# theo2021/OnDA

Hardware: AMD Instinct MI355X
Metric: adaptation-step images/sec (fwd+bwd+proto) 512x1024 bs=4 (higher is better)
Workload: dtype f32 (f16x2 split emulation); 1 GPU; hybrid_switch adaptation step (step + update_ema), 1024x512, bs=4 per micro-batch, 1 micro-batch(es) per GPU and optimizer step, dynamic branch, DeepLabV2-ResNet50 ProDA head, random-init weights; global_batch=4, parallelism=dp1, branch=dynamic, micro_batches_per_gpu=1, inputs=resident in HBM

## Files before the change

include/onda_hip.h:

```cpp
#ifndef ONDA_HIP_H
#define ONDA_HIP_H

#include <stdint.h>

#ifdef __cplusplus
extern "C" {
#endif

typedef void* onda_stream_t;

#define ONDA_OK 0
#define ONDA_EINVAL (-1)
#define ONDA_EALIGN (-2)

typedef struct OndaConv {
  int B, Hi, Wi, Cin;
  int Ho, Wo, Cout;
  int kh, kw, stride, dil, pad;
  int ldx;
  int ldy;
  int ldr;
  int out_os;
  int Hf, Wf;
  int relu;
  const int32_t* run_if;
  int64_t stat_split;
  int32_t plain_schedule;
  const int32_t* pix_table;
  int64_t pix_stride;
} OndaConv;

int onda_conv_tiles_m(int M);
int onda_conv_tiles_mc(int M, int Cout);

int64_t onda_conv_ws_floats(void);
int onda_conv2d_fwd(const float* x, const float* w, float* y, const float* scale, const float* shift,
                    const float* residual, float* stats, float* ws, const OndaConv* c, onda_stream_t s);

#define ONDA_AMAX_SLOTS 64
#define ONDA_AMAX_FLOATS 2048
int onda_absmax(const float* x, int64_t rows, int C, int ld, float* amax, onda_stream_t s);
int onda_pack_weight_h2(const float* w_oihw, void* dst, int Cout, int Cin, int taps, int rows_pad, int Kp, int dgrad,
                        int Cout_pad, const float* amax, onda_stream_t s);
typedef struct {
  const float* w;
  void* fwd;
  void* dgrad;
  float* amax;
  int Cout, Cin, taps;
  int first_block;
} OndaPackEntry;
int onda_pack_blocks(int Cout, int Cin, int taps);
int onda_pack_weights_h2_multi(const OndaPackEntry* table, int n, int64_t total_blocks, onda_stream_t s);
int onda_split_h2(const float* x, int64_t rows, int C, int ldx, void* dst, int ldo, int64_t plane, const float* amax,
                  onda_stream_t s);
typedef struct OndaLimbOut {
  void* out;
  int64_t out_plane;
  float* out_bound;
  float* out_amax;
  const float* kb;
  const float* xtrue;
  const void* res;
  int64_t res_plane;
  const float* res_amax;
  const float* res_true;
} OndaLimbOut;
int onda_conv2d_fwd_l2_limbs(const void* xl, int64_t xplane, const float* xamax, const void* w2, const float* wamax,
                             const float* scale, const float* shift, const OndaLimbOut* lo, float* ws, const OndaConv* c,
                             onda_stream_t s);

void onda_debug_stamps(void* buffer);

int onda_stem_im2col_l2(const float* x_nchw, const float* xamax, void* dst, int64_t plane, int B, int H, int W, int Ho, int Wo,
                        int Kp, onda_stream_t s);
int onda_s2d_split_h2(const float* x, int nchw, int B, int C, int H, int W, int ldx, float slope, const float* amax, void* dst,
                      onda_stream_t s);
int onda_d2s_bwd(const float* gs, const float* gamax, const float* x, int nchw, int B, int C, int H, int W, int ldx, float slope,
                 void* dst_limbs, float* dst_f32, onda_stream_t s);
int onda_conv_l2_variant(int64_t M, int Cout);
int onda_conv_l2_kernel_id(int64_t M, int Cout, int taps, int Cin);
int onda_conv_l2_tiles_m(int64_t M, int Cout, int taps, int Cin);
int onda_conv_l2_tiles_m_split(int64_t M, int Cout, int taps, int Cin, int64_t stat_split, int plain_schedule, int* tile_rows);
double onda_conv_l2_live_fraction(const OndaConv* c, int with_stats);
double onda_conv_wgrad_l2_live_fraction(const OndaConv* c, int splitk);
int onda_conv2d_fwd_l2(const void* xl, int64_t xplane, const float* xamax, const void* w2, const float* wamax, float* y,
                       const float* scale, const float* shift, const float* residual, float* stats, int stats_rows, float* ws,
                       float* yamax, const OndaConv* c, onda_stream_t s);

int onda_bn_finalize_l2(const float* partials, int tiles, int C, int64_t count, float eps, float* mean, float* invstd,
                        float* running_mean, float* running_var, int64_t* nbt, float momentum, const float* gamma,
                        const float* beta, const float* res_amax, int relu, float* xhat_amax, float* out_amax, int64_t split,
                        int tile_rows, int run_group, const float* y, int ldy, onda_stream_t s);
int onda_bn_apply_l2(const float* x, const float* mean, const float* invstd, const float* gamma, const float* beta,
                     const void* res, int64_t res_plane, const float* res_amax, void* out, int64_t out_plane,
                     const float* out_amax, int64_t M, int C, int relu, uint8_t* relu_mask, int64_t split, onda_stream_t s);
int onda_bn_train_l2(const float* x, const float* partials, int tiles, float eps, float* mean, float* invstd, float* running_mean,
                     float* running_var, int64_t* nbt, float momentum, const float* gamma, const float* beta, const void* res,
                     const float* res_amax, int relu, float* xhat_amax, void* out, float* out_amax, int64_t M, int C,
                     uint8_t* relu_mask, int64_t split, int tile_rows, int run_group, onda_stream_t s);
int64_t onda_bn_bwd_l2_ws(int64_t M, int C);
int onda_bn_bwd_l2(const float* dout, const void* out, int64_t out_plane, const float* x, const float* mean, const float* invstd,
                   const float* gamma, const float* xhat_amax, void* dx, int64_t dx_plane, float* dx_amax, float* dres, float* ws,
                   int64_t M, int C, int relu, const uint8_t* relu_mask, int64_t split, int fuse_sums, onda_stream_t s);

int onda_conv_wgrad_l2_variant(int Cout, int Cin);
int64_t onda_conv2d_wgrad_l2_table_stride(const OndaConv* c);
int onda_conv2d_wgrad_l2_table(const OndaConv* c, int32_t* table, onda_stream_t s);
int onda_conv2d_wgrad_l2(const void* xl, int64_t xplane, const float* xamax, const void* dyl, int64_t dyplane, const float* dyamax,
                         float* slabs, int lddy, int splitk, const OndaConv* c, onda_stream_t s);

int onda_conv2d_wgrad(const float* x, const float* dy, float* slabs, int lddy, int splitk,
                      const OndaConv* c, onda_stream_t s);
int onda_wgrad_reduce(const float* slabs, float* dw, int splitk, int Cout, int taps, int Cin,
                      int Cout_real, int Cin_real, int flat_k, int accumulate, onda_stream_t s);

int onda_pack_weight_fwd(const float* w_oihw, float* dst, int Cout, int Cin, int taps, int Cout_pad, int Kp,
                         onda_stream_t s);
int onda_pack_weight_dgrad(const float* w_oihw, float* dst, int Cout, int Cin, int taps, int Cout_pad,
                           onda_stream_t s);

int onda_stem_im2col(const float* x_nchw, float* col, int B, int H, int W, int Ho, int Wo, int Kp, onda_stream_t s);

int onda_bn_finalize(const float* partials, int tiles, int C, int64_t count, float eps, float* mean, float* invstd,
                     float* running_mean, float* running_var, int64_t* num_batches_tracked, float momentum,
                     onda_stream_t s);
int onda_bn_stats(const float* x, int64_t M, int C, int ldx, float* partials, int* tiles_out, onda_stream_t s);
int onda_bn_apply(const float* x, const float* mean, const float* invstd, const float* gamma, const float* beta,
                  const float* residual, float* out, int64_t M, int C, int relu, float* amax, onda_stream_t s);
int onda_bn_fold(const float* gamma, const float* beta, const float* running_mean, const float* running_var,
                 float eps, float* scale, float* shift, int C, onda_stream_t s);
int64_t onda_bn_bwd_ws(int64_t M, int C);
int onda_bn_bwd(const float* dout, const float* out, const float* x, const float* mean, const float* invstd,
                const float* gamma, float* dx, float* dres, float* ws, int64_t M, int C, int relu, float* amax, onda_stream_t s);

int64_t onda_gn_ws(int B, int64_t HW, int C);
int onda_gn_fwd(const float* x, int ldx, const float* gamma, const float* beta, const float* chmul, float* out, int ldo,
                float* mean, float* rstd, float* ws, int B, int64_t HW, int C, int groups, float eps, int relu,
                float* amax ,
                onda_stream_t s);
int onda_gn_bwd(const float* dout, int lddo, const float* out, int ldo, const float* x, int ldx, const float* gamma,
                const float* chmul, const float* mean, const float* rstd, float* dx, float* dgamma, float* dbeta,
                float* ws, int B, int64_t HW, int C, int groups, int relu, onda_stream_t s);

int onda_maxpool_fwd(const float* x, float* y, uint8_t* idx, int B, int Hi, int Wi, int C, int Ho, int Wo,
                     onda_stream_t s);
int onda_maxpool_fwd_limbs(const float* x, const float* xamax, void* yl, uint8_t* idx, int B, int Hi, int Wi, int C, int Ho, int Wo,
                           onda_stream_t s);
int onda_maxpool_bwd(const float* dy, const uint8_t* idx, float* dx, int B, int Hi, int Wi, int C, int Ho, int Wo,
                     onda_stream_t s);

int64_t onda_colsum_ws(int B, int64_t HW, int C);
int onda_colsum(const float* x, int ldx, const float* y, int ldy, float* out, float alpha, float* ws, int B,
                int64_t HW, int C, onda_stream_t s);
int onda_se_fc_fwd(const float* pooled, const float* w1, const float* b1, const float* w2, const float* b2,
                   float* hidden, float* gate, int B, int C, int R, onda_stream_t s);
int onda_se_fc_bwd(const float* dgate, const float* pooled, const float* hidden, const float* gate, const float* w1,
                   const float* w2, float* dw1, float* db1, float* dw2, float* db2, float* dpooled, float* ws,
                   float dpooled_scale, int B, int C, int R, onda_stream_t s);
int onda_chan_scale(const float* x, const float* gate, const float* add, float* out, int B, int64_t HW, int C,
                    onda_stream_t s);
int onda_chan_scale_limbs(const float* x, const float* gate, void* out, int64_t out_plane, const float* x_amax, int B, int64_t HW,
                          int C, onda_stream_t s);

int onda_upsample_fwd(const float* logits, int ldl, float* out_nchw, int B, int h, int w, int K, int H, int W,
                      onda_stream_t s);
int onda_upsample_bwd(const float* dout_nchw, float* dlogits, int ldl, int B, int h, int w, int K, int H, int W,
                      onda_stream_t s);
int onda_upsample_ce_fused(int w, int W);
int64_t onda_upsample_ce_ws(int B, int H, int W);
int onda_upsample_ce_fwd(const float* logits, int ldl, const uint8_t* labels, float* result, float* ws, int B, int h, int w, int K,
                         int H, int W, onda_stream_t s);
int64_t onda_upsample_ce_bwd_ws(int B, int w, int K, int H);
int onda_upsample_ce_bwd(const float* logits, int ldl, const uint8_t* labels, const float* result, const float* gscale, float w_ce,
                         float* dlogits, float* ws, int B, int h, int w, int K, int H, int W, onda_stream_t s);
int onda_upsample_entropy_fwd(const float* logits, int ldl, float* out, int B, int h, int w, int K, int H, int W, onda_stream_t s);
int64_t onda_upsample_entropy_bwd_ws(int B, int w, int K, int H, int W);
int onda_upsample_entropy_bwd(const float* logits, int ldl, const float* dout, float* dlogits, float* ws, int B, int h, int w, int K,
                              int H, int W, onda_stream_t s);
int onda_upsample_argmax(const float* logits, int ldl, uint8_t* cls, int B, int h, int w, int K, int H, int W,
                         onda_stream_t s);

int onda_upsample_argmax_hist(const float* logits, int ldl, const uint8_t* labels, int64_t* hist, uint8_t* cls, int B,
                              int h, int w, int K, int H, int W, onda_stream_t s);

int onda_ece_bins_local(void);
int onda_upsample_ece(const float* rows, int ld, const uint8_t* labels, int64_t* table, int bins, int probs, int64_t* hist, int B,
                      int h, int w, int K, int H, int W, onda_stream_t s);

int onda_softmax_stats(const float* logits, int ldl, float* probs, int ldp, int32_t* argmax, float* result,
                       float* ws, int64_t N, int K, onda_stream_t s);

int onda_seg_loss_fwd(const float* logits, int ldl, const int64_t* labels, float* result, float* ws, int64_t N, int K,
                      onda_stream_t s);
int onda_seg_loss_bwd(const float* logits, int ldl, const int64_t* labels, const float* result, const float* gscale,
                      float w_ce, float w_rce, float w_reg, float* dlogits, int64_t N, int K, onda_stream_t s);

int onda_target_loss_fwd(const float* logits, int ldl, const int64_t* labels, int regularizer, float w_ce, float w_rce,
                         float w_reg, float w_js, float* result, float* ws, int64_t N, int K, onda_stream_t s);
int onda_target_loss_bwd(const float* logits, int ldl, const int64_t* labels, int regularizer, float w_ce, float w_rce,
                         float w_reg, float w_js, const float* result, const float* gscale, float* dlogits, int64_t N,
                         int K, onda_stream_t s);

int onda_proto_assign_blocks(int64_t N);
int onda_proto_sigma(const float* proto, const float* sqmean, const float* counter, float* sigma, int K, int C,
                     onda_stream_t s);
int onda_proto_assign(const float* feat, int ldf, const float* prior, int ldp, const float* proto, const float* sigma,
                      int mahalanobis, float tau, float thresh, int64_t* labels, float* soft, float* result,
                      float* ws, int64_t N, int C, int K, onda_stream_t s);
int onda_proto_distances(const float* feat, int ldf, const float* proto, const float* sigma, int mahalanobis, float* dist,
                         int64_t N, int C, int K, onda_stream_t s);
int64_t onda_proto_sums_ws(int64_t N, int C, int K);
int onda_proto_class_sums(const float* feat, int ldf, const int32_t* cls, float* sums, float* counts, float* ws,
                          int64_t N, int C, int K, onda_stream_t s);
int onda_proto_ema(float* proto, float* sqmean, const float* sums, const float* counts, float lam, int K, int C,
                   onda_stream_t s);
int onda_proto_append(float* proto, float* sqmean, float* counter, const float* sums, const float* counts, int K,
                      int C, onda_stream_t s);

typedef struct OndaSgdEntry {
  float* p; const float* g; float* buf; int64_t n; float lr; int times; int fresh;
  int first_block;
} OndaSgdEntry;
int onda_multi_tensor_block(void);
int onda_sgd_multi(const OndaSgdEntry* table, int n, float momentum, float weight_decay, float grad_scale,
                   int64_t total_blocks, onda_stream_t s);
typedef struct OndaEmaEntry { float* k; const float* q; int64_t n; float keep; float blend; int first_block; } OndaEmaEntry;
int onda_ema_multi(const OndaEmaEntry* table, int n, int64_t total_blocks, onda_stream_t s);

int onda_resample_h_u8(const unsigned char* in, unsigned char* out, int H, int Win, int Wout, const int* bounds,
                       const int* kk, int ksize, onda_stream_t s);
int onda_resample_v_norm(const unsigned char* tmp, float* out, int Hin, int W, int Hout, const int* bounds, const int* kk,
                         int ksize, const float* mean3, const float* std3, int flip, onda_stream_t s);
int onda_resize_nearest_lut(const unsigned char* in, unsigned char* out, int Win, int Hout, int Wout, const int* xtab,
                            const int* ytab, const unsigned char* lut256, onda_stream_t s);

const char* onda_version(void);
float onda_limb2_scale(void);

typedef struct OndaSwitchCfg {
  int limit;
  int level_kind;
  int use_exp;
  int pad_;
  double exp_const, one_minus_exp_const, taps_total;
  double gray_lo, gray_hi, dev_threshold;
} OndaSwitchCfg;
int onda_switch_state_doubles(int limit);
int onda_switch_max_window(void);
int onda_switch_step(double* state, int32_t* istate, const void* sample, int sample_f64, const double* taps,
                     const OndaSwitchCfg* cfg, int32_t* flag, onda_stream_t s);
int onda_select_prior(const int32_t* flag, const float* a, float wa, const float* b, float wb, float* out, int64_t n,
                      onda_stream_t s);
int onda_gate_scalar(const int32_t* flag, const float* v, float* out, onda_stream_t s);

#ifdef __cplusplus
}
#endif
#endif
```

onda_amd/_lib.py:

```python
import ctypes
import os
from ctypes import POINTER, Structure, c_char_p, c_float, c_int, c_int64, c_void_p

HERE = os.path.dirname(os.path.abspath(__file__))
LIB_PATH = os.environ.get("ONDA_LIB_PATH") or os.path.join(HERE, "libonda_hip.so")

P = c_void_p
I, L, F = c_int, c_int64, c_float


class OndaConv(Structure):
    _fields_ = [(n, c_int) for n in ("B Hi Wi Cin Ho Wo Cout kh kw stride dil pad ldx ldy ldr out_os Hf Wf relu").split()] + \
               [("run_if", c_void_p), ("stat_split", c_int64), ("plain_schedule", c_int), ("pix_table", c_void_p),
                ("pix_stride", c_int64)]


class OndaSwitchCfg(Structure):
    _fields_ = [("limit", c_int), ("level_kind", c_int), ("use_exp", c_int), ("pad_", c_int), ("exp_const", ctypes.c_double),
                ("one_minus_exp_const", ctypes.c_double), ("taps_total", ctypes.c_double), ("gray_lo", ctypes.c_double),
                ("gray_hi", ctypes.c_double), ("dev_threshold", ctypes.c_double)]


class OndaLimbOut(Structure):
    _fields_ = [("out", c_void_p), ("out_plane", c_int64), ("out_bound", c_void_p), ("out_amax", c_void_p), ("kb", c_void_p),
                ("xtrue", c_void_p), ("res", c_void_p), ("res_plane", c_int64), ("res_amax", c_void_p), ("res_true", c_void_p)]


class OndaSgdEntry(Structure):
    _fields_ = [("p", c_void_p), ("g", c_void_p), ("buf", c_void_p), ("n", c_int64), ("lr", c_float),
                ("times", c_int), ("fresh", c_int), ("first_block", c_int)]


class OndaPackEntry(Structure):
    _fields_ = [("w", c_void_p), ("fwd", c_void_p), ("dgrad", c_void_p), ("amax", c_void_p), ("Cout", c_int), ("Cin", c_int),
                ("taps", c_int), ("first_block", c_int)]


class OndaEmaEntry(Structure):
    _fields_ = [("k", c_void_p), ("q", c_void_p), ("n", c_int64), ("keep", c_float), ("blend", c_float), ("first_block", c_int)]


SIGNATURES = {
    "onda_conv_tiles_m": (I, [I]),
    "onda_conv_tiles_mc": (I, [I, I]),
    "onda_conv_ws_floats": (L, []),
    "onda_conv2d_fwd": (I, [P, P, P, P, P, P, P, P, POINTER(OndaConv), P]),
    "onda_absmax": (I, [P, L, I, I, P, P]),
    "onda_pack_weight_h2": (I, [P, P, I, I, I, I, I, I, I, P, P]),
    "onda_pack_weights_h2_multi": (I, [P, I, L, P]),
    "onda_pack_blocks": (I, [I, I, I]),
    "onda_split_h2": (I, [P, L, I, I, P, I, L, P, P]),
    "onda_stem_im2col_l2": (I, [P, P, P, L, I, I, I, I, I, I, P]),
    "onda_s2d_split_h2": (I, [P, I, I, I, I, I, I, F, P, P, P]),
    "onda_d2s_bwd": (I, [P, P, P, I, I, I, I, I, I, F, P, P, P]),
    "onda_debug_stamps": (None, [P]),
    "onda_conv2d_fwd_l2_limbs": (I, [P, L, P, P, P, P, P, P, P, P, P]),
    "onda_switch_state_doubles": (I, [I]),
    "onda_switch_max_window": (I, []),
    "onda_switch_step": (I, [P, P, P, I, P, POINTER(OndaSwitchCfg), P, P]),
    "onda_select_prior": (I, [P, P, F, P, F, P, L, P]),
    "onda_gate_scalar": (I, [P, P, P, P]),
    "onda_conv_l2_variant": (I, [L, I]),
    "onda_conv_l2_kernel_id": (I, [L, I, I, I]),
    "onda_conv_l2_tiles_m": (I, [L, I, I, I]),
    "onda_conv_l2_tiles_m_split": (I, [L, I, I, I, L, I, POINTER(c_int)]),
    "onda_conv_l2_live_fraction": (ctypes.c_double, [POINTER(OndaConv), I]),
    "onda_conv_wgrad_l2_live_fraction": (ctypes.c_double, [POINTER(OndaConv), I]),
    "onda_conv_wgrad_l2_variant": (I, [I, I]),
    "onda_conv2d_wgrad_l2_table_stride": (L, [POINTER(OndaConv)]),
    "onda_conv2d_wgrad_l2_table": (I, [POINTER(OndaConv), P, P]),
    "onda_conv2d_wgrad_l2": (I, [P, L, P, P, L, P, P, I, I, POINTER(OndaConv), P]),
    "onda_conv2d_fwd_l2": (I, [P, L, P, P, P, P, P, P, P, P, I, P, P, POINTER(OndaConv), P]),
    "onda_bn_finalize_l2": (I, [P, I, I, L, F, P, P, P, P, P, F, P, P, P, I, P, P, L, I, I, P, I, P]),
    "onda_bn_apply_l2": (I, [P, P, P, P, P, P, L, P, P, L, P, L, I, I, P, L, P]),
    "onda_bn_bwd_l2_ws": (L, [L, I]),
    "onda_bn_train_l2": (I, [P, P, I, F, P, P, P, P, P, F, P, P, P, P, I, P, P, P, L, I, P, L, I, I, P]),
    "onda_bn_bwd_l2": (I, [P, P, L, P, P, P, P, P, P, L, P, P, P, L, I, I, P, L, I, P]),
    "onda_conv2d_wgrad": (I, [P, P, P, I, I, POINTER(OndaConv), P]),
    "onda_wgrad_reduce": (I, [P, P, I, I, I, I, I, I, I, I, P]),
    "onda_pack_weight_fwd": (I, [P, P, I, I, I, I, I, P]),
    "onda_pack_weight_dgrad": (I, [P, P, I, I, I, I, P]),
    "onda_stem_im2col": (I, [P, P, I, I, I, I, I, I, P]),
    "onda_bn_finalize": (I, [P, I, I, L, F, P, P, P, P, P, F, P]),
    "onda_bn_stats": (I, [P, L, I, I, P, POINTER(c_int), P]),
    "onda_bn_apply": (I, [P, P, P, P, P, P, P, L, I, I, P, P]),
    "onda_bn_fold": (I, [P, P, P, P, F, P, P, I, P]),
    "onda_bn_bwd_ws": (L, [L, I]),
    "onda_bn_bwd": (I, [P, P, P, P, P, P, P, P, P, L, I, I, P, P]),
    "onda_gn_ws": (L, [I, L, I]),
    "onda_gn_fwd": (I, [P, I, P, P, P, P, I, P, P, P, I, L, I, I, F, I, P, P]),
    "onda_gn_bwd": (I, [P, I, P, I, P, I, P, P, P, P, P, P, P, P, I, L, I, I, I, P]),
    "onda_maxpool_fwd": (I, [P, P, P, I, I, I, I, I, I, P]),
    "onda_maxpool_fwd_limbs": (I, [P, P, P, P, I, I, I, I, I, I, P]),
    "onda_maxpool_bwd": (I, [P, P, P, I, I, I, I, I, I, P]),
    "onda_colsum_ws": (L, [I, L, I]),
    "onda_colsum": (I, [P, I, P, I, P, F, P, I, L, I, P]),
    "onda_se_fc_fwd": (I, [P, P, P, P, P, P, P, I, I, I, P]),
    "onda_se_fc_bwd": (I, [P, P, P, P, P, P, P, P, P, P, P, P, F, I, I, I, P]),
    "onda_chan_scale": (I, [P, P, P, P, I, L, I, P]),
    "onda_chan_scale_limbs": (I, [P, P, P, L, P, I, L, I, P]),
    "onda_upsample_fwd": (I, [P, I, P, I, I, I, I, I, I, P]),
    "onda_upsample_bwd": (I, [P, P, I, I, I, I, I, I, I, P]),
    "onda_upsample_argmax": (I, [P, I, P, I, I, I, I, I, I, P]),
    "onda_upsample_ce_fused": (I, [I, I]),
    "onda_upsample_ce_ws": (L, [I, I, I]),
    "onda_upsample_ce_fwd": (I, [P, I, P, P, P, I, I, I, I, I, I, P]),
    "onda_upsample_ce_bwd_ws": (L, [I, I, I, I]),
    "onda_upsample_ce_bwd": (I, [P, I, P, P, P, F, P, P, I, I, I, I, I, I, P]),
    "onda_upsample_entropy_fwd": (I, [P, I, P, I, I, I, I, I, I, P]),
    "onda_upsample_entropy_bwd_ws": (L, [I, I, I, I, I]),
    "onda_upsample_entropy_bwd": (I, [P, I, P, P, P, I, I, I, I, I, I, P]),
    "onda_upsample_argmax_hist": (I, [P, I, P, P, P, I, I, I, I, I, I, P]),
    "onda_ece_bins_local": (I, []),
    "onda_upsample_ece": (I, [P, I, P, P, I, I, P, I, I, I, I, I, I, P]),
    "onda_softmax_stats": (I, [P, I, P, I, P, P, P, L, I, P]),
    "onda_seg_loss_fwd": (I, [P, I, P, P, P, L, I, P]),
    "onda_seg_loss_bwd": (I, [P, I, P, P, P, F, F, F, P, L, I, P]),
    "onda_target_loss_fwd": (I, [P, I, P, I, F, F, F, F, P, P, L, I, P]),
    "onda_target_loss_bwd": (I, [P, I, P, I, F, F, F, F, P, P, P, L, I, P]),
    "onda_proto_sigma": (I, [P, P, P, P, I, I, P]),
    "onda_proto_assign_blocks": (I, [L]),
    "onda_proto_assign": (I, [P, I, P, I, P, P, I, F, F, P, P, P, P, L, I, I, P]),
    "onda_proto_distances": (I, [P, I, P, P, I, P, L, I, I, P]),
    "onda_proto_sums_ws": (L, [L, I, I]),
    "onda_proto_class_sums": (I, [P, I, P, P, P, P, L, I, I, P]),
    "onda_proto_ema": (I, [P, P, P, P, F, I, I, P]),
    "onda_proto_append": (I, [P, P, P, P, P, I, I, P]),
    "onda_sgd_multi": (I, [P, I, F, F, F, L, P]),
    "onda_ema_multi": (I, [P, I, L, P]),
    "onda_multi_tensor_block": (I, []),
    "onda_resample_h_u8": (I, [P, P, I, I, I, P, P, I, P]),
    "onda_resample_v_norm": (I, [P, P, I, I, I, P, P, I, POINTER(c_float), POINTER(c_float), I, P]),
    "onda_resize_nearest_lut": (I, [P, P, I, I, I, P, P, P, P]),
    "onda_version": (c_char_p, []),
    "onda_limb2_scale": (F, []),
}

_lib = None


class OndaLibraryError(RuntimeError):
    pass


def load():
    global _lib
    if _lib is not None:
        return _lib
    if not os.path.exists(LIB_PATH):
        raise OndaLibraryError(
            f"{LIB_PATH} is missing: build it with `python -m onda_amd.build` (hipcc --offload-arch=gfx950). "
            "onda_amd has no fallback path.")
    import torch
    lib = ctypes.CDLL(LIB_PATH)
    for name, (res, args) in SIGNATURES.items():
        try:
            fn = getattr(lib, name)
        except AttributeError as e:
            raise OndaLibraryError(f"{LIB_PATH} does not export {name}") from e
        fn.restype, fn.argtypes = res, args
    _lib = lib
    return lib


def call(name, *args):
    rc = getattr(load(), name)(*args)
    if rc != 0:
        kind = {-1: "ONDA_EINVAL (unsupported shape / null pointer)", -2: "ONDA_EALIGN (16-byte alignment)"}.get(
            rc, f"hipError_t {rc}")
        raise RuntimeError(f"{name} failed: {kind}")


def query(name, *args):
    return getattr(load(), name)(*args)
```

onda_amd/csrc/common.h:

```cpp
#pragma once
#include <hip/hip_runtime.h>
#include <stdint.h>
#include <stdio.h>
#include <stdlib.h>

#include "onda_hip.h"

#ifndef ONDA_LIMB2_SCALE
#define ONDA_LIMB2_SCALE 2048.f
#endif
typedef float f32x4 __attribute__((ext_vector_type(4)));
typedef float f32x16 __attribute__((ext_vector_type(16)));

constexpr int LIMB2_OFS = 32;
__host__ __device__ __forceinline__ size_t limb_at(size_t row, int c, int ld) {
  return row * 2 * (size_t)ld + (size_t)((c >> 5) << 6) + (size_t)(c & 31);
}

#define ONDA_STREAM(s) (reinterpret_cast<hipStream_t>(s))
#define ONDA_REQUIRE(cond)                                                                              \
  do {                                                                                                  \
    (void)hipGetLastError();                                                                            \
    if (!(cond)) {                                                                                      \
      if (getenv("ONDA_DEBUG_REQUIRE")) fprintf(stderr, "onda_hip: %s:%d: requirement failed: %s\n", __FILE__, __LINE__, #cond); \
      return ONDA_EINVAL;                                                                               \
    }                                                                                                   \
  } while (0)
#define ONDA_ALIGNED16(p) ((reinterpret_cast<uintptr_t>(p) & 15u) == 0)
#define ONDA_LAUNCH_RESULT() static_cast<int>(hipGetLastError())

static inline int64_t ceil_div64(int64_t a, int64_t b) { return (a + b - 1) / b; }

__device__ __forceinline__ float wave_sum(float v) {
#pragma unroll
  for (int o = 32; o > 0; o >>= 1) v += __shfl_xor(v, o, 64);
  return v;
}
__device__ __forceinline__ float wave_max(float v) {
#pragma unroll
  for (int o = 32; o > 0; o >>= 1) v = fmaxf(v, __shfl_xor(v, o, 64));
  return v;
}

constexpr int AMAX_STRIDE = ONDA_AMAX_FLOATS / ONDA_AMAX_SLOTS;
__device__ __forceinline__ void amax_update(float* amax, float m) {
  m = wave_max(m);
  if ((threadIdx.x & 63) == 0 && m > 0.f)
    atomicMax(reinterpret_cast<unsigned*>(amax) + ((blockIdx.x * 4 + (threadIdx.x >> 6)) & (ONDA_AMAX_SLOTS - 1)) * AMAX_STRIDE,
              __float_as_uint(m));
}
__device__ __forceinline__ void amax_update_block(float* amax, float m, float* red) {
  m = wave_max(m);
  if ((threadIdx.x & 63) == 0) red[threadIdx.x >> 6] = m;
  __syncthreads();
  if (threadIdx.x == 0) {
    m = fmaxf(fmaxf(red[0], red[1]), fmaxf(red[2], red[3]));
    if (m > 0.f)
      atomicMax(reinterpret_cast<unsigned*>(amax) + (blockIdx.x & (ONDA_AMAX_SLOTS - 1)) * AMAX_STRIDE, __float_as_uint(m));
  }
}
__device__ __forceinline__ float amax_read(const float* __restrict__ amax) {
  static_assert(ONDA_AMAX_SLOTS == 64, "one slot per lane");
  return wave_max(amax[(threadIdx.x & 63) * AMAX_STRIDE]);
}

__device__ __forceinline__ double wave_sum_d(double v) {
#pragma unroll
  for (int o = 32; o > 0; o >>= 1) v += __shfl_xor(v, o, 64);
  return v;
}

__device__ __forceinline__ float block_sum_256(float v, float* red) {
  v = wave_sum(v);
  __syncthreads();
  if ((threadIdx.x & 63) == 0) red[threadIdx.x >> 6] = v;
  __syncthreads();
  return red[0] + red[1] + red[2] + red[3];
}
```

onda_amd/csrc/conv_l2.hip:

```cpp
#include "conv_common.h"

namespace {

typedef _Float16 f16x8 __attribute__((ext_vector_type(8)));
typedef _Float16 f16x2 __attribute__((ext_vector_type(2)));
typedef _Float16 f16x4 __attribute__((ext_vector_type(4)));
typedef float f32x2 __attribute__((ext_vector_type(2)));
typedef unsigned int u32x2 __attribute__((ext_vector_type(2)));
typedef unsigned int u32x4 __attribute__((ext_vector_type(4)));
typedef int i32x4 __attribute__((ext_vector_type(4)));

#define ZZ(i, jj) (((i) & 1) ? 3 - (jj) : (jj))

constexpr float LIMB2_SCALE = ONDA_LIMB2_SCALE, LIMB2_UNSCALE = 1.f / ONDA_LIMB2_SCALE;

#ifndef ONDA_NT_OUT
#define ONDA_NT_OUT 1
#endif
constexpr int NT_AUX = ONDA_NT_OUT ? 2 : 0;
template <class T>
__device__ __forceinline__ void store_out(T* p, T v) {
  if constexpr (ONDA_NT_OUT) __builtin_nontemporal_store(v, p); else *p = v;
}
constexpr unsigned OOB = 0x80000000u;

__device__ __forceinline__ __amdgpu_buffer_rsrc_t make_rsrc(const void* base, unsigned bytes) {
  return __builtin_amdgcn_make_buffer_rsrc(const_cast<void*>(base), 0, (int)bytes, 0x00020000);
}
__device__ __forceinline__ int swz8(int row) { return (row & 15) >> 1; }
__device__ __forceinline__ unsigned dma_chunk16(int lane, int odd) { return (unsigned)(((lane & 7) ^ (4 * odd + (lane >> 4))) << 4); }
__device__ __forceinline__ int frag_ofs(int lane, int limb) {
  return (lane & 15) * 128 + ((((limb << 2) | (lane >> 4)) ^ swz8(lane & 15)) << 4);
}
struct RowPos {
  int hw;
  int bH;
};
__device__ __forceinline__ RowPos row_pos(int m, int M, const OndaConv& c, int b0) {
  const bool vm = m < M;
  const int mm = vm ? m : 0;
  const int wo = mm % c.Wo, tq = mm / c.Wo;
  const int ho = tq % c.Ho, b = tq / c.Ho;
  const int hi0 = vm ? ho * c.stride - c.pad : -32768, wi0 = wo * c.stride - c.pad;
  return RowPos{(int)((unsigned)(hi0 & 0xFFFF) | ((unsigned)wi0 << 16)), (vm ? b - b0 : 0) * c.Hi};
}
__device__ __forceinline__ __amdgpu_buffer_rsrc_t x_window(const ConvK& a, int m0, int& b0) {
  const OndaConv& c = a.c;
  b0 = m0 / (c.Ho * c.Wo);
  const long long at = (long long)b0 * c.Hi * c.Wi * c.ldx * 4, left = a.x_total - at;
  return make_rsrc(reinterpret_cast<const char*>(a.x) + at, (unsigned)(left < 0x7FFFF000ll ? left : 0x7FFFF000ll));
}
__device__ __forceinline__ unsigned row_tap_ofs(const RowPos& p, int rr, int ss, const OndaConv& c, unsigned chunk16) {
  const int hi = (int)(short)(p.hw & 0xFFFF) + rr * c.dil, wi = (p.hw >> 16) + ss * c.dil;
  const bool ok = (unsigned)hi < (unsigned)c.Hi && (unsigned)wi < (unsigned)c.Wi;
  return ok ? (unsigned)(((p.bH + hi) * c.Wi + wi) * c.ldx) * 4u + chunk16 : 0x80000000u;
}

struct Scale2 {
  float s, inv;
};
__device__ __forceinline__ Scale2 scale_from(float m);
__device__ __forceinline__ Scale2 scale_of(const float* __restrict__ amax) { return scale_from(amax_read(amax)); }
__device__ __forceinline__ Scale2 scale_from(const float m) {
  int e = 0;
  if (m > 0.f && m < 3.0e38f) {
    int ex;
    frexpf(m, &ex);
    e = 15 - ex;
    e = e > 100 ? 100 : (e < -100 ? -100 : e);
  }
  return Scale2{ldexpf(1.f, e), ldexpf(1.f, -e)};
}

__device__ __forceinline__ unsigned cvt2h(float lo, float hi) {
  return __builtin_bit_cast(unsigned, __builtin_convertvector(f32x2{lo, hi}, f16x2));
}
__device__ __forceinline__ f32x2 unpack2h(unsigned p) {
  return __builtin_convertvector(__builtin_bit_cast(f16x2, p), f32x2);
}

__global__ __launch_bounds__(256) void split_h2_kernel(const float* __restrict__ x, long long rows, int C, int ldx,
                                                       _Float16* __restrict__ dst, int ldo, long long plane,
                                                       const float* __restrict__ amax) {
  const float s = scale_of(amax).s;
  const int c8 = C >> 3;
  const long long n = rows * c8;
  for (long long e = (long long)blockIdx.x * 256 + threadIdx.x; e < n; e += (long long)gridDim.x * 256) {
    const long long row = e / c8;
    const int ch = (int)(e - row * c8) * 8;
    const f32x4 v0 = *reinterpret_cast<const f32x4*>(x + row * ldx + ch) * s;
    const f32x4 v1 = *reinterpret_cast<const f32x4*>(x + row * ldx + ch + 4) * s;
    u32x4 l1, l2;
#pragma unroll
    for (int h = 0; h < 4; ++h) {
      const float a = h < 2 ? v0[2 * h] : v1[2 * h - 4], b = h < 2 ? v0[2 * h + 1] : v1[2 * h - 3];
      const unsigned p = cvt2h(a, b);
      const f32x2 f = unpack2h(p);
      l1[h] = p;
      l2[h] = cvt2h((a - f[0]) * LIMB2_SCALE, (b - f[1]) * LIMB2_SCALE);
    }
    _Float16* o = dst + limb_at((size_t)row, ch, ldo);
    *reinterpret_cast<u32x4*>(o) = l1;
    *reinterpret_cast<u32x4*>(o + LIMB2_OFS) = l2;
  }
}

__global__ __launch_bounds__(256) void stem_im2col_l2_kernel(const float* __restrict__ x, _Float16* __restrict__ dst,
                                                             long long plane, int B, int H, int W, int Ho, int Wo, int Kp,
                                                             const float* __restrict__ amax) {
  const float sc = scale_of(amax).s;
  const int k8 = Kp >> 3;
  const long long n = (long long)B * Ho * Wo * k8;
  for (long long e = (long long)blockIdx.x * 256 + threadIdx.x; e < n; e += (long long)gridDim.x * 256) {
    const long long m = e / k8;
    const int k0 = (int)(e - m * k8) * 8;
    const int wo = (int)(m % Wo);
    const long long tq = m / Wo;
    const int ho = (int)(tq % Ho), b = (int)(tq / Ho);
    float v[8];
#pragma unroll
    for (int j = 0; j < 8; ++j) {
      const int k = k0 + j;
      float val = 0.f;
      if (k < 147) {
        const int tap = k / 3, cc = k - tap * 3;
        const int r = tap / 7, t7 = tap - r * 7;
        const int hi = ho * 2 - 3 + r, wi = wo * 2 - 3 + t7;
        if ((unsigned)hi < (unsigned)H && (unsigned)wi < (unsigned)W) val = x[(((size_t)b * 3 + cc) * H + hi) * W + wi];
      }
      v[j] = val * sc;
    }
    u32x4 l1, l2;
#pragma unroll
    for (int h = 0; h < 4; ++h) {
      const unsigned pk = cvt2h(v[2 * h], v[2 * h + 1]);
      const f32x2 f = unpack2h(pk);
      l1[h] = pk;
      l2[h] = cvt2h((v[2 * h] - f[0]) * LIMB2_SCALE, (v[2 * h + 1] - f[1]) * LIMB2_SCALE);
    }
    _Float16* o = dst + limb_at((size_t)m, k0, Kp);
    *reinterpret_cast<u32x4*>(o) = l1;
    *reinterpret_cast<u32x4*>(o + LIMB2_OFS) = l2;
  }
}

#define ONDA_SWAP4(INSN, A, B)                                                                                          \
  asm volatile("s_nop 1\n\t" INSN " %0, %4\n\t" INSN " %1, %5\n\t" INSN " %2, %6\n\t" INSN " %3, %7\n\ts_nop 0"         \
               : "+v"(A[0]), "+v"(A[1]), "+v"(A[2]), "+v"(A[3]), "+v"(B[0]), "+v"(B[1]), "+v"(B[2]), "+v"(B[3]))
__device__ __forceinline__ void rows_reduce4(float& s1, float& s2, float& mn, float& mx) {
#if defined(__HIP_DEVICE_COMPILE__)
  float A[4] = {s1, s2, mn, mx}, B[4] = {s1, s2, mn, mx};
  ONDA_SWAP4("v_permlane16_swap_b32", A, B);
  float C[4] = {A[0] + B[0], A[1] + B[1], fminf(A[2], B[2]), fmaxf(A[3], B[3])};
  float D[4] = {C[0], C[1], C[2], C[3]};
  ONDA_SWAP4("v_permlane32_swap_b32", C, D);
  s1 = C[0] + D[0];
  s2 = C[1] + D[1];
  mn = fminf(C[2], D[2]);
  mx = fmaxf(C[3], D[3]);
#endif
}

template <int WM, int WN, bool COUNTED = false, bool AFFINE = true>
__device__ __forceinline__ void l2_epilogue(const ConvK& a, const f32x4 (&acc)[4][4], unsigned char* scratch, int tile_m, int m0,
                                            int n0, int wm, int wn, int lane, float ua, float ub, unsigned y_bytes = 0) {
  constexpr int BN = 64 * WN, NW = WM * WN, NT = NW * 64;
  constexpr int TRS = 68;
  const OndaConv& c = a.c;
  const int t = threadIdx.x, wave = t >> 6;
  unsigned long long* est = a.stamps != nullptr && t == 0 ? a.stamps + (size_t)blockIdx.x * 32 + 24 : nullptr;
  if (est) est[0] = __builtin_amdgcn_s_memtime();
  float* red = reinterpret_cast<float*>(scratch + NW * (16 * TRS * 4));
  const int SR = a.stats_rows;
  if (a.stats != nullptr) {
#pragma unroll
    for (int jn = 0; jn < 4; ++jn) {
      float s1 = 0.f, s2 = 0.f, mn = 3.0e38f, mxv = -3.0e38f;
#pragma unroll
      for (int i = 0; i < 4; ++i)
#pragma unroll
        for (int e = 0; e < 4; ++e) {
          const float v = acc[i][jn][e];
          s1 += v;
          s2 += v * v;
          mn = fminf(mn, v);
          mxv = fmaxf(mxv, v);
        }
      rows_reduce4(s1, s2, mn, mxv);
      if (lane < 16) {
        const int col = (wn * 4 + jn) * 16 + lane;
        red[(wm * BN + col) * 4 + 0] = (s1 * ua) * ub;
        red[(wm * BN + col) * 4 + 1] = (((s2 * ua) * ub) * ua) * ub;
        red[(wm * BN + col) * 4 + 2] = (mn * ua) * ub;
        red[(wm * BN + col) * 4 + 3] = (mxv * ua) * ub;
      }
    }
  }

  if (est) est[1] = __builtin_amdgcn_s_memtime();
  const bool plain = (c.out_os == 1 && c.Hf == c.Ho && c.Wf == c.Wo);
  const int cl = (lane & 15) * 4, rl = lane >> 4;
  const int n = n0 + wn * 64 + cl;
  const bool vn = n < c.Cout;
  f32x4 sc = {1.f, 1.f, 1.f, 1.f}, sh = {0.f, 0.f, 0.f, 0.f};
  if constexpr (AFFINE) {
    if (vn && a.scale) sc = *reinterpret_cast<const f32x4*>(a.scale + n);
    if (vn && a.shift) sh = *reinterpret_cast<const f32x4*>(a.shift + n);
  }
  sc = (sc * ua) * ub;
  float* tr = reinterpret_cast<float*>(scratch + wave * (16 * TRS * 4));
  float mx = 0.f;
  f32x4 rv[4][4];
  if (AFFINE && a.res) {
#pragma unroll
    for (int i = 0; i < 4; ++i)
#pragma unroll
      for (int r = 0; r < 4; ++r) {
        const int m = m0 + (wm * 4 + i) * 16 + 4 * r + rl;
        const bool live = m < a.M && vn;
        rv[i][r] = live ? *reinterpret_cast<const f32x4*>(a.res + (size_t)m * c.ldr + n) : f32x4{0.f, 0.f, 0.f, 0.f};
      }
  }
  const bool track = a.amax != nullptr;
  const bool full_rows = m0 + 64 * WM <= a.M;
  const int mw = m0 + wm * 64 + rl;
  const unsigned vbase = vn ? (unsigned)(((size_t)(mw - m0) * c.ldy + n) * 4) : OOB;
  const long long y_left = (long long)(a.M - m0) * c.ldy * 4;
  const unsigned y_win = (unsigned)(y_left < 0x7FFFF000ll ? y_left : 0x7FFFF000ll);
  float* const ytile = a.y + (size_t)m0 * c.ldy;
  float* const ybase = a.y + (size_t)mw * c.ldy + n;
#pragma unroll
  for (int i = 0; i < 4; ++i) {
#pragma unroll
    for (int jn = 0; jn < 4; ++jn)
#pragma unroll
      for (int e = 0; e < 4; ++e) tr[(4 * (lane >> 4) + e) * TRS + jn * 16 + (lane & 15)] = acc[i][jn][e];
    __builtin_amdgcn_wave_barrier();
#pragma unroll
    for (int r = 0; r < 4; ++r) {
      const int row = 4 * r + rl;
      f32x4 v = *reinterpret_cast<const f32x4*>(tr + row * TRS + cl);
      const int m = mw + i * 16 + 4 * r;
      const bool live = (full_rows || m < a.M) && vn;
      if constexpr (AFFINE) {
        v = v * sc + sh;
        if (a.res) v += rv[i][r];
        if (c.relu) {
#pragma unroll
          for (int q = 0; q < 4; ++q) v[q] = fmaxf(v[q], 0.f);
        }
      } else {
        v = v * sc;
      }
      if (plain) {
        if constexpr (COUNTED) {
#if defined(__HIP_DEVICE_COMPILE__)
          __builtin_amdgcn_raw_buffer_store_b128(__builtin_bit_cast(u32x4, v), make_rsrc(ytile, y_win),
                                                 vbase + (unsigned)((i * 16 + 4 * r) * c.ldy * 4), 0, NT_AUX);
#endif
        } else if (live) {
          store_out(reinterpret_cast<f32x4*>(ybase + (size_t)((i * 16 + 4 * r) * c.ldy)), v);
        }
      } else {
        const int mm = live ? m : 0;
        const int wo = mm % c.Wo, tq = mm / c.Wo;
        const int ho = tq % c.Ho, b = tq / c.Ho;
        const size_t orow = ((size_t)b * c.Hf + (size_t)ho * c.out_os) * c.Wf + (size_t)wo * c.out_os;
        if constexpr (COUNTED) {
#if defined(__HIP_DEVICE_COMPILE__)
          const unsigned off = live ? (unsigned)((orow * c.ldy + n) * 4) : OOB;
          __builtin_amdgcn_raw_buffer_store_b128(__builtin_bit_cast(u32x4, v), make_rsrc(a.y, y_bytes), off, 0, NT_AUX);
#endif
        } else if (live) {
          store_out(reinterpret_cast<f32x4*>(a.y + orow * c.ldy + n), v);
        }
      }
      if (track && live) mx = fmaxf(fmaxf(mx, fmaxf(fabsf(v[0]), fabsf(v[1]))), fmaxf(fabsf(v[2]), fabsf(v[3])));
    }
    __builtin_amdgcn_wave_barrier();
  }
  if (est) est[2] = __builtin_amdgcn_s_memtime();
  float* ar = red + WM * BN * 4;
  if (a.amax != nullptr) {
    mx = wave_max(mx);
    if (lane == 0) ar[wave] = mx;
  }
  if (a.stats != nullptr || a.amax != nullptr) {
    if constexpr (COUNTED) {
      asm volatile("s_waitcnt lgkmcnt(0)" ::: "memory");
      __builtin_amdgcn_s_barrier();
    } else {
      __syncthreads();
    }
  }
  if (est) est[3] = __builtin_amdgcn_s_memtime();
  if (a.stats != nullptr) {
    for (int col = t; col < BN; col += NT) {
      if (n0 + col >= c.Cout) continue;
      float s1 = 0.f, s2 = 0.f, mn = 3.0e38f, mxv = -3.0e38f;
#pragma unroll
      for (int w_ = 0; w_ < WM; ++w_) {
        s1 += red[(w_ * BN + col) * 4 + 0];
        s2 += red[(w_ * BN + col) * 4 + 1];
        mn = fminf(mn, red[(w_ * BN + col) * 4 + 2]);
        mxv = fmaxf(mxv, red[(w_ * BN + col) * 4 + 3]);
      }
      float* dst = a.stats + (size_t)tile_m * SR * c.Cout + n0 + col;
      dst[0] = s1;
      dst[c.Cout] = s2;
      if (SR == 4) {
        dst[2 * c.Cout] = mn;
        dst[3 * c.Cout] = mxv;
      }
    }
  }
  if (a.amax != nullptr && t == 0) {
    float m = ar[0];
#pragma unroll
    for (int w_ = 1; w_ < NW; ++w_) m = fmaxf(m, ar[w_]);
    if (m > 0.f)
      atomicMax(reinterpret_cast<unsigned*>(a.amax) + (blockIdx.x & (ONDA_AMAX_SLOTS - 1)) * AMAX_STRIDE, __float_as_uint(m));
  }
  if (est) est[4] = __builtin_amdgcn_s_memtime();
}

__device__ __forceinline__ float limb_out_bound(const ConvK& a) {
  float b = amax_read(a.xtrue) * a.kb[0] + a.kb[1];
  if (a.resl != nullptr) b += amax_read(a.res_true);
  return b * 1.0001f;
}

template <int WM, int WN, bool COUNTED>
__device__ __forceinline__ void l2_epilogue_limbs(const ConvK& a, const f32x4 (&acc)[4][4], unsigned char* scratch, int m0, int n0,
                                                  int wm, int wn, int lane, float ua, float ub) {
  constexpr int BN = 64 * WN, NW = WM * WN;
  constexpr int TRS = 68;
  const OndaConv& c = a.c;
  if constexpr (COUNTED) asm volatile("" : "+v"(lane));
  int t = threadIdx.x;
  if constexpr (COUNTED) asm volatile("" : "+v"(t));
  const int wave = t >> 6;
  const float bound = limb_out_bound(a);
  const float so = scale_from(bound).s;
  if (t == 0) a.ybound[(blockIdx.x & (ONDA_AMAX_SLOTS - 1)) * AMAX_STRIDE] = bound;
  const float ri = a.resl != nullptr ? scale_of(a.res_amax).inv : 0.f;
  const int cl = (lane & 15) * 4, rl = lane >> 4;
  const int n = n0 + wn * 64 + cl;
  const bool vn = n < c.Cout;
  f32x4 sc = {1.f, 1.f, 1.f, 1.f}, sh = {0.f, 0.f, 0.f, 0.f};
  if (vn && a.scale) sc = *reinterpret_cast<const f32x4*>(a.scale + n);
  if (vn && a.shift) sh = *reinterpret_cast<const f32x4*>(a.shift + n);
  sc = (sc * ua) * ub;
  float* tr = reinterpret_cast<float*>(scratch + wave * (16 * TRS * 4));
  float* ar = reinterpret_cast<float*>(scratch + NW * (16 * TRS * 4));
  const int mw = m0 + wm * 64 + rl;
  u32x2 r1[4][4], r2[4][4];
  if (a.resl != nullptr) {
#pragma unroll
    for (int i = 0; i < 4; ++i)
#pragma unroll
      for (int r = 0; r < 4; ++r) {
        const int m = mw + i * 16 + 4 * r;
        const bool live = m < a.M && vn;
        const _Float16* p = a.resl + limb_at((size_t)(live ? m : 0), live ? n : 0, c.ldr);
        r1[i][r] = live ? *reinterpret_cast<const u32x2*>(p) : u32x2{0u, 0u};
        r2[i][r] = live ? *reinterpret_cast<const u32x2*>(p + LIMB2_OFS) : u32x2{0u, 0u};
      }
  }
  float mx = 0.f;
  const long long out_left = (long long)(a.M - m0) * c.ldy * 4;
  const unsigned out_bytes = (unsigned)(out_left < 0x7FFFF000ll ? out_left : 0x7FFFF000ll);
  _Float16* const ytile = a.yl + (size_t)m0 * 2 * c.ldy;
#pragma unroll
  for (int i = 0; i < 4; ++i) {
#pragma unroll
    for (int jn = 0; jn < 4; ++jn)
#pragma unroll
      for (int e = 0; e < 4; ++e) tr[(4 * (lane >> 4) + e) * TRS + jn * 16 + (lane & 15)] = acc[i][jn][e];
    __builtin_amdgcn_wave_barrier();
#pragma unroll
    for (int r = 0; r < 4; ++r) {
      const int row = 4 * r + rl;
      f32x4 v = *reinterpret_cast<const f32x4*>(tr + row * TRS + cl);
      const int m = mw + i * 16 + 4 * r;
      const bool live = m < a.M && vn;
      v = v * sc + sh;
      if (a.resl != nullptr) {
#pragma unroll
        for (int h = 0; h < 2; ++h) {
          const f32x2 p1 = unpack2h(r1[i][r][h]), p2 = unpack2h(r2[i][r][h]);
          v[2 * h] += (p1[0] + p2[0] * LIMB2_UNSCALE) * ri;
          v[2 * h + 1] += (p1[1] + p2[1] * LIMB2_UNSCALE) * ri;
        }
      }
      if (c.relu) {
#pragma unroll
        for (int q = 0; q < 4; ++q) v[q] = fmaxf(v[q], 0.f);
      }
      if (live) mx = fmaxf(fmaxf(mx, fmaxf(fabsf(v[0]), fabsf(v[1]))), fmaxf(fabsf(v[2]), fabsf(v[3])));
      const f32x4 w = v * so;
      u32x2 l1, l2;
#pragma unroll
      for (int h = 0; h < 2; ++h) {
        const unsigned pk = cvt2h(w[2 * h], w[2 * h + 1]);
        const f32x2 f = unpack2h(pk);
        l1[h] = pk;
        l2[h] = cvt2h((w[2 * h] - f[0]) * LIMB2_SCALE, (w[2 * h + 1] - f[1]) * LIMB2_SCALE);
      }
      if constexpr (COUNTED) {
#if defined(__HIP_DEVICE_COMPILE__)
        const unsigned off = vn ? (unsigned)(limb_at((size_t)(m - m0), n, c.ldy) * 2) : OOB;
        __builtin_amdgcn_raw_buffer_store_b64(l1, make_rsrc(ytile, out_bytes), off, 0, NT_AUX);
        __builtin_amdgcn_raw_buffer_store_b64(l2, make_rsrc(ytile, out_bytes), off, 2 * LIMB2_OFS, NT_AUX);
#endif
      } else if (live) {
        _Float16* dst = a.yl + limb_at((size_t)m, n, c.ldy);
        store_out(reinterpret_cast<u32x2*>(dst), l1);
        store_out(reinterpret_cast<u32x2*>(dst + LIMB2_OFS), l2);
      }
    }
    __builtin_amdgcn_wave_barrier();
  }
  if (a.amax != nullptr) {
    mx = wave_max(mx);
    if (lane == 0) ar[wave] = mx;
    if constexpr (COUNTED) {
      asm volatile("s_waitcnt lgkmcnt(0)" ::: "memory");
      __builtin_amdgcn_s_barrier();
    } else {
      __syncthreads();
    }
    if (t == 0) {
      float mm = ar[0];
#pragma unroll
      for (int w_ = 1; w_ < NW; ++w_) mm = fmaxf(mm, ar[w_]);
      if (mm > 0.f)
        atomicMax(reinterpret_cast<unsigned*>(a.amax) + (blockIdx.x & (ONDA_AMAX_SLOTS - 1)) * AMAX_STRIDE, __float_as_uint(mm));
    }
  }
}

template <int WM, int WN, int STAGES, int OCC, bool SK, int DBG = 0>
__global__ __launch_bounds__(WM * WN * 64, OCC) void conv_l2_kernel(const ConvK a, unsigned xplane, unsigned wplane, unsigned x_bytes,
                                                                   unsigned w_bytes, const float* __restrict__ xamax,
                                                                   const float* __restrict__ wamax) {
// ... 1188 lines not shown
      }
    }
  }

  f32x4 acc[4][4], accx[4][4];
#pragma unroll
  for (int i = 0; i < 4; ++i)
#pragma unroll
    for (int j = 0; j < 4; ++j)
#pragma unroll
      for (int e = 0; e < 4; ++e) acc[i][j][e] = accx[i][j][e] = 0.f;

  if (stp) {
    stp[1] = __builtin_amdgcn_s_memtime();
    stp[5] = (unsigned long long)nlive;
  }
  int i_cur = 0, i_iss = 0;
  int st_issue = 0, st_read = 0;
  auto issue_next = [&]() {
    issue(live_at(i_iss), st_issue);
    st_issue = st_issue + STAGE == STAGES * STAGE ? 0 : st_issue + STAGE;
    ++i_iss;
  };
  bool second_part_due = false;
  auto issue_first_part = [&]() {
    second_part_due = i_iss < nlive;
    if (second_part_due) {
      issue_addr(live_at(i_iss), st_issue);
      issue_part(0);
      st_issue = st_issue + STAGE == STAGES * STAGE ? 0 : st_issue + STAGE;
      ++i_iss;
    }
  };
  auto issue_second_part = [&]() {
    if (second_part_due) issue_part(1);
    second_part_due = false;
  };
  auto wait_landed_half = [&](bool first_part_in_flight) {
    if (first_part_in_flight)
      asm volatile("s_waitcnt vmcnt(%0)" ::"n"(DPW / 2) : "memory");
    else
      asm volatile("s_waitcnt vmcnt(0)" ::: "memory");
  };
  auto wait_landed = [&](bool more_in_flight) {
    if (more_in_flight)
      asm volatile("s_waitcnt vmcnt(%0)" ::"n"(DPW) : "memory");
    else
      asm volatile("s_waitcnt vmcnt(0)" ::: "memory");
  };
  constexpr int AHEAD = STAGES >= 3 ? 2 : 1;
  static_assert(!STAGGER || STAGES >= 3, "the staggered halves need two steps in flight");
  if constexpr (MODE == 0) {
    if (i_iss < nlive) issue_next();
    if (AHEAD == 2 && i_iss < nlive) issue_next();
  }
  f16x8 af[4][2], bf[4], b1[4];
  const unsigned lds0 = (unsigned)(size_t)(__attribute__((address_space(3))) unsigned char*)lds;
  unsigned base;
  auto prepare = [&]() {
    base = lds0 + st_read;
    st_read = st_read + STAGE == STAGES * STAGE ? 0 : st_read + STAGE;
#pragma unroll
    for (int i = 0; i < 4; ++i) {
      const unsigned a0 = base + fa[i][0], a1 = base + fa[i][1];
      af[i][0] = tr_read8<0>(a0, a1);
      af[i][1] = tr_read8<256>(a0, a1);
    }
#pragma unroll
    for (int j = 0; j < 4; ++j) {
      const unsigned a0 = base + fb[j][0], a1 = base + fb[j][1];
      bf[j] = tr_read8<256>(a0, a1);
      if constexpr (STAGGER) b1[j] = tr_read8<0>(a0, a1);
    }
  };
  auto prepared = [&]() {
    lds_wait(af[0][0], af[1][0], af[2][0], af[3][0]);
    lds_wait(af[0][1], af[1][1], af[2][1], af[3][1]);
    lds_wait(bf[0], bf[1], bf[2], bf[3]);
    if constexpr (STAGGER) lds_wait(b1[0], b1[1], b1[2], b1[3]);
    __builtin_amdgcn_sched_barrier(0);
  };
  auto compute = [&]() {
    if constexpr (!STAGGER) {
#pragma unroll
      for (int j = 0; j < 4; ++j) b1[j] = tr_read8(base + fb[j][0], base + fb[j][1]);
    }
#pragma unroll
    for (int i = 0; i < 4; ++i)
#pragma unroll
      for (int jj = 0; jj < 4; ++jj) accx[i][ZZ(i, jj)] = __builtin_amdgcn_mfma_f32_16x16x32_f16(af[i][0], bf[ZZ(i, jj)], accx[i][ZZ(i, jj)], 0, 0, 0);
    if constexpr (!STAGGER) lds_wait(b1[0], b1[1], b1[2], b1[3]);
    if constexpr (STAGGER) issue_second_part();
    __builtin_amdgcn_sched_barrier(0);
#pragma unroll
    for (int i = 0; i < 4; ++i)
#pragma unroll
      for (int jj = 0; jj < 4; ++jj) accx[i][ZZ(i, jj)] = __builtin_amdgcn_mfma_f32_16x16x32_f16(af[i][1], b1[ZZ(i, jj)], accx[i][ZZ(i, jj)], 0, 0, 0);
#pragma unroll
    for (int i = 0; i < 4; ++i)
#pragma unroll
      for (int jj = 0; jj < 4; ++jj) acc[i][ZZ(i, jj)] = __builtin_amdgcn_mfma_f32_16x16x32_f16(af[i][0], b1[ZZ(i, jj)], acc[i][ZZ(i, jj)], 0, 0, 0);
  };
  if constexpr (MODE >= 1) {
    static_assert(STAGGER && GPW == 1 && STAGES == 3, "the eight-wave tile");
    const unsigned lddy4 = (unsigned)a.lddy * 4u, ldx4 = (unsigned)c.ldx * 4u;
    unsigned dy_lane[2], x_lane[2];
#pragma unroll
    for (int h = 0; h < 2; ++h) {
      const unsigned pix = (unsigned)(wave * 4 + 2 * lam + h);
      dy_lane[h] = pix * lddy4;
      x_lane[h] = (pix + (unsigned)(mbeg - b_first * c.Ho * c.Wo)) * ldx4;
    }
    const int base_px = b_first * c.Hi * c.Wi;
    const i32x4* tab = MODE == 2 ? reinterpret_cast<const i32x4*>(a.pix + (size_t)tap * a.pix_stride + mbeg + wave * 4) : nullptr;
    i32x4 t_next = {-1, -1, -1, -1};
    auto offsets = [&](int kt, const i32x4& te, unsigned kill) {
#pragma unroll
      for (int h = 0; h < 2; ++h) {
        pdy_s[0][h] = (unsigned)kt * 32u * lddy4 + dy_lane[h] + kill;
        if constexpr (MODE == 1) {
          px_s[0][h] = (unsigned)kt * 32u * ldx4 + x_lane[h] + kill;
        } else {
          const int lo = te[h], hi = te[2 + h];
          const int e = lam ? hi : lo;
          px_s[0][h] = (e >= 0 ? __umul24((unsigned)(e - base_px), ldx4) : PAST) + kill;
        }
      }
    };
    auto issue_first = [&]() {
      stage_s = st_issue;
      issue_part(0);
    };
    auto issue_second = [&]() {
      issue_part(1);
      st_issue = st_issue + STAGE == STAGES * STAGE ? 0 : st_issue + STAGE;
      ++i_iss;
    };
    auto issue_dmas = [&]() {
      issue_first();
      issue_second();
    };
    const unsigned long long tab_u = reinterpret_cast<unsigned long long>(tab);
    const unsigned tab_lo = __builtin_amdgcn_readfirstlane((unsigned)tab_u), tab_hi = __builtin_amdgcn_readfirstlane((unsigned)(tab_u >> 32));
    auto entry = [&](int kt) -> i32x4 {
      i32x4 r = {0, 0, 0, 0};
      if constexpr (MODE == 2) {
        const unsigned long long p = (((unsigned long long)tab_hi << 32) | tab_lo) + (unsigned long long)(unsigned)kt * 128ull;
        asm volatile("s_load_dwordx4 %0, %1, 0x0" : "=s"(r) : "s"(p));
      }
      return r;
    };
    auto entry_wait = [&](i32x4& r) {
      if constexpr (MODE == 2) asm volatile("s_waitcnt lgkmcnt(0)" : "+s"(r));
    };
    const int n_pre = late ? 3 : 2;
    if (nlive > 0) {
      for (int j = 0; j < n_pre; ++j) {
        const int kt = live_at(j < nlive ? j : 0);
        i32x4 te = entry(kt);
        entry_wait(te);
        offsets(kt, te, j < nlive ? 0u : PAST);
        issue_dmas();
      }
      int kt_next = live_at(i_iss < nlive ? i_iss : 0);
      t_next = entry(kt_next);
      entry_wait(t_next);
      if (late) {
        asm volatile("s_waitcnt vmcnt(%0)" ::"n"(2 * DPW) : "memory");
        __builtin_amdgcn_s_barrier();
      }
      for (; i_cur < nlive; ++i_cur) {
        if (!late) asm volatile("s_waitcnt vmcnt(%0)" ::"n"(DPW / 2) : "memory");
        __builtin_amdgcn_s_barrier();
        if (i_cur > 0) issue_second();
        const unsigned short ktv = live_list[i_iss + 1 < nlive ? i_iss + 1 : 0];
        prepare();
        prepared();
        const int kt_after = __builtin_amdgcn_readfirstlane((int)ktv);
        i32x4 t_after = entry(kt_after);
        if (late) asm volatile("s_waitcnt vmcnt(%0)" ::"n"(DPW) : "memory");
        __builtin_amdgcn_s_barrier();
        offsets(kt_next, t_next, i_iss < nlive ? 0u : PAST);
#pragma unroll
        for (int i = 0; i < 4; ++i)
#pragma unroll
          for (int jj = 0; jj < 4; ++jj) accx[i][ZZ(i, jj)] = __builtin_amdgcn_mfma_f32_16x16x32_f16(af[i][0], bf[ZZ(i, jj)], accx[i][ZZ(i, jj)], 0, 0, 0);
        issue_first();
#pragma unroll
        for (int i = 0; i < 4; ++i)
#pragma unroll
          for (int jj = 0; jj < 4; ++jj) accx[i][ZZ(i, jj)] = __builtin_amdgcn_mfma_f32_16x16x32_f16(af[i][1], b1[ZZ(i, jj)], accx[i][ZZ(i, jj)], 0, 0, 0);
#pragma unroll
        for (int i = 0; i < 4; ++i)
#pragma unroll
          for (int jj = 0; jj < 4; ++jj) acc[i][ZZ(i, jj)] = __builtin_amdgcn_mfma_f32_16x16x32_f16(af[i][0], b1[ZZ(i, jj)], acc[i][ZZ(i, jj)], 0, 0, 0);
        constexpr int NI = DPW / 2;
        __builtin_amdgcn_sched_group_barrier(0x008, 16, 0);
#pragma unroll
        for (int q = 0; q < 14; ++q) {
          __builtin_amdgcn_sched_group_barrier(0x008, 1, 0);
          __builtin_amdgcn_sched_group_barrier(0x002, 2, 0);
        }
#pragma unroll
        for (int q = 0; q < NI; ++q) {
          __builtin_amdgcn_sched_group_barrier(0x008, 2, 0);
          __builtin_amdgcn_sched_group_barrier(0x006, 2, 0);
          __builtin_amdgcn_sched_group_barrier(0x020, 1, 0);
        }
        __builtin_amdgcn_sched_group_barrier(0x008, 48 - 16 - 14 - 2 * NI, 0);
        __builtin_amdgcn_sched_barrier(0);
        entry_wait(t_after);
        kt_next = kt_after;
        t_next = t_after;
      }
      if (!late) __builtin_amdgcn_s_barrier();
      asm volatile("s_waitcnt vmcnt(0)" ::: "memory");
    }
  } else if constexpr (!STAGGER) {
    for (; i_cur < nlive; ++i_cur) {
      wait_landed(AHEAD == 2 && i_cur + 1 < nlive);
      __builtin_amdgcn_s_barrier();
      if (i_iss < nlive) issue_next();
      prepare();
      prepared();
      compute();
    }
  } else {
    if (late && nlive > 0) {
      wait_landed(nlive > 1);
      __builtin_amdgcn_s_barrier();
    }
    for (; i_cur < nlive; ++i_cur) {
      if (!late) wait_landed(i_cur + 1 < nlive);
      __builtin_amdgcn_s_barrier();
      unsigned long long tk0 = 0, tk1 = 0, tk2 = 0;
      if (stp) tk0 = __builtin_amdgcn_s_memtime();
      issue_first_part();
      if (stp) tk1 = __builtin_amdgcn_s_memtime();
      prepare();
      prepared();
      if (stp) tk2 = __builtin_amdgcn_s_memtime();
      if (late && i_cur + 1 < nlive) wait_landed_half(i_cur + 2 < nlive);
      __builtin_amdgcn_s_barrier();
      if (stp && i_cur == nlive / 2) {
        const unsigned long long tk3 = __builtin_amdgcn_s_memtime();
        stp[4] = ((tk1 - tk0) << 40) | ((tk2 - tk1) << 20) | (tk3 - tk2);
        stp[6] = tk3;
      }
      compute();
      if (stp && i_cur == nlive / 2) stp[7] = __builtin_amdgcn_s_memtime() - stp[6];
    }
    if (!late && nlive > 0) __builtin_amdgcn_s_barrier();
  }

#pragma unroll
  for (int i = 0; i < 4; ++i)
#pragma unroll
    for (int j = 0; j < 4; ++j) acc[i][j] = ((acc[i][j] + accx[i][j] * LIMB2_UNSCALE) * unscale_a) * unscale_b;
  if (stp) stp[2] = __builtin_amdgcn_s_memtime();
  __syncthreads();
  float* tr = reinterpret_cast<float*>(lds + (t >> 6) * 4096);
  const int cl = (lane & 15) * 4, rl = lane >> 4;
  const int cc = c0 + wn * 64 + cl;
#pragma unroll
  for (int i = 0; i < 4; ++i) {
#pragma unroll
    for (int jn = 0; jn < 4; ++jn)
#pragma unroll
      for (int e = 0; e < 4; ++e) tr[(4 * (lane >> 4) + e) * 64 + jn * 16 + (lane & 15)] = acc[i][jn][e];
    __builtin_amdgcn_wave_barrier();
#pragma unroll
    for (int r = 0; r < 4; ++r) {
      const int row = 4 * r + rl;
      const f32x4 v = *reinterpret_cast<const f32x4*>(tr + row * 64 + cl);
      const int n = n0 + (wm * 4 + i) * 16 + row;
      if (n < c.Cout && cc < c.Cin) *reinterpret_cast<f32x4*>(a.slabs + (((size_t)ks * c.Cout + n) * a.taps + tap) * c.Cin + cc) = v;
    }
    __builtin_amdgcn_wave_barrier();
  }
  if (stp) stp[3] = __builtin_amdgcn_s_memtime();
}

}

extern "C" {

int onda_split_h2(const float* x, int64_t rows, int C, int ldx, void* dst, int ldo, int64_t plane, const float* amax,
                  onda_stream_t s) {
  (void)plane;
  ONDA_REQUIRE(x && dst && amax && rows > 0 && C > 0 && C % 8 == 0 && ldx >= C && ldx % 4 == 0 && ldo >= C && ldo % 32 == 0);
  if (!ONDA_ALIGNED16(x) || !ONDA_ALIGNED16(dst)) return ONDA_EALIGN;
  const long long n = rows * (C / 8);
  const int blocks = (int)(n / 256 / 4 + 1 > 2048 ? 2048 : n / 256 / 4 + 1);
  hipLaunchKernelGGL(split_h2_kernel, dim3(blocks), dim3(256), 0, ONDA_STREAM(s), x, (long long)rows, C, ldx,
                     static_cast<_Float16*>(dst), ldo, (long long)plane, amax);
  return ONDA_LAUNCH_RESULT();
}

int onda_stem_im2col_l2(const float* x_nchw, const float* xamax, void* dst, int64_t plane, int B, int H, int W, int Ho, int Wo,
                        int Kp, onda_stream_t s) {
  (void)plane;
  ONDA_REQUIRE(x_nchw && xamax && dst && Kp % 32 == 0 && Kp >= 147 && B > 0 && Ho > 0 && Wo > 0);
  if (!ONDA_ALIGNED16(dst)) return ONDA_EALIGN;
  const long long n = (long long)B * Ho * Wo * (Kp / 8);
  const int blocks = (int)(n / 256 / 2 + 1 > 4096 ? 4096 : n / 256 / 2 + 1);
  hipLaunchKernelGGL(stem_im2col_l2_kernel, dim3(blocks), dim3(256), 0, ONDA_STREAM(s), x_nchw, static_cast<_Float16*>(dst),
                     (long long)plane, B, H, W, Ho, Wo, Kp, xamax);
  return ONDA_LAUNCH_RESULT();
}

}

namespace {
struct L2Overrides { bool has_variant; int variant; bool short_k128, stationary; int sched; };
L2Overrides l2_overrides() {
  static const int short_k128 = getenv("ONDA_L2_SHORTK128") ? atoi(getenv("ONDA_L2_SHORTK128")) : 1;
  const char* v = getenv("ONDA_L2_VARIANT");
  const char* a = getenv("ONDA_L2_STATIONARY");
  return {v != nullptr, v ? atoi(v) : 0, short_k128 != 0, a != nullptr && atoi(a) != 0, conv_sched_override()};
}

int l2_variant_mc(long long M, int Cout, const L2Overrides& o) {
  if (o.has_variant) return o.variant;
  if (Cout <= 64) return 2;
  const long long t256 = ((M + 255) / 256) * ((Cout + 127) / 128);
  return t256 >= 200 ? 0 : 1;
}

constexpr int L2X_MAX_KSTEPS = 32;

struct L2Epilogue { bool plain; bool dense_out; long long y_total; };

struct L2Plan {
  int kernel, variant, BM, BN, tilesM, tilesN, grid, G, rem, sub, tiles_dp;
  bool balanced;
  int rem_rows() const { return tilesM - (tilesM * tilesN - rem) / tilesN; }
  int stats_rows_total() const { return tilesM + (balanced ? rem_rows() * (sub - 1) : 0); }
};

L2Plan l2_plan(long long M, int Cout, int taps, int Cin, bool have_ws, long long stat_split, bool plain_schedule, const L2Epilogue* epi) {
  const L2Overrides o = l2_overrides();
  const int KT = taps * (Cin / 32);
  L2Plan q;
  q.variant = l2_variant_mc(M, Cout, o);
  if (q.variant == 0 && o.short_k128 && !o.has_variant && (KT <= 8 || (KT <= 16 && Cout >= 512) || (KT <= 32 && Cout >= 2048)))
    q.variant = 1;
  q.BM = q.variant == 1 ? 128 : 256;
  q.BN = q.variant == 2 ? 64 : 128;
  q.tilesM = (int)((M + q.BM - 1) / q.BM);
  q.tilesN = (Cout + q.BN - 1) / q.BN;
  const int cus = conv_resident_workgroups() / 2;
  q.G = q.variant == 0 ? cus : 2 * cus;
  q.sub = q.BM / (256 / (q.BN / 4));
  const int tiles = q.tilesM * q.tilesN;
  q.rem = tiles % q.G;
  const double t_tile_us = 2.0 * q.BM * q.BN * taps * Cin / 1.4e6;
  const double fix_us = 6.0 + (q.G + 2.0 * q.rem) * (q.BM * q.BN / 16384.0) * 0.02;
  q.balanced = have_ws && q.rem != 0 && KT >= 4 && t_tile_us * (1.0 - (double)q.rem / q.G) > fix_us &&
               (size_t)q.G * 2 * q.BM * q.BN <= (size_t)onda_conv_ws_floats() && q.G <= 1024;
  if (plain_schedule) q.balanced = false;
  const bool stationary = o.stationary && !o.has_variant && taps == 1 && (Cin == 64 || Cin == 128 || Cin == 256) && Cout >= 256 &&
                          q.variant == 1;
  if (stationary) q.balanced = false;
  if (o.sched == 1 || (o.sched != 0 && !have_ws)) q.balanced = false;
  else if (o.sched == 2) q.balanced = q.rem != 0;
  if (q.balanced && stat_split > 0 && (stat_split + q.BM - 1) / q.BM > (tiles - q.rem) / q.tilesN) q.balanced = false;
  if (stationary && (!epi || (epi->plain && epi->dense_out))) q.kernel = 4;
  else if (q.variant == 0 && KT <= L2X_MAX_KSTEPS && (!epi || epi->dense_out || epi->y_total < 0x7FFFF000ll)) q.kernel = 3;
  else q.kernel = q.variant;
  q.tiles_dp = q.kernel == 3 && !q.balanced ? tiles : tiles - q.rem;
  if (q.kernel == 4) q.grid = tiles < cus ? tiles : cus;
  else if (q.kernel == 3) q.grid = q.balanced || tiles > q.G ? q.G : tiles;
  else q.grid = q.balanced ? q.G : tiles;
  return q;
}
}

extern "C" {

int onda_conv_l2_variant(int64_t M, int Cout) { return l2_variant_mc(M, Cout, l2_overrides()); }

int onda_conv_l2_kernel_id(int64_t M, int Cout, int taps, int Cin) { return l2_plan(M, Cout, taps, Cin, true, 0, false, nullptr).kernel; }

int onda_conv_l2_tiles_m(int64_t M, int Cout, int taps, int Cin) { return l2_plan(M, Cout, taps, Cin, true, 0, false, nullptr).stats_rows_total(); }
int onda_conv_l2_tiles_m_split(int64_t M, int Cout, int taps, int Cin, int64_t stat_split, int plain_schedule, int* tile_rows) {
  const L2Plan q = l2_plan(M, Cout, taps, Cin, true, stat_split, plain_schedule != 0, nullptr);
  if (tile_rows) *tile_rows = q.BM;
  return q.stats_rows_total();
}

double onda_conv_l2_live_fraction(const OndaConv* c, int with_stats) {
  if (!c) return 1.0;
  const long long M = (long long)c->B * c->Ho * c->Wo;
  const int taps = c->kh * c->kw, kcper = c->Cin / 32;
  if (M <= 0 || taps <= 1 || kcper <= 0) return 1.0;
  const L2Plan q = l2_plan(M, c->Cout, taps, c->Cin, true, with_stats ? (long long)c->stat_split : 0, c->plain_schedule != 0, nullptr);
  if (q.kernel == 3) return 1.0;
  const int tiles = q.tilesM * q.tilesN, tiles_dp = q.balanced ? tiles - q.rem : tiles;
  long long live_steps = (long long)(tiles - tiles_dp) * taps * kcper;
  for (int tile_m = 0; tile_m * q.tilesN < tiles_dp; ++tile_m) {
    const int n_dp = tiles_dp - tile_m * q.tilesN < q.tilesN ? tiles_dp - tile_m * q.tilesN : q.tilesN;
    const long long m0 = (long long)tile_m * q.BM, m_last = (M < m0 + q.BM ? M : m0 + q.BM) - 1;
    const long long r0 = m0 / c->Wo, r1 = m_last / c->Wo;
    int live = 0;
    for (int tp = 0; tp < taps; ++tp) {
      const int dh = (tp / c->kw) * c->dil - c->pad;
      bool alive = false;
      for (long long r = r0; r <= r1 && !alive; ++r) alive = (unsigned)((int)(r % c->Ho) * c->stride + dh) < (unsigned)c->Hi;
      live += alive;
    }
    if (live == 0) live = 1;
    live_steps += (long long)n_dp * live * kcper;
  }
  return (double)live_steps / ((double)tiles * taps * kcper);
}

double onda_conv_wgrad_l2_live_fraction(const OndaConv* c, int splitk) {
  if (!c || splitk < 1) return 1.0;
  const long long M = (long long)c->B * c->Ho * c->Wo;
  const int taps = c->kh * c->kw;
  if (M <= 0 || taps <= 1) return 1.0;
  const long long mchunk = ((M + splitk - 1) / splitk + 31) / 32 * 32;
  long long live = 0, all = 0;
  for (int ks = 0; ks < splitk; ++ks) {
    const long long mbeg = ks * mchunk, mend = M < mbeg + mchunk ? M : mbeg + mchunk;
    const long long KT = mend > mbeg ? (mend - mbeg + 31) / 32 : 0;
    all += KT * taps;
    for (int tp = 0; tp < taps; ++tp) {
      const int dh = (tp / c->kw) * c->dil - c->pad;
      for (long long kt = 0; kt < KT; ++kt) {
        const long long m_first = mbeg + kt * 32, m_last = (mend < m_first + 32 ? mend : m_first + 32) - 1;
        bool alive = false;
        for (long long r = m_first / c->Wo; r <= m_last / c->Wo && !alive; ++r)
          alive = (unsigned)((int)(r % c->Ho) * c->stride + dh) < (unsigned)c->Hi;
        live += alive;
      }
    }
  }
  return all > 0 ? (double)live / (double)all : 1.0;
}

static int l2_fwd_impl(const void* xl, int64_t xplane, const float* xamax, const void* w2, const float* wamax, float* y,
                       const float* scale, const float* shift, const float* residual, float* stats, int stats_rows, float* ws,
                       float* yamax, const OndaConv* c, onda_stream_t s, const OndaLimbOut* lo) {
  ONDA_REQUIRE(xl && xamax && w2 && wamax && (y || lo) && c && ws && (stats_rows == 2 || stats_rows == 4));
  if (lo != nullptr) {
    ONDA_REQUIRE(lo->out && lo->out_bound && lo->kb && lo->xtrue && !stats && !residual);
    ONDA_REQUIRE(c->out_os == 1 && c->Hf == c->Ho && c->Wf == c->Wo && c->ldy % 32 == 0 && c->ldy >= c->Cout);
    ONDA_REQUIRE(!lo->res || (lo->res_amax && c->ldr % 32 == 0 && c->ldr >= c->Cout));
    if (!ONDA_ALIGNED16(lo->out) || (lo->res && !ONDA_ALIGNED16(lo->res))) return ONDA_EALIGN;
  }
  ONDA_REQUIRE(c->Cin > 0 && c->Cin % 32 == 0 && c->Cout > 0 && c->Cout % 4 == 0 && c->ldx % 32 == 0 && c->ldx >= c->Cin);
  ONDA_REQUIRE(c->kh >= 1 && c->kw >= 1 && c->stride >= 1 && c->dil >= 1 && c->out_os >= 1);
  (void)xplane;
  if (!ONDA_ALIGNED16(xl) || !ONDA_ALIGNED16(w2)) return ONDA_EALIGN;
  if (c->ldy % 4 != 0 || (y && !ONDA_ALIGNED16(y)) || (residual && (c->ldr % 4 != 0 || !ONDA_ALIGNED16(residual)))) return ONDA_EALIGN;
  if (scale && !ONDA_ALIGNED16(scale)) return ONDA_EALIGN;
  if (shift && !ONDA_ALIGNED16(shift)) return ONDA_EALIGN;
  const long long M = (long long)c->B * c->Ho * c->Wo;
  ONDA_REQUIRE(M > 0 && M < (1ll << 31));
  ONDA_REQUIRE((long long)c->Ho * c->stride + (long long)c->dil * (c->kh - 1) < 32768 &&
               (long long)c->Wo * c->stride + (long long)c->dil * (c->kw - 1) < 32768 && c->pad < 32768);
  {
    const long long img = (long long)c->Hi * c->Wi * c->ldx * 4, per_tile = 256 / ((long long)c->Ho * c->Wo) + 2;
    ONDA_REQUIRE((per_tile < c->B ? per_tile : c->B) * img < 0x7FFFF000ll);
  }
  ONDA_REQUIRE(c->stat_split >= 0 && c->stat_split < M);
  const size_t limb_elems = (size_t)c->Cout * c->kh * c->kw * c->Cin;
  ONDA_REQUIRE(limb_elems * 4 < (1ull << 31));

  ConvK k;
  k.x = static_cast<const float*>(xl); k.w = w2; k.y = y; k.scale = scale; k.shift = shift; k.res = residual; k.stats = stats; k.ws = ws;
  k.amax = yamax;
  k.stats_rows = stats_rows;
  if (lo != nullptr) {
    k.yl = static_cast<_Float16*>(lo->out);
    k.yplane = lo->out_plane;
    k.ybound = lo->out_bound;
    k.amax = lo->out_amax;
    k.kb = lo->kb;
    k.xtrue = lo->xtrue;
    k.resl = static_cast<const _Float16*>(lo->res);
    k.resplane = lo->res_plane;
    k.res_amax = lo->res_amax;
    k.res_true = lo->res_true ? lo->res_true : lo->res_amax;
  }
  k.skip_dead_taps = 1;
  k.late_issue = 1;
  static const int stamp_on = getenv("ONDA_L2X_STAMP") ? atoi(getenv("ONDA_L2X_STAMP")) : 0;
  if (stamp_on)
    k.stamps = reinterpret_cast<unsigned long long*>(ws + onda_conv_ws_floats()) - 1024 * 32;
  k.c = *c;
  k.x_total = (long long)c->B * c->Hi * c->Wi * c->ldx * 4;
  k.M = (int)M;
  k.taps = c->kh * c->kw;
  k.kcper = c->Cin / 32;

  const bool dense_out = c->out_os == 1 && c->Hf == c->Ho && c->Wf == c->Wo;
  const long long y_rows = (long long)c->B * (dense_out ? (long long)c->Ho * c->Wo : (long long)c->Hf * c->Wf);
  const long long y_total = ((y_rows - 1) * c->ldy + c->Cout) * 4;
  const L2Epilogue epi = {lo == nullptr && !scale && !shift && !residual && !c->relu && !yamax, dense_out, y_total};
  const L2Plan q = l2_plan(M, c->Cout, k.taps, c->Cin, true, stats ? (long long)c->stat_split : 0, c->plain_schedule != 0, &epi);
  ONDA_REQUIRE(q.variant >= 0 && q.variant <= 2);
  k.tilesM = q.tilesM;
  k.tilesN = q.tilesN;
  k.tiles_dp = q.tiles_dp;

  const unsigned x_bytes = 0, w_bytes = (unsigned)(limb_elems * 4);
  const unsigned xpl = 0, wpl = 0;
  hipStream_t st = ONDA_STREAM(s);
#define L2_FIXUP(BM_, BN_) \
  hipLaunchKernelGGL((conv_l2_fixup_kernel<BM_, BN_>), dim3(q.rem_rows() * q.tilesN, q.sub), dim3(256), 0, st, k, q.G, q.tilesM)
#define L2_LAUNCH(WM_, WN_, ST_, OCC_, ...)                                                                                  \
  do {                                                                                                                       \
    if (q.balanced) {                                                                                                        \
      hipLaunchKernelGGL((conv_l2_kernel<WM_, WN_, ST_, OCC_, true, ##__VA_ARGS__>), dim3(q.grid), dim3(WM_ * WN_ * 64), 0, st, k, xpl, \
                         wpl, x_bytes, w_bytes, xamax, wamax);                                                               \
      L2_FIXUP(64 * WM_, 64 * WN_);                                                                                          \
    } else {                                                                                                                 \
      hipLaunchKernelGGL((conv_l2_kernel<WM_, WN_, ST_, OCC_, false, ##__VA_ARGS__>), dim3(q.grid), dim3(WM_ * WN_ * 64), 0, st, k, xpl, \
                         wpl, x_bytes, w_bytes, xamax, wamax);                                                               \
    }                                                                                                                        \
  } while (0)
#define L2A_LAUNCH(KB_, NST_, A2L_) \
  hipLaunchKernelGGL((conv_l2a_kernel<KB_, NST_, A2L_, 0>), dim3(q.grid), dim3(512), 0, st, k, w_bytes, (unsigned)y_total, xamax, wamax)
  switch (q.kernel) {
    case 0:
#ifdef ONDA_L2_ABLATIONS
    {
      static const int dbg = getenv("ONDA_L2_DBG") ? atoi(getenv("ONDA_L2_DBG")) : 0;
#define L2_DBG_CASE(D_) case D_: L2_LAUNCH(4, 2, 3, 2, D_); return ONDA_LAUNCH_RESULT()
      switch (dbg) {
        L2_DBG_CASE(1); L2_DBG_CASE(2); L2_DBG_CASE(5); L2_DBG_CASE(7); L2_DBG_CASE(8); L2_DBG_CASE(9); L2_DBG_CASE(10); L2_DBG_CASE(11);
        L2_DBG_CASE(12);
      }
#undef L2_DBG_CASE
    }
#endif
      L2_LAUNCH(4, 2, 3, 2);
      break;
    case 1: L2_LAUNCH(2, 2, 2, 2); break;
    case 2: L2_LAUNCH(4, 1, 2, 2); break;
    case 3:
      hipLaunchKernelGGL((conv_l2x_kernel<4, 2, 3, 2>), dim3(q.grid), dim3(512), 0, st, k, xpl, wpl, x_bytes, w_bytes, (unsigned)y_total,
                         xamax, wamax);
      if (q.balanced) L2_FIXUP(256, 128);
      break;
    case 4:
      ONDA_REQUIRE(c->pad == 0 && (c->stride == 1 || (c->Hi >= (c->Ho - 1) * c->stride + 1 && c->Wi >= (c->Wo - 1) * c->stride + 1)));
      if (c->Cin == 256) L2A_LAUNCH(8, 3, true);
      else if (c->Cin == 128) L2A_LAUNCH(4, 3, false);
      else L2A_LAUNCH(2, 3, false);
      break;
  }
#undef L2A_LAUNCH
#undef L2_LAUNCH
#undef L2_FIXUP
  return ONDA_LAUNCH_RESULT();
}

int onda_conv2d_fwd_l2(const void* xl, int64_t xplane, const float* xamax, const void* w2, const float* wamax, float* y,
                       const float* scale, const float* shift, const float* residual, float* stats, int stats_rows, float* ws,
                       float* yamax, const OndaConv* c, onda_stream_t s) {
  return l2_fwd_impl(xl, xplane, xamax, w2, wamax, y, scale, shift, residual, stats, stats_rows, ws, yamax, c, s, nullptr);
}

int onda_conv2d_fwd_l2_limbs(const void* xl, int64_t xplane, const float* xamax, const void* w2, const float* wamax,
                             const float* scale, const float* shift, const OndaLimbOut* lo, float* ws, const OndaConv* c,
                             onda_stream_t s) {
  ONDA_REQUIRE(lo != nullptr);
  return l2_fwd_impl(xl, xplane, xamax, w2, wamax, nullptr, scale, shift, nullptr, nullptr, 2, ws, nullptr, c, s, lo);
}

static unsigned long long* g_debug_stamps = nullptr;
void onda_debug_stamps(void* p) { g_debug_stamps = static_cast<unsigned long long*>(p); }

int onda_conv_wgrad_l2_variant(int Cout, int Cin) {
  (void)Cin;
  return Cout >= 256 ? 0 : 1;
}

}

namespace {
__global__ __launch_bounds__(256) void wgrad_pixel_table_kernel(int* __restrict__ t, long long stride, int B, int Hi, int Wi, int Ho,
                                                               int Wo, int kw, int cstride, int dil, int pad) {
  const long long M = (long long)B * Ho * Wo;
  const int tap = blockIdx.y, rr = tap / kw, ss = tap - rr * kw;
  for (long long m = (long long)blockIdx.x * 256 + threadIdx.x; m < stride; m += (long long)gridDim.x * 256) {
    int v = -1;
    if (m < M) {
      const int wo = (int)(m % Wo);
      const long long q = m / Wo;
      const int ho = (int)(q % Ho), b = (int)(q / Ho);
      const int hi = ho * cstride + rr * dil - pad, wi = wo * cstride + ss * dil - pad;
      if ((unsigned)hi < (unsigned)Hi && (unsigned)wi < (unsigned)Wi) v = (b * Hi + hi) * Wi + wi;
    }
    t[(size_t)tap * stride + m] = v;
  }
}
}

extern "C" {

static bool wgrad_l2_linear(const OndaConv* c) {
  return c->kh == 1 && c->kw == 1 && c->stride == 1 && c->pad == 0 && c->Hi == c->Ho && c->Wi == c->Wo;
}

int64_t onda_conv2d_wgrad_l2_table_stride(const OndaConv* c) {
  if (!c || c->B <= 0 || c->Ho <= 0 || c->Wo <= 0) return 0;
// ... 66 lines not shown
```

onda_amd/csrc/norm_l2.hip:

```cpp
#include "common.h"

namespace {

typedef _Float16 f16x2 __attribute__((ext_vector_type(2)));
typedef float f32x2 __attribute__((ext_vector_type(2)));
typedef unsigned int u32x4 __attribute__((ext_vector_type(4)));
typedef unsigned int u32x2 __attribute__((ext_vector_type(2)));

constexpr float LIMB2_SCALE = ONDA_LIMB2_SCALE, LIMB2_UNSCALE = 1.f / ONDA_LIMB2_SCALE;

struct Scale2 {
  float s, inv;
};
__device__ __forceinline__ Scale2 scale_of(const float* __restrict__ amax) {
  const float m = amax_read(amax);
  int e = 0;
  if (m > 0.f && m < 3.0e38f) {
    int ex;
    frexpf(m, &ex);
    e = 15 - ex;
    e = e > 100 ? 100 : (e < -100 ? -100 : e);
  }
  return Scale2{ldexpf(1.f, e), ldexpf(1.f, -e)};
}
__device__ __forceinline__ unsigned cvt2h(float lo, float hi) {
  return __builtin_bit_cast(unsigned, __builtin_convertvector(f32x2{lo, hi}, f16x2));
}
__device__ __forceinline__ f32x2 unpack2h(unsigned p) {
  return __builtin_convertvector(__builtin_bit_cast(f16x2, p), f32x2);
}
__device__ __forceinline__ void split8(const f32x4 v0, const f32x4 v1, u32x4& l1, u32x4& l2) {
#pragma unroll
  for (int h = 0; h < 4; ++h) {
    const float a = h < 2 ? v0[2 * h] : v1[2 * h - 4], b = h < 2 ? v0[2 * h + 1] : v1[2 * h - 3];
    const unsigned p = cvt2h(a, b);
    const f32x2 f = unpack2h(p);
    l1[h] = p;
    l2[h] = cvt2h((a - f[0]) * LIMB2_SCALE, (b - f[1]) * LIMB2_SCALE);
  }
}
__device__ __forceinline__ void join8(const u32x4 l1, const u32x4 l2, f32x4& v0, f32x4& v1) {
#pragma unroll
  for (int h = 0; h < 4; ++h) {
    const f32x2 a = unpack2h(l1[h]), b = unpack2h(l2[h]);
    const float x0 = a[0] + b[0] * LIMB2_UNSCALE, x1 = a[1] + b[1] * LIMB2_UNSCALE;
    if (h < 2) {
      v0[2 * h] = x0;
      v0[2 * h + 1] = x1;
    } else {
      v1[2 * h - 4] = x0;
      v1[2 * h - 3] = x1;
    }
  }
}

#define LD4(p) (*reinterpret_cast<const f32x4*>(p))

__device__ __forceinline__ void store_limb_lines(_Float16* o, u32x4 l1, u32x4 l2, bool whole) {
  if (!whole) {
    *reinterpret_cast<u32x4*>(o) = l1;
    *reinterpret_cast<u32x4*>(o + LIMB2_OFS) = l2;
    return;
  }
  const bool hi = (threadIdx.x & 4) != 0;
  const u32x4 send = hi ? l1 : l2;
  u32x4 recv;
#pragma unroll
  for (int j = 0; j < 4; ++j) recv[j] = (unsigned)__shfl_xor((int)send[j], 4, 64);
  const unsigned long long mine = reinterpret_cast<unsigned long long>(o);
  const unsigned long long partner = ((unsigned long long)(unsigned)__shfl_xor((int)(mine >> 32), 4, 64) << 32) |
                                     (unsigned)__shfl_xor((int)(unsigned)mine, 4, 64);
  _Float16* po = reinterpret_cast<_Float16*>(partner);
  _Float16* a1 = hi ? po + LIMB2_OFS : o;
  _Float16* a2 = hi ? o + LIMB2_OFS : po;
  *reinterpret_cast<u32x4*>(a1) = hi ? recv : l1;
  *reinterpret_cast<u32x4*>(a2) = hi ? l2 : recv;
}

#ifndef ONDA_NT_BN
#define ONDA_NT_BN 0
#endif
template <class T>
__device__ __forceinline__ T ld_stream(const T* p) {
  if constexpr (ONDA_NT_BN & 1) return __builtin_nontemporal_load(p); else return *p;
}
template <class T>
__device__ __forceinline__ void st_stream(T* p, T v) {
  if constexpr (ONDA_NT_BN & 2) __builtin_nontemporal_store(v, p); else *p = v;
}
#define LD4S(p) ld_stream(reinterpret_cast<const f32x4*>(p))

__device__ __forceinline__ void grid_publish(float* amax_buf) {
  __threadfence();
  __syncthreads();
  if (threadIdx.x == 0) __hip_atomic_fetch_add(reinterpret_cast<int*>(amax_buf) + 1, 1, __ATOMIC_RELEASE, __HIP_MEMORY_SCOPE_AGENT);
}
__device__ __forceinline__ void grid_wait(float* amax_buf, int target) {
  if (threadIdx.x == 0) {
    int* flag = reinterpret_cast<int*>(amax_buf) + 1;
    int spins = 0;
    while (__hip_atomic_load(flag, __ATOMIC_ACQUIRE, __HIP_MEMORY_SCOPE_AGENT) < target) {
      if (++spins > (1 << 21)) {
        reinterpret_cast<int*>(amax_buf)[2] = 1;
        break;
      }
      __builtin_amdgcn_s_sleep(8);
    }
  }
  __syncthreads();
  __builtin_amdgcn_fence(__ATOMIC_ACQUIRE, "agent");
  asm volatile("" ::: "memory");
}

template <int NV, int NS, bool MINMAX>
__device__ __forceinline__ void reduce_rows16(const float* __restrict__ partials, int rows, int C, int ch0, double (&sum)[NS > 0 ? NS : 1],
                                              float (&ext)[NV - NS > 0 ? NV - NS : 1]) {
  constexpr int NE = NV - NS;
  __shared__ double lsum[4][NS > 0 ? NS : 1][16];
  __shared__ float lext[4][NE > 0 ? NE : 1][16];
  const int t = threadIdx.x, q = t & 3, rg = t >> 2, wave = t >> 6;
  const int col = ch0 + 4 * q;
  double s[NS > 0 ? NS : 1][4];
  float x[NE > 0 ? NE : 1][4];
#pragma unroll
  for (int v = 0; v < NS; ++v)
#pragma unroll
    for (int j = 0; j < 4; ++j) s[v][j] = 0.0;
#pragma unroll
  for (int v = 0; v < NE; ++v)
#pragma unroll
    for (int j = 0; j < 4; ++j) x[v][j] = MINMAX && v == 0 ? 3.0e38f : -3.0e38f;
  if (col < C) {
#pragma unroll 2
    for (int r = rg; r < rows; r += 64) {
      const float* p = partials + (size_t)r * NV * C + col;
      f32x4 val[NV];
#pragma unroll
      for (int v = 0; v < NV; ++v) val[v] = LD4(p + (size_t)v * C);
#pragma unroll
      for (int v = 0; v < NS; ++v)
#pragma unroll
        for (int j = 0; j < 4; ++j) s[v][j] += (double)val[v][j];
#pragma unroll
      for (int v = 0; v < NE; ++v)
#pragma unroll
        for (int j = 0; j < 4; ++j)
          x[v][j] = MINMAX && v == 0 ? fminf(x[v][j], val[NS + v][j]) : fmaxf(x[v][j], val[NS + v][j]);
    }
  }
#pragma unroll
  for (int o = 4; o < 64; o <<= 1) {
#pragma unroll
    for (int v = 0; v < NS; ++v)
#pragma unroll
      for (int j = 0; j < 4; ++j) s[v][j] += __shfl_xor(s[v][j], o, 64);
#pragma unroll
    for (int v = 0; v < NE; ++v)
#pragma unroll
      for (int j = 0; j < 4; ++j) {
        const float other = __shfl_xor(x[v][j], o, 64);
        x[v][j] = MINMAX && v == 0 ? fminf(x[v][j], other) : fmaxf(x[v][j], other);
      }
  }
  if ((t & 63) < 4) {
#pragma unroll
    for (int v = 0; v < NS; ++v)
#pragma unroll
      for (int j = 0; j < 4; ++j) lsum[wave][v][4 * q + j] = s[v][j];
#pragma unroll
    for (int v = 0; v < NE; ++v)
#pragma unroll
      for (int j = 0; j < 4; ++j) lext[wave][v][4 * q + j] = x[v][j];
  }
  __syncthreads();
  if (t < 16) {
#pragma unroll
    for (int v = 0; v < NS; ++v) sum[v] = ((lsum[0][v][t] + lsum[1][v][t]) + lsum[2][v][t]) + lsum[3][v][t];
#pragma unroll
    for (int v = 0; v < NE; ++v) {
      const float a = lext[0][v][t], b = lext[1][v][t], c = lext[2][v][t], d = lext[3][v][t];
      ext[v] = MINMAX && v == 0 ? fminf(fminf(a, b), fminf(c, d)) : fmaxf(fmaxf(a, b), fmaxf(c, d));
    }
  }
}

struct BnFinalizeArgs {
  const float* partials;
  int tiles, C;
  double count;
  float eps;
  float *mean, *invstd, *rmean, *rvar;
  int64_t* nbt;
  float momentum;
  const float *gamma, *beta, *res_amax;
  int relu;
  float *xhat_amax, *out_amax;
  long long split;
  int bm, run_group;
  const float* y;
  int ldy;
};
__device__ __forceinline__ void bn_finalize_block(const BnFinalizeArgs& a, const int bx, const int g) {
  const float* __restrict__ partials = a.partials;
  const int tiles = a.tiles, C = a.C, relu = a.relu, bm = a.bm, run_group = a.run_group, ldy = a.ldy;
  double count = a.count;
  const float eps = a.eps, momentum = a.momentum;
  float *mean = a.mean, *invstd = a.invstd, *rmean = a.rmean, *rvar = a.rvar, *xhat_amax = a.xhat_amax, *out_amax = a.out_amax;
  int64_t* nbt = a.nbt;
  const float* __restrict__ gamma = a.gamma;
  const float* __restrict__ beta = a.beta;
  const float* __restrict__ res_amax = a.res_amax;
  const float* __restrict__ y = a.y;
  const long long split = a.split;
  if (bx == 0 && g == 0 && threadIdx.x == 0 && nbt) *nbt += 1;
  int row0 = 0, nrows = tiles;
  if (split > 0) {
    const int ts = (int)(split / bm);
    if (g == 0) nrows = ts; else row0 = ts, nrows = tiles - ts;
    count = g == 0 ? (double)split : count - (double)split;
  }
  double sum[2];
  float ext[2];
  reduce_rows16<4, 2, true>(partials + (size_t)row0 * 4 * C, nrows, C, bx * 16, sum, ext);
  const int ch = bx * 16 + threadIdx.x;
  float bound = 0.f;
  if (threadIdx.x < 16 && ch < C) {
    if (split > 0 && split % bm != 0) {
      double c1 = 0.0, c2 = 0.0;
      float mn = 3.0e38f, mx = -3.0e38f;
      for (long long r = split - split % bm; r < split; ++r) {
        const float v = y[(size_t)r * ldy + ch];
        c1 += (double)v;
        c2 += (double)v * (double)v;
        mn = fminf(mn, v);
        mx = fmaxf(mx, v);
      }
      if (g == 0) {
        sum[0] += c1;
        sum[1] += c2;
        ext[0] = fminf(ext[0], mn);
        ext[1] = fmaxf(ext[1], mx);
      } else {
        sum[0] -= c1;
        sum[1] -= c2;
      }
    }
    const double mu = sum[0] / count;
    double var = sum[1] / count - mu * mu;
    if (var < 0.0) var = 0.0;
    const float muf = (float)mu, is = (float)(1.0 / sqrt(var + (double)eps));
    const float lo = (ext[0] - muf) * is, hi = (ext[1] - muf) * is;
    const float gm = gamma[ch], b = beta[ch];
    const float f_lo = lo * gm + b, f_hi = hi * gm + b;
    bound = relu ? fmaxf(0.f, fmaxf(f_lo, f_hi)) : fmaxf(fabsf(f_lo), fabsf(f_hi));
    mean[g * C + ch] = muf;
    invstd[g * C + ch] = is;
    xhat_amax[g * C + ch] = fmaxf(fabsf(lo), fabsf(hi));
    if (rmean && (split <= 0 || g == run_group)) {
      const double unbiased = count > 1.0 ? var * count / (count - 1.0) : var;
      rmean[ch] = (1.f - momentum) * rmean[ch] + momentum * muf;
      rvar[ch] = (1.f - momentum) * rvar[ch] + momentum * (float)unbiased;
    }
  }
  if (res_amax != nullptr) bound += amax_read(res_amax);
  bound *= 1.0000005f;
  __shared__ float red[4];
  float m = wave_max(bound);
  if ((threadIdx.x & 63) == 0) red[threadIdx.x >> 6] = m;
  __syncthreads();
  if (threadIdx.x == 0) {
    m = fmaxf(fmaxf(red[0], red[1]), fmaxf(red[2], red[3]));
    if (m > 0.f)
      atomicMax(reinterpret_cast<unsigned*>(out_amax) + ((bx + 7 * g) & (ONDA_AMAX_SLOTS - 1)) * AMAX_STRIDE, __float_as_uint(m));
  }
}
__global__ __launch_bounds__(256) void bn_finalize_l2_kernel(const BnFinalizeArgs a) { bn_finalize_block(a, blockIdx.x, blockIdx.y); }

template <bool FUSED>
__global__ __launch_bounds__(256) void bn_apply_l2_kernel(const float* __restrict__ x, const float* mean, const float* invstd,
                                                          const float* __restrict__ gamma, const float* __restrict__ beta,
                                                          const _Float16* __restrict__ res, size_t res_plane,
                                                          const float* __restrict__ res_amax, _Float16* __restrict__ out,
                                                          size_t out_plane, const float* out_amax, size_t total8, int C, int relu,
                                                          unsigned char* __restrict__ mask, size_t group1_at, const BnFinalizeArgs fin,
                                                          int nfin) {
  if constexpr (FUSED) {
    const int nb = (C + 15) / 16;
    if ((int)blockIdx.x < nfin) {
      bn_finalize_block(fin, blockIdx.x % nb, blockIdx.x / nb);
      grid_publish(fin.out_amax);
    }
    grid_wait(fin.out_amax, nfin);
  }
  const int c8 = C / 8;
  const float so = scale_of(out_amax).s;
  const float ri = res ? scale_of(res_amax).inv : 0.f;
  const size_t e0 = (size_t)blockIdx.x * blockDim.x + threadIdx.x;
  const int col = (int)(e0 % c8) * 8;
  const f32x4 ga0 = LD4(gamma + col), ga1 = LD4(gamma + col + 4);
  const f32x4 sc0 = LD4(invstd + col) * ga0, sc1 = LD4(invstd + col + 4) * ga1;
  const f32x4 mu0 = LD4(mean + col), mu1 = LD4(mean + col + 4), be0 = LD4(beta + col), be1 = LD4(beta + col + 4);
  const int g1 = group1_at > 0 ? C : 0;
  const f32x4 tc0 = LD4(invstd + g1 + col) * ga0, tc1 = LD4(invstd + g1 + col + 4) * ga1;
  const f32x4 nu0 = LD4(mean + g1 + col), nu1 = LD4(mean + g1 + col + 4);
  const size_t stride = (size_t)gridDim.x * blockDim.x;
  const size_t lcol = limb_at(0, col, C);
  auto lofs = [&](size_t e) { return (size_t)((unsigned)e / (unsigned)c8) * 2 * (size_t)C + lcol; };
  auto one = [&](size_t e, f32x4 x0, f32x4 x1, u32x4 r1, u32x4 r2, bool whole) {
    const bool second = group1_at > 0 && e >= group1_at;
    f32x4 v0 = (x0 - (second ? nu0 : mu0)) * (second ? tc0 : sc0) + be0, v1 = (x1 - (second ? nu1 : mu1)) * (second ? tc1 : sc1) + be1;
    if (res) {
      f32x4 q0, q1;
      join8(r1, r2, q0, q1);
      v0 += q0 * ri;
      v1 += q1 * ri;
    }
    if (mask) {
      unsigned bits = 0;
#pragma unroll
      for (int j = 0; j < 4; ++j) bits |= (v0[j] > 0.f ? 1u << j : 0u) | (v1[j] > 0.f ? 16u << j : 0u);
      mask[e] = (unsigned char)bits;
    }
    if (relu) {
#pragma unroll
      for (int j = 0; j < 4; ++j) {
        v0[j] = fmaxf(v0[j], 0.f);
        v1[j] = fmaxf(v1[j], 0.f);
      }
    }
    u32x4 l1, l2;
    split8(v0 * so, v1 * so, l1, l2);
    store_limb_lines(out + lofs(e), l1, l2, whole);
  };
  size_t e = e0;
  for (; e + stride < total8; e += 2 * stride) {
    const size_t f = e + stride;
    const f32x4 a0 = LD4S(x + e * 8), a1 = LD4S(x + e * 8 + 4), b0 = LD4S(x + f * 8), b1 = LD4S(x + f * 8 + 4);
    u32x4 ra1 = {}, ra2 = {}, rb1 = {}, rb2 = {};
    if (res) {
      ra1 = ld_stream(reinterpret_cast<const u32x4*>(res + lofs(e)));
      ra2 = ld_stream(reinterpret_cast<const u32x4*>(res + lofs(e) + LIMB2_OFS));
      rb1 = ld_stream(reinterpret_cast<const u32x4*>(res + lofs(f)));
      rb2 = ld_stream(reinterpret_cast<const u32x4*>(res + lofs(f) + LIMB2_OFS));
    }
    const bool whole = __ballot(1) == ~0ull;
    one(e, a0, a1, ra1, ra2, whole);
    one(f, b0, b1, rb1, rb2, whole);
  }
  if (e < total8) {
    u32x4 r1 = {}, r2 = {};
    if (res) {
      r1 = *reinterpret_cast<const u32x4*>(res + lofs(e));
      r2 = *reinterpret_cast<const u32x4*>(res + lofs(e) + LIMB2_OFS);
    }
    one(e, LD4(x + e * 8), LD4(x + e * 8 + 4), r1, r2, __ballot(1) == ~0ull);
  }
}

struct ColPlan3 {
  int cx, ry, gridx, chunks;
  int64_t rows_per_chunk;
};
static inline ColPlan3 col_plan3(int64_t M, int C) {
  ColPlan3 p;
  const int c4 = C / 4;
  p.cx = 1;
  while (p.cx < c4 && p.cx < 64) p.cx <<= 1;
  p.ry = 256 / p.cx;
  p.gridx = (c4 + p.cx - 1) / p.cx;
  int64_t target = 2048 / p.gridx;
  if (target < 1) target = 1;
  int64_t rpc = (M + target - 1) / target;
  const int64_t min_rows = (int64_t)p.ry * 8;
  if (rpc < min_rows) rpc = min_rows;
  p.rows_per_chunk = rpc;
  p.chunks = (int)((M + rpc - 1) / rpc);
  return p;
}

__device__ __forceinline__ f32x4 relu_mask4(const _Float16* __restrict__ out, const unsigned char* __restrict__ mask, size_t o, f32x4 g,
                                            int C) {
  if (mask != nullptr) {
    const unsigned bits = (unsigned)mask[o >> 3] >> ((o & 4) ? 4 : 0);
#pragma unroll
    for (int j = 0; j < 4; ++j) g[j] = (bits >> j) & 1u ? g[j] : 0.f;
    return g;
  }
  const unsigned orow = (unsigned)(o / (unsigned)C);
  const u32x2 h1 = *reinterpret_cast<const u32x2*>(out + limb_at(orow, (int)(o - (size_t)orow * C), C));
#pragma unroll
  for (int j = 0; j < 2; ++j) {
    const f32x2 a = unpack2h(h1[j]);
    g[2 * j] = a[0] > 0.f ? g[2 * j] : 0.f;
    g[2 * j + 1] = a[1] > 0.f ? g[2 * j + 1] : 0.f;
  }
  return g;
}

__global__ __launch_bounds__(256) void bn_bwd_reduce_l2_kernel(const float* __restrict__ dout, const _Float16* __restrict__ out,
                                                               size_t out_plane, const float* __restrict__ x,
                                                               const float* __restrict__ mean, const float* __restrict__ invstd,
                                                               float* __restrict__ dres, int64_t M, int C, int relu, int cx,
                                                               int64_t rows_per_chunk, float* __restrict__ partials,
                                                               const unsigned char* __restrict__ mask, int64_t split, int chunks0) {
  __shared__ f32x4 red[3][256];
  const int t = threadIdx.x;
  const int ry_n = 256 / cx;
  const int tx = t % cx, ty = t / cx;
  const int col = (blockIdx.x * cx + tx) * 4;
  const int chunk = blockIdx.y;
  const bool second = split > 0 && chunk >= chunks0;
  const int64_t r0 = second ? split + (int64_t)(chunk - chunks0) * rows_per_chunk : (int64_t)chunk * rows_per_chunk;
  const int64_t r1 = min(split > 0 && !second ? split : M, r0 + rows_per_chunk);
  f32x4 s1 = {0.f, 0.f, 0.f, 0.f}, s2 = {0.f, 0.f, 0.f, 0.f}, s3 = {0.f, 0.f, 0.f, 0.f};
  if (col < C) {
    const int gofs = second ? C : 0;
    const f32x4 mu = LD4(mean + gofs + col), is = LD4(invstd + gofs + col);
    for (int64_t r = r0 + ty; r < r1; r += ry_n) {
      const size_t o = (size_t)r * C + col;
      f32x4 g = LD4(dout + o);
      if (relu) g = relu_mask4(out, mask, o, g, C);
      if (dres) *reinterpret_cast<f32x4*>(dres + o) = g;
      const f32x4 xh = (LD4(x + o) - mu) * is;
      s1 += g;
      s2 += g * xh;
#pragma unroll
      for (int j = 0; j < 4; ++j) s3[j] = fmaxf(s3[j], fabsf(g[j]));
    }
  }
  red[0][t] = s1;
  red[1][t] = s2;
  red[2][t] = s3;
  __syncthreads();
  if (ty == 0 && col < C) {
    for (int y = 1; y < ry_n; ++y) {
      s1 += red[0][y * cx + tx];
      s2 += red[1][y * cx + tx];
      const f32x4 o3 = red[2][y * cx + tx];
#pragma unroll
      for (int j = 0; j < 4; ++j) s3[j] = fmaxf(s3[j], o3[j]);
    }
    float* dst = partials + ((size_t)chunk * 3) * C + col;
    *reinterpret_cast<f32x4*>(dst) = s1;
    *reinterpret_cast<f32x4*>(dst + C) = s2;
    *reinterpret_cast<f32x4*>(dst + 2 * C) = s3;
  }
}

struct BnBwdSumsArgs {
  const float* partials;
  int chunks, C;
  double inv_m0, inv_m1;
  const float *gamma, *invstd, *xhat_amax;
  float *sums, *dx_amax;
  int chunks0, groups;
};
__device__ __forceinline__ void bn_bwd_sums_block(const BnBwdSumsArgs& a, const int bx, const int g) {
  const int C = a.C;
  const int row0 = g == 0 ? 0 : a.chunks0, nrows = a.groups == 1 ? a.chunks : (g == 0 ? a.chunks0 : a.chunks - a.chunks0);
  const double inv_m = g == 0 ? a.inv_m0 : a.inv_m1;
  double sum[2];
  float ext[1];
  reduce_rows16<3, 2, false>(a.partials + (size_t)row0 * 3 * C, nrows, C, bx * 16, sum, ext);
  const int ch = bx * 16 + threadIdx.x;
  float bound = 0.f;
  if (threadIdx.x < 16 && ch < C) {
    a.sums[g * 2 * C + ch] = (float)sum[0];
    a.sums[g * 2 * C + C + ch] = (float)sum[1];
    bound = fabsf(a.gamma[ch] * a.invstd[g * C + ch]) *
            (ext[0] + (float)(fabs(sum[0]) * inv_m) + a.xhat_amax[g * C + ch] * (float)(fabs(sum[1]) * inv_m));
  }
  bound *= 1.000001f;
  __shared__ float red[4];
  float m = wave_max(bound);
  if ((threadIdx.x & 63) == 0) red[threadIdx.x >> 6] = m;
  __syncthreads();
  if (threadIdx.x == 0) {
    m = fmaxf(fmaxf(red[0], red[1]), fmaxf(red[2], red[3]));
    if (m > 0.f)
      atomicMax(reinterpret_cast<unsigned*>(a.dx_amax) + ((bx + 7 * g) & (ONDA_AMAX_SLOTS - 1)) * AMAX_STRIDE, __float_as_uint(m));
  }
}
__global__ __launch_bounds__(256) void bn_bwd_sums_l2_kernel(const BnBwdSumsArgs a) { bn_bwd_sums_block(a, blockIdx.x, blockIdx.y); }

template <bool FUSED>
__global__ __launch_bounds__(256) void bn_bwd_apply_l2_kernel(const float* __restrict__ dout, const _Float16* __restrict__ out,
                                                              size_t out_plane, const float* __restrict__ x,
                                                              const float* __restrict__ mean, const float* __restrict__ invstd,
                                                              const float* __restrict__ gamma, const float* sums,
                                                              _Float16* __restrict__ dx, size_t dx_plane, const float* dx_amax,
                                                              size_t total8, int C, float inv_m, int relu,
                                                              const unsigned char* __restrict__ mask, size_t group1_at, float inv_m1,
                                                              const BnBwdSumsArgs fin, int nfin) {
  if constexpr (FUSED) {
    const int nb = (C + 15) / 16;
    if ((int)blockIdx.x < nfin) {
      bn_bwd_sums_block(fin, blockIdx.x % nb, blockIdx.x / nb);
      grid_publish(fin.dx_amax);
    }
    grid_wait(fin.dx_amax, nfin);
  }
  const int c8 = C / 8;
  const float sd = scale_of(dx_amax).s;
  const size_t e0 = (size_t)blockIdx.x * blockDim.x + threadIdx.x;
  const int col = (int)(e0 % c8) * 8;
  f32x4 is[2][2], mu[2][2], gi[2][2], m1[2][2], m2[2][2];
#pragma unroll
  for (int g = 0; g < 2; ++g) {
    const int go = g && group1_at > 0 ? C : 0;
    const float im = g && group1_at > 0 ? inv_m1 : inv_m;
#pragma unroll
    for (int h = 0; h < 2; ++h) {
      const int cc = col + 4 * h;
      is[g][h] = LD4(invstd + go + cc);
      mu[g][h] = LD4(mean + go + cc);
      gi[g][h] = LD4(gamma + cc) * is[g][h];
      m1[g][h] = LD4(sums + 2 * go + cc) * im;
      m2[g][h] = LD4(sums + 2 * go + C + cc) * im;
    }
  }
  for (size_t e = e0; e < total8; e += (size_t)gridDim.x * blockDim.x) {
    const bool second = group1_at > 0 && e >= group1_at;
    f32x4 v[2];
#pragma unroll
    for (int h = 0; h < 2; ++h) {
      const size_t o = e * 8 + 4 * h;
      f32x4 g = LD4S(dout + o);
      if (relu) g = relu_mask4(out, mask, o, g, C);
      const f32x4 xh = (LD4S(x + o) - (second ? mu[1][h] : mu[0][h])) * (second ? is[1][h] : is[0][h]);
      v[h] = (second ? gi[1][h] : gi[0][h]) * (g - (second ? m1[1][h] : m1[0][h]) - xh * (second ? m2[1][h] : m2[0][h]));
    }
    u32x4 l1, l2;
    split8(v[0] * sd, v[1] * sd, l1, l2);
    store_limb_lines(dx + (size_t)((unsigned)e / (unsigned)c8) * 2 * (size_t)C + limb_at(0, col, C), l1, l2, __ballot(1) == ~0ull);
  }
}

__global__ __launch_bounds__(256) void chan_scale_limbs_kernel(const float* __restrict__ x, const float* __restrict__ gate,
                                                               _Float16* __restrict__ out, size_t plane,
                                                               const float* __restrict__ amax, int64_t HW, int C, size_t total8) {
  const int c8 = C / 8;
  const float so = scale_of(amax).s;
  for (size_t e = (size_t)blockIdx.x * blockDim.x + threadIdx.x; e < total8; e += (size_t)gridDim.x * blockDim.x) {
    const int col = (int)(e % c8) * 8;
    const size_t b = (e / c8) / HW;
    const f32x4 v0 = LD4S(x + e * 8) * LD4(gate + b * C + col), v1 = LD4S(x + e * 8 + 4) * LD4(gate + b * C + col + 4);
    u32x4 l1, l2;
    split8(v0 * so, v1 * so, l1, l2);
    _Float16* o = out + (size_t)((unsigned)e / (unsigned)c8) * 2 * (size_t)C + limb_at(0, col, C);
    st_stream(reinterpret_cast<u32x4*>(o), l1);
    st_stream(reinterpret_cast<u32x4*>(o + LIMB2_OFS), l2);
  }
}

static inline unsigned ew_grid(size_t total) {
  size_t g = (total + 255) / 256;
#ifndef ONDA_EW_GRID_CAP
#define ONDA_EW_GRID_CAP 4096
#endif
  if (g > ONDA_EW_GRID_CAP) g = ONDA_EW_GRID_CAP;
  if (g < 1) g = 1;
  return (unsigned)g;
}

}

extern "C" {

static BnFinalizeArgs finalize_args(const float* partials, int tiles, int C, int64_t count, float eps, float* mean, float* invstd,
                                    float* running_mean, float* running_var, int64_t* nbt, float momentum, const float* gamma,
                                    const float* beta, const float* res_amax, int relu, float* xhat_amax, float* out_amax,
                                    int64_t split, int tile_rows, int run_group, const float* y, int ldy) {
  return BnFinalizeArgs{partials, tiles, C, (double)count, eps, mean, invstd, running_mean, running_var, nbt, momentum, gamma, beta,
                        res_amax, relu, xhat_amax, out_amax, (long long)split, tile_rows > 0 ? tile_rows : 1, run_group, y, ldy};
}

int onda_bn_finalize_l2(const float* partials, int tiles, int C, int64_t count, float eps, float* mean, float* invstd,
                        float* running_mean, float* running_var, int64_t* nbt, float momentum, const float* gamma,
                        const float* beta, const float* res_amax, int relu, float* xhat_amax, float* out_amax, int64_t split,
                        int tile_rows, int run_group, const float* y, int ldy, onda_stream_t s) {
  ONDA_REQUIRE(partials && mean && invstd && gamma && beta && xhat_amax && out_amax && tiles >= 1 && C >= 4 && C % 4 == 0 && count >= 1);
  ONDA_REQUIRE(split >= 0 && split < count && (split == 0 || (tile_rows > 0 && y && ldy >= C && split / tile_rows < tiles)));
  if (!ONDA_ALIGNED16(partials)) return ONDA_EALIGN;
  hipLaunchKernelGGL(bn_finalize_l2_kernel, dim3((C + 15) / 16, split > 0 ? 2 : 1), dim3(256), 0, ONDA_STREAM(s),
                     finalize_args(partials, tiles, C, count, eps, mean, invstd, running_mean, running_var, nbt, momentum, gamma, beta,
                                   res_amax, relu, xhat_amax, out_amax, split, tile_rows, run_group, y, ldy));
  return ONDA_LAUNCH_RESULT();
}

int onda_chan_scale_limbs(const float* x, const float* gate, void* out, int64_t out_plane, const float* x_amax, int B, int64_t HW,
                          int C, onda_stream_t s) {
  ONDA_REQUIRE(x && gate && out && x_amax && C % 32 == 0 && B > 0 && HW > 0);
  (void)out_plane;
  if (!ONDA_ALIGNED16(x) || !ONDA_ALIGNED16(out) || !ONDA_ALIGNED16(gate)) return ONDA_EALIGN;
  const size_t total8 = (size_t)B * HW * C / 8;
  hipLaunchKernelGGL(chan_scale_limbs_kernel, dim3(ew_grid(total8)), dim3(256), 0, ONDA_STREAM(s), x, gate,
                     static_cast<_Float16*>(out), (size_t)out_plane, x_amax, HW, C, total8);
  return ONDA_LAUNCH_RESULT();
}

int onda_bn_apply_l2(const float* x, const float* mean, const float* invstd, const float* gamma, const float* beta,
                     const void* res, int64_t res_plane, const float* res_amax, void* out, int64_t out_plane,
                     const float* out_amax, int64_t M, int C, int relu, uint8_t* relu_mask, int64_t split, onda_stream_t s) {
  ONDA_REQUIRE(x && mean && invstd && gamma && beta && out && out_amax && C % 32 == 0 && (!res || res_amax));
  ONDA_REQUIRE(256 % (C / 8) == 0 || (C / 8) % 256 == 0);
  ONDA_REQUIRE(split >= 0 && split < M);
  if (!ONDA_ALIGNED16(x) || !ONDA_ALIGNED16(out) || (res && !ONDA_ALIGNED16(res))) return ONDA_EALIGN;
  const size_t total8 = (size_t)M * C / 8;
  hipLaunchKernelGGL(bn_apply_l2_kernel<false>, dim3(ew_grid(total8)), dim3(256), 0, ONDA_STREAM(s), x, mean, invstd, gamma, beta,
                     static_cast<const _Float16*>(res), (size_t)res_plane, res_amax, static_cast<_Float16*>(out), (size_t)out_plane,
                     out_amax, total8, C, relu, relu_mask, (size_t)split * C / 8, BnFinalizeArgs{}, 0);
  return ONDA_LAUNCH_RESULT();
}

int onda_bn_train_l2(const float* x, const float* partials, int tiles, float eps, float* mean, float* invstd, float* running_mean,
                     float* running_var, int64_t* nbt, float momentum, const float* gamma, const float* beta, const void* res,
                     const float* res_amax, int relu, float* xhat_amax, void* out, float* out_amax, int64_t M, int C,
                     uint8_t* relu_mask, int64_t split, int tile_rows, int run_group, onda_stream_t s) {
  ONDA_REQUIRE(x && partials && mean && invstd && gamma && beta && xhat_amax && out && out_amax && tiles >= 1 && M >= 1);
  ONDA_REQUIRE(C % 32 == 0 && (!res || res_amax) && (256 % (C / 8) == 0 || (C / 8) % 256 == 0));
  ONDA_REQUIRE(split >= 0 && split < M && (split == 0 || (tile_rows > 0 && split / tile_rows < tiles)));
  if (!ONDA_ALIGNED16(x) || !ONDA_ALIGNED16(out) || (res && !ONDA_ALIGNED16(res)) || !ONDA_ALIGNED16(partials)) return ONDA_EALIGN;
  const size_t total8 = (size_t)M * C / 8;
  const int nfin = (C + 15) / 16 * (split > 0 ? 2 : 1);
  const unsigned grid = ew_grid(total8) > (unsigned)nfin ? ew_grid(total8) : (unsigned)nfin;
  hipLaunchKernelGGL(bn_apply_l2_kernel<true>, dim3(grid), dim3(256), 0, ONDA_STREAM(s), x, mean, invstd, gamma, beta,
                     static_cast<const _Float16*>(res), (size_t)0, res_amax, static_cast<_Float16*>(out), (size_t)0, out_amax, total8, C,
                     relu, relu_mask, (size_t)split * C / 8,
                     finalize_args(partials, tiles, C, M, eps, mean, invstd, running_mean, running_var, nbt, momentum, gamma, beta, res_amax,
                                   relu, xhat_amax, out_amax, split, tile_rows, run_group, x, C),
                     nfin);
  return ONDA_LAUNCH_RESULT();
}

static inline void bwd_chunks(const ColPlan3& p, int64_t M, int64_t split, int& chunks0, int& chunks) {
  if (split <= 0) {
    chunks0 = chunks = p.chunks;
    return;
  }
  chunks0 = (int)((split + p.rows_per_chunk - 1) / p.rows_per_chunk);
  chunks = chunks0 + (int)((M - split + p.rows_per_chunk - 1) / p.rows_per_chunk);
}

int64_t onda_bn_bwd_l2_ws(int64_t M, int C) {
  const ColPlan3 p = col_plan3(M, C);
  return (int64_t)(p.chunks + 1) * 3 * C + 4 * C;
}

int onda_bn_bwd_l2(const float* dout, const void* out, int64_t out_plane, const float* x, const float* mean, const float* invstd,
                   const float* gamma, const float* xhat_amax, void* dx, int64_t dx_plane, float* dx_amax, float* dres, float* ws,
                   int64_t M, int C, int relu, const uint8_t* relu_mask, int64_t split, int fuse_sums, onda_stream_t s) {
  ONDA_REQUIRE(dout && x && mean && invstd && gamma && xhat_amax && dx && dx_amax && ws && C % 32 == 0 && (!relu || out || relu_mask));
  ONDA_REQUIRE(256 % (C / 8) == 0 || (C / 8) % 256 == 0);
  ONDA_REQUIRE(split >= 0 && split < M);
  if (!ONDA_ALIGNED16(dout) || !ONDA_ALIGNED16(x) || !ONDA_ALIGNED16(dx) || (out && !ONDA_ALIGNED16(out))) return ONDA_EALIGN;
  const ColPlan3 p = col_plan3(M, C);
  int chunks0, chunks;
  bwd_chunks(p, M, split, chunks0, chunks);
  float* sums = ws + (size_t)(p.chunks + 1) * 3 * C;
  hipStream_t st = ONDA_STREAM(s);
  hipLaunchKernelGGL(bn_bwd_reduce_l2_kernel, dim3(p.gridx, chunks), dim3(256), 0, st, dout, static_cast<const _Float16*>(out),
                     (size_t)out_plane, x, mean, invstd, dres, M, C, relu, p.cx, p.rows_per_chunk, ws, relu_mask, split, chunks0);
  const double inv_m0 = 1.0 / (double)(split > 0 ? split : M), inv_m1 = 1.0 / (double)(M - split);
  const int groups = split > 0 ? 2 : 1;
  const BnBwdSumsArgs fin{ws, chunks, C, inv_m0, inv_m1, gamma, invstd, xhat_amax, sums, dx_amax, chunks0, groups};
  const size_t total8 = (size_t)M * C / 8;
  if (fuse_sums) {
    const int nfin = (C + 15) / 16 * groups;
    const unsigned grid = ew_grid(total8) > (unsigned)nfin ? ew_grid(total8) : (unsigned)nfin;
    hipLaunchKernelGGL(bn_bwd_apply_l2_kernel<true>, dim3(grid), dim3(256), 0, st, dout, static_cast<const _Float16*>(out),
                       (size_t)out_plane, x, mean, invstd, gamma, sums, static_cast<_Float16*>(dx), (size_t)dx_plane, dx_amax, total8, C,
                       (float)inv_m0, relu, relu_mask, (size_t)split * C / 8, (float)inv_m1, fin, nfin);
    return ONDA_LAUNCH_RESULT();
  }
  hipLaunchKernelGGL(bn_bwd_sums_l2_kernel, dim3((C + 15) / 16, groups), dim3(256), 0, st, fin);
  hipLaunchKernelGGL(bn_bwd_apply_l2_kernel<false>, dim3(ew_grid(total8)), dim3(256), 0, st, dout, static_cast<const _Float16*>(out),
                     (size_t)out_plane, x, mean, invstd, gamma, sums, static_cast<_Float16*>(dx), (size_t)dx_plane, dx_amax, total8,
                     C, (float)inv_m0, relu, relu_mask, (size_t)split * C / 8, (float)inv_m1, BnBwdSumsArgs{}, 0);
  return ONDA_LAUNCH_RESULT();
}

}
```

onda_amd/framework/model/deeplabv2.py:

```python
import os

import torch
import torch.nn as nn

from onda_amd import ops

affine_par = True


class HipConv2d(nn.Conv2d):

    def __init__(self, *args, **kwargs):
        super().__init__(*args, **kwargs)
        self._pack = ops._PackCache()

    def geom(self):
        return self.kernel_size[0], self.stride[0], self.dilation[0], self.padding[0]

    def forward(self, x, want_stats=False, cout_pad=None):
        k, stride, dil, pad = self.geom()
        return ops.Conv2dFn.apply(x, self.weight, self.bias, self._pack, stride, dil, pad, want_stats, cout_pad)


class HipBatchNorm2d(nn.BatchNorm2d):

    def folded(self):
        key = tuple((t.data_ptr(), t._version) for t in (self.weight, self.bias, self.running_mean, self.running_var))
        if getattr(self, "_fold_key", None) != key:
            self._fold = ops.bn_eval_fold(self.weight, self.bias, self.running_mean, self.running_var)
            self._fold_key = key
        return self._fold

    def __deepcopy__(self, memo):
        self.__dict__.pop("_bound_cache", None)
        fold = self.__dict__.pop("_fold", None), self.__dict__.pop("_fold_key", None)
        cls = self.__class__
        new = cls.__new__(cls)
        memo[id(self)] = new
        from copy import deepcopy
        for k, v in self.__dict__.items():
            new.__dict__[k] = deepcopy(v, memo)
        if fold[0] is not None:
            self._fold, self._fold_key = fold
        return new




def conv_bn(conv, bn, x, relu, residual=None):
    k, stride, dil, pad = conv.geom()
    if bn.training:
        limbs = ops.limb_mode(conv.out_channels)
        y, stats = conv(x, want_stats=4 if limbs else True)
        running = (bn.running_mean, bn.running_var, bn.num_batches_tracked) if bn.track_running_stats else None
        if bn.momentum is None:
            raise NotImplementedError("onda_amd: cumulative-average BatchNorm (momentum=None) is not on the hot path")
        fn = ops.BNTrainLimbFn if stats.shape[1] == 4 else ops.BNTrainFn
        return fn.apply(y, stats, bn.weight, bn.bias, residual, relu, running, bn.momentum)
    scale, shift = bn.folded()
    with torch.no_grad():
        wp = conv._pack.get_fwd(conv.weight)
        limb_out = None
        if ops.limb_mode(conv.out_channels) and ops._use_l2(wp, x.shape[3]):
            w = conv.weight
            key = (w.data_ptr(), w._version, id(scale), id(shift))
            hit = getattr(bn, "_bound_cache", None)
            if hit is None or hit[0] != key:
                hit = bn._bound_cache = (key, ops.fold_bounds(w, scale, shift), scale, shift)
            limb_out = hit[1]
        y, _, _ = ops.conv_forward(x, wp, k, stride, dil, pad, conv.out_channels, scale=scale, shift=shift, residual=residual,
                                   relu=relu, limb_out=limb_out)
    return y


class Bottleneck(nn.Module):
    expansion = 4

    def __init__(self, inplanes, planes, stride=1, dilation=1, downsample=None, norm_module=HipBatchNorm2d,
                 norm_grad=False):
        super().__init__()
        self.conv1 = HipConv2d(inplanes, planes, kernel_size=1, stride=stride, bias=False)
        self.bn1 = norm_module(planes, affine=affine_par)
        self.conv2 = HipConv2d(planes, planes, kernel_size=3, stride=1, padding=dilation, bias=False,
                               dilation=dilation)
        self.bn2 = norm_module(planes, affine=affine_par)
        self.conv3 = HipConv2d(planes, planes * 4, kernel_size=1, bias=False)
        self.bn3 = norm_module(planes * 4, affine=affine_par)
        if not norm_grad:
            for bn in (self.bn1, self.bn2, self.bn3):
                for p in bn.parameters():
                    p.requires_grad = False
        self.relu = nn.ReLU(inplace=True)
        self.downsample = downsample
        self.stride = stride

    def forward(self, x):
        ops.share_grad(x)
        y = conv_bn(self.conv1, self.bn1, x, True)
        y = conv_bn(self.conv2, self.bn2, y, True)
        if self.downsample is not None:
            residual = conv_bn(self.downsample[0], self.downsample[1], x, False)
        else:
            residual = x
        return conv_bn(self.conv3, self.bn3, y, True, residual)


class SEBlock(nn.Module):
    def __init__(self, inplanes, r=16):
        super().__init__()
        self.global_pool = nn.AdaptiveAvgPool2d((1, 1))
        self.se = nn.Sequential(nn.Linear(inplanes, inplanes // r), nn.ReLU(inplace=True),
                                nn.Linear(inplanes // r, inplanes), nn.Sigmoid())

    def forward(self, x):
        return ops.SEScaleFn.apply(x, self.se[0].weight, self.se[0].bias, self.se[2].weight, self.se[2].bias)


_rank_generators = {}


def _default_drop_mask(batch, channels, p, device):
    from onda_amd import dist as odist
    gen = None
    if odist.is_on():
        key = str(device)
        gen = _rank_generators.get(key)
        if gen is None:
            gen = _rank_generators[key] = torch.Generator(device=device)
            gen.manual_seed(torch.initial_seed() + odist.seed_offset())
    return torch.empty(batch, channels, 1, 1, device=device).bernoulli_(1 - p, generator=gen).div_(1 - p)


drop_mask_fn = _default_drop_mask

_forced_masks = []


def force_mask(mask):
    _forced_masks.append(mask)


def draw_mask(model, batch, device):
    head = model.layer6.head[0]
    if not (head.training and head.p > 0):
        return None
    return drop_mask_fn(batch, 256, head.p, device).reshape(batch, 256).contiguous()


class Classifier_Module2(nn.Module):

    def __init__(self, inplanes, dilation_series, padding_series, num_classes, droprate=0.1, use_se=True):
        super().__init__()
        self.num_classes = num_classes
        self.conv2d_list = nn.ModuleList()
        self.conv2d_list.append(nn.Sequential(
            HipConv2d(inplanes, 256, kernel_size=1, stride=1, padding=0, dilation=1, bias=True),
            nn.GroupNorm(num_groups=32, num_channels=256, affine=True), nn.ReLU(inplace=True)))
        for dilation, padding in zip(dilation_series, padding_series):
            self.conv2d_list.append(nn.Sequential(
                HipConv2d(inplanes, 256, kernel_size=3, stride=1, padding=padding, dilation=dilation, bias=True),
                nn.GroupNorm(num_groups=32, num_channels=256, affine=True), nn.ReLU(inplace=True)))
        mods = [SEBlock(256 * (len(dilation_series) + 1))] if use_se else []
        mods += [HipConv2d(256 * (len(dilation_series) + 1), 256, kernel_size=3, stride=1, padding=1, dilation=1,
                           bias=True),
                 nn.GroupNorm(num_groups=32, num_channels=256, affine=True)]
        self.bottleneck = nn.Sequential(*mods)
        self.head = nn.Sequential(nn.Dropout2d(droprate),
                                  HipConv2d(256, num_classes, kernel_size=1, padding=0, dilation=1, bias=False))
        for m in self.bottleneck:
            if isinstance(m, nn.Conv2d):
                nn.init.kaiming_normal_(m.weight.data, a=0, mode="fan_in")
                m.bias.data.zero_()
            elif isinstance(m, nn.GroupNorm):
                m.weight.data.fill_(1)
                m.bias.data.zero_()
        for m in self.head:
            if isinstance(m, nn.Conv2d):
                m.weight.data.normal_(0, 0.001)

    def forward(self, x, get_feat=False):
        ys, gammas, betas = [], [], []
        ops.share_grad(x)
        for seq in self.conv2d_list:
            y, _ = seq[0](x)
            ys.append(y)
            gammas.append(seq[1].weight)
            betas.append(seq[1].bias)
        y = ops.GNConcatFn.apply(True, None, *ys, *gammas, *betas)
        rest = list(self.bottleneck)
        if isinstance(rest[0], SEBlock):
            y = rest[0](y)
            rest = rest[1:]
        y, _ = rest[0](y)
        drop = self.head[0]
        chmul = None
        if drop.training and drop.p > 0:
            if _forced_masks:
                chmul = _forced_masks.pop(0)
            else:
                chmul = drop_mask_fn(y.shape[0], y.shape[3], drop.p, y.device).reshape(y.shape[0], y.shape[3]).contiguous()
        feat = ops.GNConcatFn.apply(False, chmul, y, rest[1].weight, rest[1].bias)
        out_pad, _ = self.head[1](feat, cout_pad=ops.HEAD_PAD)
        out = ops.ClassSliceFn.apply(out_pad, self.num_classes)
        if get_feat:
            return {"feat": feat.permute(0, 3, 1, 2), "out": out}
        return out


class ResNetMulti(nn.Module):
    def __init__(self, block, layers, num_classes, multi_level, classifier_module="normal",
                 norm_module=HipBatchNorm2d, norm_grad=False):
        if classifier_module != "ProDA":
            raise NotImplementedError("onda_amd implements the ProDA classifier head (MODEL.CLASSIFIER: 'ProDA'), the one "
                                      "the hybrid_switch / static_model configs use")
        self.multi_level = multi_level
        self.feat = True
        self.inplanes = 64
        super().__init__()
        self.conv1 = HipConv2d(3, 64, kernel_size=7, stride=2, padding=3, bias=False)
        self.bn1 = norm_module(64, affine=affine_par)
        if not norm_grad:
            for p in self.bn1.parameters():
                p.requires_grad = False
        self.relu = nn.ReLU(inplace=True)
        self.maxpool = nn.MaxPool2d(kernel_size=3, stride=2, padding=1, ceil_mode=True)
        self.layer1 = self._make_layer(block, 64, layers[0], norm_module=norm_module, norm_grad=norm_grad)
        self.layer2 = self._make_layer(block, 128, layers[1], stride=2, norm_module=norm_module, norm_grad=norm_grad)
        self.layer3 = self._make_layer(block, 256, layers[2], stride=1, dilation=2, norm_module=norm_module,
                                       norm_grad=norm_grad)
        self.layer4 = self._make_layer(block, 512, layers[3], stride=1, dilation=4, norm_module=norm_module,
                                       norm_grad=norm_grad)
        if self.multi_level:
            self.layer5 = Classifier_Module2(1024, [6, 12, 18, 24], [6, 12, 18, 24], num_classes)
        self.layer6 = Classifier_Module2(2048, [6, 12, 18, 24], [6, 12, 18, 24], num_classes)
        for m in self.modules():
            if isinstance(m, nn.Conv2d):
                m.weight.data.normal_(0, 0.01)
            elif isinstance(m, nn.BatchNorm2d):
                m.weight.data.fill_(1)
                m.bias.data.zero_()

    def _make_layer(self, block, planes, blocks, stride=1, dilation=1, norm_module=HipBatchNorm2d, norm_grad=False):
        downsample = None
        if stride != 1 or self.inplanes != planes * block.expansion or dilation in (2, 4):
            downsample = nn.Sequential(
                HipConv2d(self.inplanes, planes * block.expansion, kernel_size=1, stride=stride, bias=False),
                norm_module(planes * block.expansion, affine=affine_par))
            if not norm_grad:
                for p in downsample[1].parameters():
                    p.requires_grad = False
        layers = [block(self.inplanes, planes, stride, dilation=dilation, downsample=downsample)]
        self.inplanes = planes * block.expansion
        for _ in range(1, blocks):
            layers.append(block(self.inplanes, planes, dilation=dilation))
        return nn.Sequential(*layers)

    def __deepcopy__(self, memo):
        packer = self.__dict__.pop("_packer", None)
        sync = self.__dict__.pop("_onda_grad_sync", None)
        try:
            cls = self.__class__
            new = cls.__new__(cls)
            memo[id(self)] = new
            from copy import deepcopy
            for k, v in self.__dict__.items():
                new.__dict__[k] = deepcopy(v, memo)
        finally:
            if packer is not None:
                self.__dict__["_packer"] = packer
            if sync is not None:
                self.__dict__["_onda_grad_sync"] = sync
        return new

    def _stem(self, x):
        bn = self.bn1
        if bn.training:
            return self._stem_train(x, self._running(bn))
        return ops.MaxPoolFn.apply(ops.stem_eval(x, self.conv1.weight, self.conv1._pack, *bn.folded()), True)

    @staticmethod
    def _running(bn):
        return (bn.running_mean, bn.running_var, bn.num_batches_tracked) if bn.track_running_stats else None

    def _stem_train(self, x, running):
        bn = self.bn1
        y, stats = ops.StemConvFn.apply(x, self.conv1.weight, self.conv1._pack, True)
        y = ops.BNTrainFn.apply(y, stats, bn.weight, bn.bias, None, True, running, bn.momentum)
        return ops.MaxPoolFn.apply(y, True)

    def forward(self, x):
        if x.dim() != 4 or x.shape[1] != 3:
            raise ValueError(f"expected an image batch f32[B,3,H,W], got {tuple(x.shape)}")
        ops._require_cuda(x, "image batch")
        x = x.to(torch.float32)
        packer = self.__dict__.get("_packer")
        if packer is None:
            plain = [m for name, m in self.named_modules() if isinstance(m, HipConv2d) and m is not self.conv1
                     and not name.endswith("head.1") and (self.multi_level or not name.startswith("layer5."))]
            packer = self.__dict__["_packer"] = ops.ModelPacker(plain)
        packer.refresh(need_dgrad=torch.is_grad_enabled() and self.training)
        y = self._stem(x)
        y = self.layer1(y)
        y = self.layer2(y)
        y = self.layer3(y)
        x1 = self.layer5(y, True) if self.multi_level else None
        y = self.layer4(y)
        x2 = self.layer6(y, True)
        return x1, x2

    def get_1x_lr_params_no_scale(self):
        for top in (self.conv1, self.bn1, self.layer1, self.layer2, self.layer3, self.layer4):
            for mod in top.modules():
                for p in mod.parameters():
                    if p.requires_grad:
                        yield p

    def get_10x_lr_params(self):
        groups = []
        if self.multi_level:
            groups.append(self.layer5.parameters())
        groups.append(self.layer6.parameters())
        for g in groups:
            for p in g:
                yield p

    def optim_parameters(self, lr):
        return [{"params": self.get_1x_lr_params_no_scale(), "lr": lr},
                {"params": self.get_10x_lr_params(), "lr": 10 * lr}]


def get_deeplab_v2(num_classes=19, multi_level=True, layers=[3, 4, 23, 3], classifier="normal",
                   norm_module=HipBatchNorm2d, norm_grad=False):
    if norm_module is nn.BatchNorm2d:
        norm_module = HipBatchNorm2d
    return ResNetMulti(Bottleneck, layers, num_classes, multi_level, classifier_module=classifier,
                       norm_module=norm_module, norm_grad=norm_grad)
```

onda_amd/ops/conv.py:

```python
import ctypes
from ctypes import byref

import torch

from .. import _lib
from .._lib import OndaLimbOut, call, query
from . import _state
from ._state import STEM_K
from .core import _conv_ws, _desc, _group_split, _l2_name, _launch, _p, _require_cuda, _stream, as_nhwc, conv_out_size, nhwc_ld
from .limbs import H2Weight, Limbs, amax_slot, is_limb_only, known_amax, limb_only, limbs_of, tag_amax
from .tables import _table


def _use_l2(wp, cin):
    return isinstance(wp, H2Weight) and _state.H2_PATH == "dma" and cin % 32 == 0


def _pack_h2(weight, rows_pad, kp, dgrad, cout_pad):
    cout, cin, kh, kw = weight.shape
    w = weight.detach().contiguous()
    slot = known_amax(weight)
    if slot is None:
        slot = amax_slot(weight.device, long_lived=True)
        call("onda_absmax", _p(w), 1, w.numel(), w.numel(), _p(slot), _stream())
# ... 175 lines not shown
        return dx
    if yamax is not None:
        raise RuntimeError("onda_amd: max|dx| from the data gradient's epilogue needs the pre-split path")
    if is_limb_only(dy):
        raise RuntimeError("onda_amd: a limb-only gradient reached a data-gradient kernel that does not take limb planes")
    if isinstance(wpd, H2Weight):
        raise RuntimeError("onda_amd: a pre-split weight reached a data gradient the pre-split kernels do not take (Cout % 32 != 0)")
    _launch("conv_fwd_kernel<128,%d>" % (128 if cin > 64 else 64), 2.0 * B * Ho * Wo * cin * k * k * Co, "onda_conv2d_fwd",
            _p(dy), _p(wpd), _p(dx), None, None, None, None, _p(_conv_ws(dy.device)), byref(d), _stream(),
            tag=("dgrad", B * Ho * Wo if stride != 1 else B * Hi * Wi, cin, Co, k, stride, dil))
    return dx


def _wgrad_splitk(M, cout, cin, taps, l2=False):
    if l2:
        tn = 256 if query("onda_conv_wgrad_l2_variant", cout, cin) == 0 else 128
        tiles = -(-cout // tn) * -(-cin // 128) * taps
        G = query("onda_conv_ws_floats") // (3 * 128 * 128) // (2 if tn == 256 else 1)
        return max(_best_splitk(M, cout, cin, taps, tiles, G, 3.2e14 if tn == 256 else 2.0e14), -(-M // 65536))
    t = 128 if (cout > 64 and cin > 64) else 64
    tiles = -(-cout // t) * -(-cin // t) * taps
    G = query("onda_conv_ws_floats") // (3 * 128 * 128) * (1 if t == 128 else 2)
    return _best_splitk(M, cout, cin, taps, tiles, G, 1.2e14)


def _best_splitk(M, cout, cin, taps, tiles, G, rate):
    t_ideal = 2.0 * M * cout * cin * taps / rate
    wbytes = 4.0 * cout * cin * taps
    best, best_t = 1, None
    for sk in range(1, 257):
        if sk > 1 and (M // sk < 256 or sk * wbytes > (512 << 20)):
            break
        blocks = tiles * sk
        eff = (blocks / G) / -(-blocks // G)
        est = t_ideal / eff + 2.0 * sk * wbytes / 3e12
        if best_t is None or est < best_t * 0.995:
            best, best_t = sk, est
    return best


_PIX_TABLES = {}


def _wgrad_pixel_table(d, device):
    stride = query("onda_conv2d_wgrad_l2_table_stride", byref(d))
    if stride == 0:
        return
    key = (str(device), d.Hi, d.Wi, d.Ho, d.Wo, d.kh, d.kw, d.stride, d.dil, d.pad)
    hit = _PIX_TABLES.get(key)
    cur = torch.cuda.current_stream(device)
    if hit is None or hit[1] < d.B:
        table = torch.empty(d.kh * d.kw * stride, device=device, dtype=torch.int32)
        call("onda_conv2d_wgrad_l2_table", byref(d), _p(table), cur.cuda_stream)
        done = torch.cuda.Event()
        done.record(cur)
        if hit is not None:
            hit[0].record_stream(cur)
        hit = _PIX_TABLES[key] = (table, d.B, stride, done, {cur.cuda_stream})
    elif cur.cuda_stream not in hit[4]:
        cur.wait_event(hit[3])
        hit[4].add(cur.cuda_stream)
    d.pix_table, d.pix_stride = hit[0].data_ptr(), hit[2]


def conv_wgrad(x, dy, k, stride, dil, pad, cout_real, cin_real, flat_k=0, into=None, xlimbs=None):
    B, Hi, Wi, Cin = x.shape
    _, Ho, Wo, Co = dy.shape
    taps = k * k
    M = B * Ho * Wo
    l2 = _state.CONV_MODE == "f16x2" and Cin % 32 == 0 and Co % 32 == 0
    sk = _wgrad_splitk(M, Co, Cin, taps, l2)
    slabs = torch.empty(sk, Co, taps, Cin, device=x.device, dtype=torch.float32)
    d = _desc(B, Hi, Wi, Cin, Ho, Wo, Co, k, stride, dil, pad, 0 if is_limb_only(x) else nhwc_ld(x), Co)
    if not l2 and (is_limb_only(x) or is_limb_only(dy)):
        raise RuntimeError("onda_amd: a limb-only tensor reached a weight-gradient kernel that does not take limb planes")
    if l2:
        xl = xlimbs if xlimbs is not None else limbs_of(x)
        dyl = limbs_of(dy)
        d.ldx = xl.ld
        _wgrad_pixel_table(d, x.device)
        _launch("conv_wgrad_l2_kernel<%d>" % query("onda_conv_wgrad_l2_variant", Co, Cin), 2.0 * M * Co * taps * Cin,
                "onda_conv2d_wgrad_l2", _p(xl.planes), xl.plane, _p(xl.amax), _p(dyl.planes), dyl.plane, _p(dyl.amax), _p(slabs),
                dyl.ld, sk, byref(d), _stream(), tag=("wgrad", M, Co, Cin, k, stride, dil, sk),
                issued=lambda: query("onda_conv_wgrad_l2_live_fraction", byref(d), sk))
    else:
        _launch("conv_wgrad_kernel<%s>" % ("128,128" if (Co > 64 and Cin > 64) else "64,64"), 2.0 * M * Co * taps * Cin,
                "onda_conv2d_wgrad", _p(x), _p(dy), _p(slabs), nhwc_ld(dy), sk, byref(d), _stream(),
                tag=("wgrad", M, Co, Cin, k, stride, dil, sk))
    return _wgrad_finish(slabs, into, sk, Co, taps, Cin, cout_real, cin_real, flat_k, k, x.device)


def _wgrad_finish(slabs, into, sk, Co, taps, Cin, cout_real, cin_real, flat_k, k, device):
    if into is not None:
        call("onda_wgrad_reduce", _p(slabs), _p(into), sk, Co, taps, Cin, cout_real, cin_real, flat_k, 1, _stream())
        return None
    if flat_k:
        dw = torch.empty(cout_real, cin_real, 7, 7, device=device, dtype=torch.float32)
    else:
        dw = torch.empty(cout_real, cin_real, k, k, device=device, dtype=torch.float32)
    call("onda_wgrad_reduce", _p(slabs), _p(dw), sk, Co, taps, Cin, cout_real, cin_real, flat_k, 0, _stream())
    return dw


def _accumulate_target(weight):
    g = weight.grad
    if g is not None and g.is_contiguous() and g.dtype == torch.float32 and g.shape == weight.shape:
        return g
    return None


def colsum(x, y=None, alpha=1.0, per_image=False):
    B, H, W, C = x.shape
    nb, hw = (B, H * W) if per_image else (1, B * H * W)
    ws = torch.empty(query("onda_colsum_ws", nb, hw, C), device=x.device, dtype=torch.float32)
    out = torch.empty(nb, C, device=x.device, dtype=torch.float32)
    call("onda_colsum", _p(x), nhwc_ld(x), _p(y), nhwc_ld(y) if y is not None else 0, _p(out), float(alpha), _p(ws),
         nb, hw, C, _stream())
    return out if per_image else out[0]


class _PackCache:

    def __init__(self):
        self.key_f = self.key_d = None
        self.fwd = self.dgrad = None

    @staticmethod
    def _key(w):
        return (w.data_ptr(), w._version, w.device, _state.CONV_MODE)

    def get_fwd(self, w, cout_pad=None, kp=None):
        k = self._key(w)
        if self.key_f != k:
            self.fwd, self.key_f = pack_weight_fwd(w, cout_pad, kp), k
        return self.fwd

    def get_dgrad(self, w, cout_pad=None):
        k = self._key(w)
        if self.key_d != k:
            self.dgrad, self.key_d = pack_weight_dgrad(w, cout_pad), k
        return self.dgrad

    def __deepcopy__(self, memo):
        return _PackCache()


class ModelPacker:

    def __init__(self, convs):
        self.convs = [c for c in convs if c.weight.shape[0] % 32 == 0 and c.weight.shape[1] % 32 == 0]
        self.bufs = {}

    def refresh(self, need_dgrad):
        if _state.CONV_MODE != "f16x2" or not self.convs:
            return
        stale = []
        for c in self.convs:
            w, cache = c.weight, c._pack
            key = _PackCache._key(w)
            if cache.key_f != key or (need_dgrad and cache.key_d != key):
                stale.append((c, key))
        if not stale:
            return
        dev = stale[0][0].weight.device
        ents, biggest = [], 0
        for c, key in stale:
            w = c.weight.detach()
            if not w.is_contiguous():
                w = w.contiguous()
            cout, cin, kh, kw = w.shape
            buf = self.bufs.get(id(c))
            if buf is None or buf[0].device != w.device:
                buf = self.bufs[id(c)] = (torch.empty(2, cout, kh * kw * cin, device=w.device, dtype=torch.float16),
                                          torch.empty(2, cin, kh * kw * cout, device=w.device, dtype=torch.float16))
            slot = amax_slot(w.device, long_lived=True)
            tag_amax(c.weight, slot)
            cache = c._pack
            cache.fwd, cache.key_f = H2Weight(buf[0], slot), key
            if need_dgrad:
                cache.dgrad, cache.key_d = H2Weight(buf[1], slot), key
            else:
                cache.key_d = None
            ents.append(_lib.OndaPackEntry(w.data_ptr(), buf[0].data_ptr(), buf[1].data_ptr() if need_dgrad else None, slot.data_ptr(),
                                           cout, cin, kh * kw, biggest))
            biggest += query("onda_pack_blocks", cout, cin, kh * kw)
            self._keep = getattr(self, "_keep", [])
            self._keep.append(w)
        table = _table(ents, _lib.OndaPackEntry, dev)
        call("onda_pack_weights_h2_multi", _p(table), len(ents), biggest, _stream())
        self._keep = []


class Conv2dFn(torch.autograd.Function):

    @staticmethod
    def forward(ctx, x, weight, bias, cache, stride, dil, pad, want_stats, cout_pad):
        cout, cin, k, _ = weight.shape
        co = cout_pad or cout
        wp = cache.get_fwd(weight, cout_pad)
        y, stats, _tiles = conv_forward(x, wp, k, stride, dil, pad, co, shift=_pad_vec(bias, co), want_stats=want_stats)
        ctx.save_for_backward(x, weight)
        hit = getattr(x, "_onda_limbs", None)
        ctx.xlimbs = hit[1] if hit is not None and hit[0] == x._version else None
        ctx.weight_param = weight
        ctx.sink = _sink_of(x) if ctx.needs_input_grad[0] else None
        ctx.cache, ctx.geom, ctx.has_bias = cache, (k, stride, dil, pad, cout, cin, cout_pad), bias is not None
        ctx.set_materialize_grads(False)
        if want_stats:
            ctx.mark_non_differentiable(stats)
            return y, stats
        return y, None

    @staticmethod
    def backward(ctx, dy, _dstats):
        if dy is None:
            return (None,) * 9
        x, weight = ctx.saved_tensors
        k, stride, dil, pad, cout, cin, cout_pad = ctx.geom
        if not is_limb_only(dy):
            dy = as_nhwc(dy)
        dx = dw = db = None
        if ctx.needs_input_grad[0]:
            sink = ctx.sink
            wpd = ctx.cache.get_dgrad(weight, cout_pad)
            if sink is not None and sink.buf is not None:
                conv_dgrad(dy, wpd, k, stride, dil, pad, cin, x.shape[1:3], accumulate=sink.buf)
                _sink_done(sink)
            else:
                dx = _sink_give(sink, conv_dgrad(dy, wpd, k, stride, dil, pad, cin, x.shape[1:3]), True)
        if ctx.needs_input_grad[1]:
            into = _accumulate_target(ctx.weight_param)
            dw = conv_wgrad(x, dy, k, stride, dil, pad, cout, cin, into=into, xlimbs=ctx.xlimbs)
            if into is not None and _state.GRAD_READY is not None:
                _state.GRAD_READY(ctx.weight_param)
        if ctx.has_bias and ctx.needs_input_grad[2]:
            db = colsum(dy)[:cout]
        return dx, dw, db, None, None, None, None, None, None


def _pad_vec(v, n):
    if v is None or v.numel() == n:
        return v
    out = torch.zeros(n, device=v.device, dtype=v.dtype)
    out[: v.numel()] = v.detach()
    return out


def stem_patches(x_nchw, Ho, Wo, l2):
    hit = getattr(x_nchw, "_onda_patches", None)
    key = (x_nchw._version, bool(l2), Ho, Wo)
    if hit is not None and hit[0] == key:
        return hit[1]
    B, _, H, W = x_nchw.shape
    dev = x_nchw.device
    if l2:
        amax = amax_slot(dev)
        call("onda_absmax", _p(x_nchw), 1, x_nchw.numel(), x_nchw.numel(), _p(amax), _stream())
        M = B * Ho * Wo
        planes = torch.empty(2, M, STEM_K, device=dev, dtype=torch.float16)
        call("onda_stem_im2col_l2", _p(x_nchw), _p(amax), _p(planes), M * STEM_K, B, H, W, Ho, Wo, STEM_K, _stream())
        col = limb_only((B, Ho, Wo, STEM_K), dev, Limbs(planes, amax, STEM_K, M * STEM_K))
    else:
        col = torch.empty(B, Ho, Wo, STEM_K, device=dev, dtype=torch.float32)
        call("onda_stem_im2col", _p(x_nchw), _p(col), B, H, W, Ho, Wo, STEM_K, _stream())
    try:
        x_nchw._onda_patches = (key, col)
    except AttributeError:
        pass
    return col


def stem_prefetch(x_nchw):
    B, _, H, W = x_nchw.shape
    l2 = _state.CONV_MODE == "f16x2" and _state.H2_PATH == "dma" and STEM_K % 32 == 0
    return stem_patches(x_nchw, conv_out_size(H, 7, 2, 1, 3), conv_out_size(W, 7, 2, 1, 3), l2)


class StemConvFn(torch.autograd.Function):

    @staticmethod
    def forward(ctx, x_nchw, weight, cache, want_stats):
        _require_cuda(x_nchw, "image")
        x_nchw = x_nchw.contiguous()
        B, _, H, W = x_nchw.shape
        Ho, Wo = conv_out_size(H, 7, 2, 1, 3), conv_out_size(W, 7, 2, 1, 3)
        wp = cache.get_fwd(weight, None, STEM_K)
        col = stem_patches(x_nchw, Ho, Wo, _use_l2(wp, STEM_K))
        y, stats, _ = conv_forward(col, wp, 1, 1, 1, 0, weight.shape[0], want_stats=want_stats)
        ctx.save_for_backward(col)
        ctx.col_limbs = limbs_of(col) if is_limb_only(col) else None
        ctx.cout, ctx.weight = weight.shape[0], weight
        ctx.set_materialize_grads(False)
        if want_stats:
            ctx.mark_non_differentiable(stats)
            return y, stats
        return y, None

    @staticmethod
    def backward(ctx, dy, _dstats):
        if dy is None:
            return None, None, None, None
        (col,) = ctx.saved_tensors
        into = _accumulate_target(ctx.weight)
        dw = conv_wgrad(col, as_nhwc(dy), 1, 1, 1, 0, ctx.cout, 3, flat_k=49, into=into, xlimbs=ctx.col_limbs)
        if into is not None and _state.GRAD_READY is not None:
            _state.GRAD_READY(ctx.weight)
        return None, dw, None, None


def stem_eval(x_nchw, weight, cache, scale, shift):
    _require_cuda(x_nchw, "image")
    with torch.no_grad():
        x_nchw = x_nchw.contiguous()
        B, _, H, W = x_nchw.shape
        Ho, Wo = conv_out_size(H, 7, 2, 1, 3), conv_out_size(W, 7, 2, 1, 3)
        wp = cache.get_fwd(weight, None, STEM_K)
        col = stem_patches(x_nchw, Ho, Wo, _use_l2(wp, STEM_K))
        y, _, _ = conv_forward(col, wp, 1, 1, 1, 0, weight.shape[0], scale=scale, shift=shift, relu=True)
    return y
```

onda_amd/ops/norm.py:

```python
import ctypes
import os
from ctypes import byref

import torch

from .. import _lib
from .._lib import OndaConv, OndaLimbOut, call, query
from . import _state
from ._state import BN_EPS, GN_EPS, GN_GROUPS, HEAD_PAD, STEM_K
from .core import _group_split, _p, _stream, as_nhwc, nhwc_ld
from .limbs import Limbs, _stat_tile_rows, amax_slot, is_limb_only, known_amax, limb_mode, limb_only, limbs_of, tag_amax
from .conv import _sink_give, _sink_of, colsum


class BNTrainFn(torch.autograd.Function):

    @staticmethod
    def _groups(B, H, W):
        split, M = _group_split(B, H, W), B * H * W
        return [(0, M)] if not split else [(0, split), (split, M - split)]

    @staticmethod
    def forward(ctx, y, stats, gamma, beta, residual, relu, running, momentum):
        B, H, W, C = y.shape
        groups = BNTrainFn._groups(B, H, W)
        G = len(groups)
        mean = torch.empty(G, C, device=y.device, dtype=torch.float32)
        invstd = torch.empty_like(mean)
        out = torch.empty_like(y)
        res = as_nhwc(residual) if residual is not None else None
        if res is not None and nhwc_ld(res) != C:
            res = res.contiguous()
        if G > 1 and (nhwc_ld(y) != C or not y.is_contiguous()):
            raise RuntimeError("onda_amd: row groups need a dense conv output")
        amax = amax_slot(y.device) if _state.CONV_MODE == "f16x2" else None
        for g, (r0, rows) in enumerate(groups):
            part, nrows = stats, stats.shape[0]
            if G > 1:
                bm = _stat_tile_rows(stats)
                if groups[1][0] % bm == 0 and stats.shape[1] == 2:
                    ts = groups[1][0] // bm
                    part = stats[:ts] if g == 0 else stats[ts:]
                    nrows = part.shape[0]
                else:
                    part = torch.empty(query("onda_bn_bwd_ws", rows, C), device=y.device, dtype=torch.float32)
                    n = ctypes.c_int(0)
                    call("onda_bn_stats", y.data_ptr() + 4 * r0 * C, rows, C, C, _p(part), byref(n), _stream())
                    nrows = n.value
            run = running if (running is not None and g == G - 1) else None
            rm, rv, nbt = run if run is not None else (None, None, None)
            call("onda_bn_finalize", _p(part), nrows, C, rows, BN_EPS, _p(mean[g]), _p(invstd[g]), _p(rm), _p(rv), _p(nbt),
                 float(momentum), _stream())
            off = 4 * r0 * C
            call("onda_bn_apply", y.data_ptr() + off, _p(mean[g]), _p(invstd[g]), _p(gamma), _p(beta),
                 res.data_ptr() + off if res is not None else None, out.data_ptr() + off, rows, C, int(relu), _p(amax), _stream())
        if running is not None:
            for t in running:
                torch.autograd.graph.increment_version(t)
        if amax is not None:
            tag_amax(out, amax)
        ctx.save_for_backward(y, out if relu else None, mean, invstd, gamma)
        ctx.relu, ctx.has_res, ctx.groups = relu, residual is not None, groups
        ctx.res_sink = _sink_of(residual) if (residual is not None and ctx.needs_input_grad[4]) else None
        return out

    @staticmethod
    def backward(ctx, dout):
        y, out, mean, invstd, gamma = ctx.saved_tensors
        B, H, W, C = y.shape
        dout = dout.contiguous()
        dx = torch.empty_like(y)
        amax = amax_slot(y.device) if _state.CONV_MODE == "f16x2" else None
        need_res = ctx.has_res and ctx.needs_input_grad[4]
        dres = None
        if need_res:
            dres = torch.empty_like(y) if ctx.relu else dout
        for g, (r0, rows) in enumerate(ctx.groups):
            ws = torch.empty(query("onda_bn_bwd_ws", rows, C), device=y.device, dtype=torch.float32)
            off = 4 * r0 * C
            call("onda_bn_bwd", dout.data_ptr() + off, out.data_ptr() + off if out is not None else None, y.data_ptr() + off,
                 _p(mean[g]), _p(invstd[g]), _p(gamma), dx.data_ptr() + off,
                 dres.data_ptr() + off if (need_res and ctx.relu) else None, _p(ws), rows, C, int(ctx.relu), _p(amax), _stream())
        if amax is not None:
            tag_amax(dx, amax)
        if need_res:
            dres = _sink_give(ctx.res_sink, dres, ctx.relu)
        return dx, None, None, None, dres, None, None, None






class BNTrainLimbFn(torch.autograd.Function):

    @staticmethod
    def forward(ctx, y, stats, gamma, beta, residual, relu, running, momentum):
        B, H, W, C = y.shape
        M = B * H * W
        dev = y.device
        split = _group_split(B, H, W)
        mean = torch.empty((2 if split else 1) * C, device=dev, dtype=torch.float32)
        invstd = torch.empty_like(mean)
        xhat_amax = torch.empty_like(mean)
        rm, rv, nbt = running if running is not None else (None, None, None)
        res = limbs_of(residual) if residual is not None else None
        if res is not None and (res.ld != C or tuple(residual.shape) != (B, H, W, C)):
            raise RuntimeError("onda_amd: residual of a BatchNorm must be a dense [B,H,W,C] activation")
        out_amax = amax_slot(dev)
        tile_rows = _stat_tile_rows(stats) if split else 0
        planes = torch.empty(2, M, C, device=dev, dtype=torch.float16)
        mask = torch.empty(M * C // 8, device=dev, dtype=torch.uint8) if relu and any(ctx.needs_input_grad) else None
        if _state.FUSE_BN_FINALIZE and nhwc_ld(y) == C:
            call("onda_bn_train_l2", _p(y), _p(stats), stats.shape[0], BN_EPS, _p(mean), _p(invstd), _p(rm), _p(rv), _p(nbt),
                 float(momentum), _p(gamma), _p(beta), _p(res.planes) if res is not None else None,
                 _p(res.amax) if res is not None else None, int(relu), _p(xhat_amax), _p(planes), _p(out_amax), M, C, _p(mask),
                 split, tile_rows, 1, _stream())
        else:
            call("onda_bn_finalize_l2", _p(stats), stats.shape[0], C, M, BN_EPS, _p(mean), _p(invstd), _p(rm), _p(rv), _p(nbt),
                 float(momentum), _p(gamma), _p(beta), _p(res.amax) if res is not None else None, int(relu), _p(xhat_amax),
                 _p(out_amax), split, tile_rows, 1, _p(y) if split else None, nhwc_ld(y) if split else 0, _stream())
            call("onda_bn_apply_l2", _p(y), _p(mean), _p(invstd), _p(gamma), _p(beta), _p(res.planes) if res is not None else None,
                 res.plane if res is not None else 0, _p(res.amax) if res is not None else None, _p(planes), M * C, _p(out_amax),
                 M, C, int(relu), _p(mask), split, _stream())
        if running is not None:
            for t in running:
                torch.autograd.graph.increment_version(t)
        lb = Limbs(planes, out_amax, C, M * C)
        ctx.split = split
        ctx.save_for_backward(y, mean, invstd, gamma, xhat_amax)
        ctx.out_limbs = lb if relu and mask is None else None
        ctx.relu_mask = mask
        ctx.relu, ctx.has_res = relu, residual is not None
        ctx.res_sink = _sink_of(residual) if (residual is not None and ctx.needs_input_grad[4]) else None
        return limb_only((B, H, W, C), dev, lb)

    @staticmethod
    def backward(ctx, dout):
        y, mean, invstd, gamma, xhat_amax = ctx.saved_tensors
        B, H, W, C = y.shape
        M = B * H * W
        dev = y.device
        if is_limb_only(dout):
            raise RuntimeError("onda_amd: the gradient of a BatchNorm output must be an fp32 tensor")
        dout = dout.contiguous()
        ws = torch.empty(query("onda_bn_bwd_l2_ws", M, C), device=dev, dtype=torch.float32)
        planes = torch.empty(2, M, C, device=dev, dtype=torch.float16)
        dx_amax = amax_slot(dev)
        need_res = ctx.has_res and ctx.needs_input_grad[4]
        dres = None
        if need_res:
            dres = torch.empty_like(y) if ctx.relu else dout
        ol = ctx.out_limbs
        call("onda_bn_bwd_l2", _p(dout), _p(ol.planes) if ol is not None else None, ol.plane if ol is not None else 0, _p(y),
             _p(mean), _p(invstd), _p(gamma), _p(xhat_amax), _p(planes), M * C, _p(dx_amax),
             _p(dres) if (need_res and ctx.relu) else None, _p(ws), M, C, int(ctx.relu), _p(ctx.relu_mask), ctx.split,
             int(_state.FUSE_BN_FINALIZE), _stream())
        dx = limb_only((B, H, W, C), dev, Limbs(planes, dx_amax, C, M * C))
        if need_res:
            dres = _sink_give(ctx.res_sink, dres, ctx.relu)
        return dx, None, None, None, dres, None, None, None


def fold_bounds(weight, scale, shift):
    with torch.no_grad():
        l1 = weight.detach().abs().sum(dim=(1, 2, 3))
        return torch.stack([(scale.abs() * l1).max(), shift.abs().max()]).float().contiguous()


def bn_eval_fold(gamma, beta, rm, rv):
    C = gamma.numel()
    scale = torch.empty(C, device=gamma.device, dtype=torch.float32)
    shift = torch.empty_like(scale)
    call("onda_bn_fold", _p(gamma), _p(beta), _p(rm), _p(rv), BN_EPS, _p(scale), _p(shift), C, _stream())
    return scale, shift


class MaxPoolFn(torch.autograd.Function):
    @staticmethod
    def forward(ctx, x, limbs=False):
        B, Hi, Wi, C = x.shape
        Ho, Wo = -(-(Hi - 1) // 2) + 1, -(-(Wi - 1) // 2) + 1
        if (Ho - 1) * 2 - 1 >= Hi:
            Ho -= 1
        if (Wo - 1) * 2 - 1 >= Wi:
            Wo -= 1
        idx = torch.empty(B, Ho, Wo, C, device=x.device, dtype=torch.uint8)
        x = x.contiguous()
        slot = known_amax(x)
        ctx.save_for_backward(idx)
        ctx.in_shape = (B, Hi, Wi, C)
        if limbs and slot is not None and limb_mode(C):
            planes = torch.empty(2, B * Ho * Wo, C, device=x.device, dtype=torch.float16)
            call("onda_maxpool_fwd_limbs", _p(x), _p(slot), _p(planes), _p(idx), B, Hi, Wi, C, Ho, Wo, _stream())
            return limb_only((B, Ho, Wo, C), x.device, Limbs(planes, slot, C, B * Ho * Wo * C))
        y = torch.empty(B, Ho, Wo, C, device=x.device, dtype=torch.float32)
        call("onda_maxpool_fwd", _p(x), _p(y), _p(idx), B, Hi, Wi, C, Ho, Wo, _stream())
        if slot is not None:
            tag_amax(y, slot)
        return y

    @staticmethod
    def backward(ctx, dy):
        (idx,) = ctx.saved_tensors
        B, Hi, Wi, C = ctx.in_shape
        dy = dy.contiguous()
        dx = torch.empty(B, Hi, Wi, C, device=dy.device, dtype=torch.float32)
        call("onda_maxpool_bwd", _p(dy), _p(idx), _p(dx), B, Hi, Wi, C, dy.shape[1], dy.shape[2], _stream())
        return dx, None


class GNConcatFn(torch.autograd.Function):

    @staticmethod
    def forward(ctx, relu, chmul, *args):
        n = len(args) // 3
        ys, gammas, betas = args[:n], args[n:2 * n], args[2 * n:]
        B, H, W, C = ys[0].shape
        HW = H * W
        cat = torch.empty(B, H, W, C * n, device=ys[0].device, dtype=torch.float32)
        ws = torch.empty(query("onda_gn_ws", B, HW, C), device=cat.device, dtype=torch.float32)
        amax = amax_slot(cat.device) if _state.CONV_MODE == "f16x2" else None
        means, rstds = [], []
        for i in range(n):
            mean = torch.empty(B * GN_GROUPS, device=cat.device, dtype=torch.float32)
            rstd = torch.empty_like(mean)
            sl = cat[..., i * C:(i + 1) * C]
            call("onda_gn_fwd", _p(ys[i]), nhwc_ld(ys[i]), _p(gammas[i]), _p(betas[i]), _p(chmul), _p(sl), C * n,
                 _p(mean), _p(rstd), _p(ws), B, HW, C, GN_GROUPS, GN_EPS, int(relu), _p(amax), _stream())
            means.append(mean)
            rstds.append(rstd)
        if amax is not None:
            tag_amax(cat, amax)
        ctx.save_for_backward(cat, chmul, *ys, *gammas, *means, *rstds)
        ctx.n, ctx.relu = n, relu
        return cat

    @staticmethod
    def backward(ctx, dcat):
        n = ctx.n
        saved = ctx.saved_tensors
        cat, chmul = saved[0], saved[1]
        ys, gammas = saved[2:2 + n], saved[2 + n:2 + 2 * n]
        means, rstds = saved[2 + 2 * n:2 + 3 * n], saved[2 + 3 * n:2 + 4 * n]
        B, H, W, C = ys[0].shape
        HW = H * W
        dcat = as_nhwc(dcat)
        ldd = nhwc_ld(dcat)
        ws = torch.empty(query("onda_gn_ws", B, HW, C), device=cat.device, dtype=torch.float32)
        dys, dgs, dbs = [], [], []
        for i in range(n):
            dx = torch.empty(B, H, W, C, device=cat.device, dtype=torch.float32)
            dg = torch.empty(C, device=cat.device, dtype=torch.float32)
            db = torch.empty_like(dg)
            call("onda_gn_bwd", dcat.data_ptr() + 4 * i * C, ldd, cat.data_ptr() + 4 * i * C, C * n, _p(ys[i]),
                 nhwc_ld(ys[i]), _p(gammas[i]), _p(chmul), _p(means[i]), _p(rstds[i]), _p(dx), _p(dg), _p(db), _p(ws),
                 B, HW, C, GN_GROUPS, int(ctx.relu), _stream())
            dys.append(dx)
            dgs.append(dg)
            dbs.append(db)
        return (None, None, *dys, *dgs, *dbs)




class SEScaleFn(torch.autograd.Function):

    @staticmethod
    def forward(ctx, x, w1, b1, w2, b2):
        B, H, W, C = x.shape
        R = w1.shape[0]
        pooled = colsum(x, alpha=1.0 / (H * W), per_image=True)
        hidden = torch.empty(B, R, device=x.device, dtype=torch.float32)
        gate = torch.empty(B, C, device=x.device, dtype=torch.float32)
        call("onda_se_fc_fwd", _p(pooled), _p(w1), _p(b1), _p(w2), _p(b2), _p(hidden), _p(gate), B, C, R, _stream())
        slot = known_amax(x)
        if slot is not None and limb_mode(C) and x.is_contiguous():
            planes = torch.empty(2, B * H * W, C, device=x.device, dtype=torch.float16)
            call("onda_chan_scale_limbs", _p(x), _p(gate), _p(planes), B * H * W * C, _p(slot), B, H * W, C, _stream())
            out = limb_only((B, H, W, C), x.device, Limbs(planes, slot, C, B * H * W * C))
        else:
            out = torch.empty_like(x)
            call("onda_chan_scale", _p(x), _p(gate), None, _p(out), B, H * W, C, _stream())
        ctx.save_for_backward(x, pooled, hidden, gate, w1, w2)
        return out

    @staticmethod
    def backward(ctx, dout):
        x, pooled, hidden, gate, w1, w2 = ctx.saved_tensors
        B, H, W, C = x.shape
        R = w1.shape[0]
        dout = dout.contiguous()
        dgate = colsum(dout, x, per_image=True)
        dw1, db1 = torch.empty_like(w1), torch.empty(R, device=x.device, dtype=torch.float32)
        dw2, db2 = torch.empty_like(w2), torch.empty(C, device=x.device, dtype=torch.float32)
        dpooled = torch.empty(B, C, device=x.device, dtype=torch.float32)
        ws = torch.empty(B * R, device=x.device, dtype=torch.float32)
        call("onda_se_fc_bwd", _p(dgate), _p(pooled), _p(hidden), _p(gate), _p(w1), _p(w2), _p(dw1), _p(db1), _p(dw2),
             _p(db2), _p(dpooled), _p(ws), 1.0 / (H * W), B, C, R, _stream())
        dx = torch.empty_like(x)
        call("onda_chan_scale", _p(dout), _p(gate), _p(dpooled), _p(dx), B, H * W, C, _stream())
        return dx, dw1, db1, dw2, db2
```

Measured before the change: 42.81 images/s.

## Fuse stem BatchNorm, ReLU and maxpool forward/backward; tile stem im2col in shared memory

Adds fused kernels that apply the stem BatchNorm, ReLU and 3x3/2 maxpool in one pass, writing limb planes and argmax indices directly. A matching backward recomputes the pre-pool values from y and folds the maxpool scatter into the BN-backward reduce and apply. This avoids materializing the full-resolution BN output and its gradient. Separately, the stem im2col now stages an input strip in shared memory and uses cooperative limb stores, and the BN finalize straddle-row reduction is parallelized across the block. The cost is more complex index recomputation inside the fused kernels.

```diff
diff --git a/include/onda_hip.h b/include/onda_hip.h
--- a/include/onda_hip.h
+++ b/include/onda_hip.h
@@ -103,6 +103,12 @@
 int onda_bn_bwd_l2(const float* dout, const void* out, int64_t out_plane, const float* x, const float* mean, const float* invstd,
                    const float* gamma, const float* xhat_amax, void* dx, int64_t dx_plane, float* dx_amax, float* dres, float* ws,
                    int64_t M, int C, int relu, const uint8_t* relu_mask, int64_t split, int fuse_sums, onda_stream_t s);
+int onda_bn_relu_maxpool_l2(const float* y, const float* mean, const float* invstd, const float* gamma, const float* beta, void* out,
+                            const float* out_amax, uint8_t* idx, int B, int Hi, int Wi, int C, int Ho, int Wo, int first_images,
+                            onda_stream_t s);
+int onda_bn_relu_maxpool_bwd_l2(const float* dy, const uint8_t* idx, const float* y, const float* mean, const float* invstd,
+                                const float* gamma, const float* beta, const float* xhat_amax, void* dx, float* dx_amax, float* ws,
+                                int B, int Hi, int Wi, int C, int Ho, int Wo, int first_images, onda_stream_t s);
 
 int onda_conv_wgrad_l2_variant(int Cout, int Cin);
 int64_t onda_conv2d_wgrad_l2_table_stride(const OndaConv* c);
diff --git a/onda_amd/_lib.py b/onda_amd/_lib.py
--- a/onda_amd/_lib.py
+++ b/onda_amd/_lib.py
@@ -76,6 +76,8 @@
     "onda_bn_bwd_l2_ws": (L, [L, I]),
     "onda_bn_train_l2": (I, [P, P, I, F, P, P, P, P, P, F, P, P, P, P, I, P, P, P, L, I, P, L, I, I, P]),
     "onda_bn_bwd_l2": (I, [P, P, L, P, P, P, P, P, P, L, P, P, P, L, I, I, P, L, I, P]),
+    "onda_bn_relu_maxpool_l2": (I, [P, P, P, P, P, P, P, P, I, I, I, I, I, I, I, P]),
+    "onda_bn_relu_maxpool_bwd_l2": (I, [P, P, P, P, P, P, P, P, P, P, P, I, I, I, I, I, I, I, P]),
     "onda_conv2d_wgrad": (I, [P, P, P, I, I, POINTER(OndaConv), P]),
     "onda_wgrad_reduce": (I, [P, P, I, I, I, I, I, I, I, I, P]),
     "onda_pack_weight_fwd": (I, [P, P, I, I, I, I, I, P]),
diff --git a/onda_amd/csrc/common.h b/onda_amd/csrc/common.h
--- a/onda_amd/csrc/common.h
+++ b/onda_amd/csrc/common.h
@@ -15,6 +15,28 @@
 constexpr int LIMB2_OFS = 32;
 __host__ __device__ __forceinline__ size_t limb_at(size_t row, int c, int ld) {
   return row * 2 * (size_t)ld + (size_t)((c >> 5) << 6) + (size_t)(c & 31);
+}
+
+typedef unsigned int onda_u32x4 __attribute__((ext_vector_type(4)));
+__device__ __forceinline__ void store_limb_lines(_Float16* o, onda_u32x4 l1, onda_u32x4 l2, bool whole) {
+  if (!whole) {
+    *reinterpret_cast<onda_u32x4*>(o) = l1;
+    *reinterpret_cast<onda_u32x4*>(o + LIMB2_OFS) = l2;
+    return;
+  }
+  const bool hi = (threadIdx.x & 4) != 0;
+  const onda_u32x4 send = hi ? l1 : l2;
+  onda_u32x4 recv;
+#pragma unroll
+  for (int j = 0; j < 4; ++j) recv[j] = (unsigned)__shfl_xor((int)send[j], 4, 64);
+  const unsigned long long mine = reinterpret_cast<unsigned long long>(o);
+  const unsigned long long partner = ((unsigned long long)(unsigned)__shfl_xor((int)(mine >> 32), 4, 64) << 32) |
+                                     (unsigned)__shfl_xor((int)(unsigned)mine, 4, 64);
+  _Float16* po = reinterpret_cast<_Float16*>(partner);
+  _Float16* a1 = hi ? po + LIMB2_OFS : o;
+  _Float16* a2 = hi ? o + LIMB2_OFS : po;
+  *reinterpret_cast<onda_u32x4*>(a1) = hi ? recv : l1;
+  *reinterpret_cast<onda_u32x4*>(a2) = hi ? l2 : recv;
 }
 
 #define ONDA_STREAM(s) (reinterpret_cast<hipStream_t>(s))
diff --git a/onda_amd/csrc/conv_l2.hip b/onda_amd/csrc/conv_l2.hip
--- a/onda_amd/csrc/conv_l2.hip
+++ b/onda_amd/csrc/conv_l2.hip
@@ -105,42 +105,52 @@
   }
 }
 
-__global__ __launch_bounds__(256) void stem_im2col_l2_kernel(const float* __restrict__ x, _Float16* __restrict__ dst,
-                                                             long long plane, int B, int H, int W, int Ho, int Wo, int Kp,
-                                                             const float* __restrict__ amax) {
+constexpr int STEM_WT = 64, STEM_NC = 2 * STEM_WT + 5, STEM_KP_MAX = 256;
+__global__ __launch_bounds__(256) void stem_im2col_l2_kernel(const float* __restrict__ x, _Float16* __restrict__ dst, int H, int W,
+                                                             int Ho, int Wo, int Kp, int strips, const float* __restrict__ amax) {
+  __shared__ unsigned tile[21 * STEM_NC];
+  __shared__ short ofs[STEM_KP_MAX];
   const float sc = scale_of(amax).s;
-  const int k8 = Kp >> 3;
-  const long long n = (long long)B * Ho * Wo * k8;
-  for (long long e = (long long)blockIdx.x * 256 + threadIdx.x; e < n; e += (long long)gridDim.x * 256) {
-    const long long m = e / k8;
-    const int k0 = (int)(e - m * k8) * 8;
-    const int wo = (int)(m % Wo);
-    const long long tq = m / Wo;
-    const int ho = (int)(tq % Ho), b = (int)(tq / Ho);
-    float v[8];
-#pragma unroll
-    for (int j = 0; j < 8; ++j) {
-      const int k = k0 + j;
-      float val = 0.f;
-      if (k < 147) {
-        const int tap = k / 3, cc = k - tap * 3;
-        const int r = tap / 7, t7 = tap - r * 7;
-        const int hi = ho * 2 - 3 + r, wi = wo * 2 - 3 + t7;
-        if ((unsigned)hi < (unsigned)H && (unsigned)wi < (unsigned)W) val = x[(((size_t)b * 3 + cc) * H + hi) * W + wi];
-      }
-      v[j] = val * sc;
+  const int strip = (int)(blockIdx.x % (unsigned)strips), bh = (int)(blockIdx.x / (unsigned)strips);
+  const int ho = bh % Ho, b = bh / Ho;
+  const int wo0 = strip * STEM_WT, npx = min(STEM_WT, Wo - wo0);
+  for (int k = threadIdx.x; k < Kp; k += 256) {
+    const int tap = k / 3, cc = k - tap * 3, r = tap / 7, t7 = tap - r * 7;
+    ofs[k] = k < 147 ? (short)((cc * 7 + r) * STEM_NC + t7) : (short)-1;
+  }
+  for (int i = threadIdx.x; i < 21 * STEM_NC; i += 256) {
+    const int row = i / STEM_NC, ci = i - row * STEM_NC;
+    const int cc = row / 7, r = row - cc * 7;
+    const int hi = ho * 2 - 3 + r, wi = wo0 * 2 - 3 + ci;
+    float val = 0.f;
+    if (ci < 2 * npx + 5 && (unsigned)hi < (unsigned)H && (unsigned)wi < (unsigned)W) val = x[(((size_t)b * 3 + cc) * H + hi) * W + wi];
+    const float v = val * sc;
+    const _Float16 h1 = (_Float16)v;
+    const _Float16 h2 = (_Float16)((v - (float)h1) * LIMB2_SCALE);
+    tile[i] = (unsigned)__builtin_bit_cast(unsigned short, h1) | ((unsigned)__builtin_bit_cast(unsigned short, h2) << 16);
+  }
+  __syncthreads();
+  const int k8 = Kp >> 3, nitems = npx * k8;
+  _Float16* base = dst + ((size_t)bh * Wo + wo0) * 2 * (size_t)Kp;
+  for (int i0 = 0; i0 < nitems; i0 += 256) {
+    const int it = i0 + threadIdx.x;
+    const bool valid = it < nitems;
+    const bool whole = __ballot(valid) == ~0ull;
+    if (!valid) continue;
+    const int p = it / k8, j = it - p * k8;
+    unsigned w[8];
+#pragma unroll
+    for (int jj = 0; jj < 8; ++jj) {
+      const int o = ofs[j * 8 + jj];
+      w[jj] = o < 0 ? 0u : tile[o + 2 * p];
     }
     u32x4 l1, l2;
 #pragma unroll
     for (int h = 0; h < 4; ++h) {
-      const unsigned pk = cvt2h(v[2 * h], v[2 * h + 1]);
-      const f32x2 f = unpack2h(pk);
-      l1[h] = pk;
-      l2[h] = cvt2h((v[2 * h] - f[0]) * LIMB2_SCALE, (v[2 * h + 1] - f[1]) * LIMB2_SCALE);
-    }
-    _Float16* o = dst + limb_at((size_t)m, k0, Kp);
-    *reinterpret_cast<u32x4*>(o) = l1;
-    *reinterpret_cast<u32x4*>(o + LIMB2_OFS) = l2;
+      l1[h] = (w[2 * h] & 0xffffu) | (w[2 * h + 1] << 16);
+      l2[h] = (w[2 * h] >> 16) | (w[2 * h + 1] & 0xffff0000u);
+    }
+    store_limb_lines(base + (size_t)p * 2 * Kp + (j >> 2) * 64 + (j & 3) * 8, l1, l2, whole);
   }
 }
 
@@ -1935,10 +1945,10 @@
   (void)plane;
   ONDA_REQUIRE(x_nchw && xamax && dst && Kp % 32 == 0 && Kp >= 147 && B > 0 && Ho > 0 && Wo > 0);
   if (!ONDA_ALIGNED16(dst)) return ONDA_EALIGN;
-  const long long n = (long long)B * Ho * Wo * (Kp / 8);
-  const int blocks = (int)(n / 256 / 2 + 1 > 4096 ? 4096 : n / 256 / 2 + 1);
-  hipLaunchKernelGGL(stem_im2col_l2_kernel, dim3(blocks), dim3(256), 0, ONDA_STREAM(s), x_nchw, static_cast<_Float16*>(dst),
-                     (long long)plane, B, H, W, Ho, Wo, Kp, xamax);
+  const int strips = (Wo + STEM_WT - 1) / STEM_WT;
+  ONDA_REQUIRE(Kp <= STEM_KP_MAX && H > 0 && W > 0 && (long long)B * Ho * strips < (1ll << 31));
+  hipLaunchKernelGGL(stem_im2col_l2_kernel, dim3((unsigned)(B * Ho * strips)), dim3(256), 0, ONDA_STREAM(s), x_nchw,
+                     static_cast<_Float16*>(dst), H, W, Ho, Wo, Kp, strips, xamax);
   return ONDA_LAUNCH_RESULT();
 }
 
diff --git a/onda_amd/csrc/norm_l2.hip b/onda_amd/csrc/norm_l2.hip
--- a/onda_amd/csrc/norm_l2.hip
+++ b/onda_amd/csrc/norm_l2.hip
@@ -55,27 +55,6 @@
 }
 
 #define LD4(p) (*reinterpret_cast<const f32x4*>(p))
-
-__device__ __forceinline__ void store_limb_lines(_Float16* o, u32x4 l1, u32x4 l2, bool whole) {
-  if (!whole) {
-    *reinterpret_cast<u32x4*>(o) = l1;
-    *reinterpret_cast<u32x4*>(o + LIMB2_OFS) = l2;
-    return;
-  }
-  const bool hi = (threadIdx.x & 4) != 0;
-  const u32x4 send = hi ? l1 : l2;
-  u32x4 recv;
-#pragma unroll
-  for (int j = 0; j < 4; ++j) recv[j] = (unsigned)__shfl_xor((int)send[j], 4, 64);
-  const unsigned long long mine = reinterpret_cast<unsigned long long>(o);
-  const unsigned long long partner = ((unsigned long long)(unsigned)__shfl_xor((int)(mine >> 32), 4, 64) << 32) |
-                                     (unsigned)__shfl_xor((int)(unsigned)mine, 4, 64);
-  _Float16* po = reinterpret_cast<_Float16*>(partner);
-  _Float16* a1 = hi ? po + LIMB2_OFS : o;
-  _Float16* a2 = hi ? o + LIMB2_OFS : po;
-  *reinterpret_cast<u32x4*>(a1) = hi ? recv : l1;
-  *reinterpret_cast<u32x4*>(a2) = hi ? l2 : recv;
-}
 
 #ifndef ONDA_NT_BN
 #define ONDA_NT_BN 0
@@ -213,37 +192,76 @@
   const float* __restrict__ y = a.y;
   const long long split = a.split;
   if (bx == 0 && g == 0 && threadIdx.x == 0 && nbt) *nbt += 1;
+  const bool straddle = split > 0 && split % bm != 0;
   int row0 = 0, nrows = tiles;
   if (split > 0) {
     const int ts = (int)(split / bm);
-    if (g == 0) nrows = ts; else row0 = ts, nrows = tiles - ts;
+    if (g == 0) nrows = ts; else row0 = ts + (straddle ? 1 : 0), nrows = tiles - row0;
     count = g == 0 ? (double)split : count - (double)split;
+  }
+  __shared__ double ysum[4][2][16];
+  __shared__ float yext[4][2][16];
+  const int yq = threadIdx.x & 3, ycol = bx * 16 + 4 * yq;
+  f32x4 yv[4];
+  bool yok[4] = {false, false, false, false};
+  if (straddle) {
+    const long long t0 = split - split % bm, t1 = min(t0 + (long long)bm, (long long)a.count);
+    const long long ra = g == 0 ? t0 : split, rb = g == 0 ? split : t1;
+#pragma unroll
+    for (int i = 0; i < 4; ++i) {
+      const long long r = ra + (threadIdx.x >> 2) + 64 * i;
+      yok[i] = ycol < C && r < rb;
+      if (yok[i]) yv[i] = LD4(y + (size_t)r * ldy + ycol);
+    }
   }
   double sum[2];
   float ext[2];
   reduce_rows16<4, 2, true>(partials + (size_t)row0 * 4 * C, nrows, C, bx * 16, sum, ext);
+  if (straddle) {
+    double c1[4] = {0.0, 0.0, 0.0, 0.0}, c2[4] = {0.0, 0.0, 0.0, 0.0};
+    float mn[4] = {3.0e38f, 3.0e38f, 3.0e38f, 3.0e38f}, mx[4] = {-3.0e38f, -3.0e38f, -3.0e38f, -3.0e38f};
+#pragma unroll
+    for (int i = 0; i < 4; ++i) {
+      if (!yok[i]) continue;
+#pragma unroll
+      for (int j = 0; j < 4; ++j) {
+        const float v = yv[i][j];
+        c1[j] += (double)v;
+        c2[j] += (double)v * (double)v;
+        mn[j] = fminf(mn[j], v);
+        mx[j] = fmaxf(mx[j], v);
+      }
+    }
+#pragma unroll
+    for (int o = 4; o < 64; o <<= 1) {
+#pragma unroll
+      for (int j = 0; j < 4; ++j) {
+        c1[j] += __shfl_xor(c1[j], o, 64);
+        c2[j] += __shfl_xor(c2[j], o, 64);
+        mn[j] = fminf(mn[j], __shfl_xor(mn[j], o, 64));
+        mx[j] = fmaxf(mx[j], __shfl_xor(mx[j], o, 64));
+      }
+    }
+    if ((threadIdx.x & 63) < 4) {
+#pragma unroll
+      for (int j = 0; j < 4; ++j) {
+        ysum[threadIdx.x >> 6][0][4 * yq + j] = c1[j];
+        ysum[threadIdx.x >> 6][1][4 * yq + j] = c2[j];
+        yext[threadIdx.x >> 6][0][4 * yq + j] = mn[j];
+        yext[threadIdx.x >> 6][1][4 * yq + j] = mx[j];
+      }
+    }
+    __syncthreads();
+  }
   const int ch = bx * 16 + threadIdx.x;
   float bound = 0.f;
   if (threadIdx.x < 16 && ch < C) {
-    if (split > 0 && split % bm != 0) {
-      double c1 = 0.0, c2 = 0.0;
-      float mn = 3.0e38f, mx = -3.0e38f;
-      for (long long r = split - split % bm; r < split; ++r) {
-        const float v = y[(size_t)r * ldy + ch];
-        c1 += (double)v;
-        c2 += (double)v * (double)v;
-        mn = fminf(mn, v);
-        mx = fmaxf(mx, v);
-      }
-      if (g == 0) {
-        sum[0] += c1;
-        sum[1] += c2;
-        ext[0] = fminf(ext[0], mn);
-        ext[1] = fmaxf(ext[1], mx);
-      } else {
-        sum[0] -= c1;
-        sum[1] -= c2;
-      }
+    if (straddle) {
+      const int t = threadIdx.x;
+      sum[0] += ((ysum[0][0][t] + ysum[1][0][t]) + ysum[2][0][t]) + ysum[3][0][t];
+      sum[1] += ((ysum[0][1][t] + ysum[1][1][t]) + ysum[2][1][t]) + ysum[3][1][t];
+      ext[0] = fminf(ext[0], fminf(fminf(yext[0][0][t], yext[1][0][t]), fminf(yext[2][0][t], yext[3][0][t])));
+      ext[1] = fmaxf(ext[1], fmaxf(fmaxf(yext[0][1][t], yext[1][1][t]), fmaxf(yext[2][1][t], yext[3][1][t])));
     }
     const double mu = sum[0] / count;
     double var = sum[1] / count - mu * mu;
@@ -275,6 +293,8 @@
   }
 }
 __global__ __launch_bounds__(256) void bn_finalize_l2_kernel(const BnFinalizeArgs a) { bn_finalize_block(a, blockIdx.x, blockIdx.y); }
+
+__device__ __forceinline__ f32x4 bn_affine(const f32x4 x, const f32x4 mu, const f32x4 sc, const f32x4 be) { return (x - mu) * sc + be; }
 
 template <bool FUSED>
 __global__ __launch_bounds__(256) void bn_apply_l2_kernel(const float* __restrict__ x, const float* mean, const float* invstd,
@@ -308,7 +328,7 @@
   auto lofs = [&](size_t e) { return (size_t)((unsigned)e / (unsigned)c8) * 2 * (size_t)C + lcol; };
   auto one = [&](size_t e, f32x4 x0, f32x4 x1, u32x4 r1, u32x4 r2, bool whole) {
     const bool second = group1_at > 0 && e >= group1_at;
-    f32x4 v0 = (x0 - (second ? nu0 : mu0)) * (second ? tc0 : sc0) + be0, v1 = (x1 - (second ? nu1 : mu1)) * (second ? tc1 : sc1) + be1;
+    f32x4 v0 = bn_affine(x0, second ? nu0 : mu0, second ? tc0 : sc0, be0), v1 = bn_affine(x1, second ? nu1 : mu1, second ? tc1 : sc1, be1);
     if (res) {
       f32x4 q0, q1;
       join8(r1, r2, q0, q1);
@@ -354,6 +374,66 @@
       r2 = *reinterpret_cast<const u32x4*>(res + lofs(e) + LIMB2_OFS);
     }
     one(e, LD4(x + e * 8), LD4(x + e * 8 + 4), r1, r2, __ballot(1) == ~0ull);
+  }
+}
+
+__global__ __launch_bounds__(256) void bn_relu_maxpool_l2_kernel(const float* __restrict__ y, const float* __restrict__ mean,
+                                                                 const float* __restrict__ invstd, const float* __restrict__ gamma,
+                                                                 const float* __restrict__ beta, _Float16* __restrict__ out,
+                                                                 const float* __restrict__ out_amax, unsigned char* __restrict__ idx,
+                                                                 int Hi, int Wi, int Ho, int Wo, int C, size_t total8, size_t group1_at) {
+  const int c8 = C / 8;
+  const float so = scale_of(out_amax).s;
+  const size_t e0 = (size_t)blockIdx.x * blockDim.x + threadIdx.x;
+  const int col = (int)(e0 % c8) * 8;
+  const f32x4 ga0 = LD4(gamma + col), ga1 = LD4(gamma + col + 4);
+  const f32x4 sc0 = LD4(invstd + col) * ga0, sc1 = LD4(invstd + col + 4) * ga1;
+  const f32x4 mu0 = LD4(mean + col), mu1 = LD4(mean + col + 4), be0 = LD4(beta + col), be1 = LD4(beta + col + 4);
+  const int g1 = group1_at > 0 ? C : 0;
+  const f32x4 tc0 = LD4(invstd + g1 + col) * ga0, tc1 = LD4(invstd + g1 + col + 4) * ga1;
+  const f32x4 nu0 = LD4(mean + g1 + col), nu1 = LD4(mean + g1 + col + 4);
+  const size_t lcol = limb_at(0, col, C);
+  for (size_t e = e0; e < total8; e += (size_t)gridDim.x * blockDim.x) {
+    const bool second = group1_at > 0 && e >= group1_at;
+    const f32x4 m0 = second ? nu0 : mu0, m1 = second ? nu1 : mu1, a0 = second ? tc0 : sc0, a1 = second ? tc1 : sc1;
+    const unsigned q = (unsigned)e / (unsigned)c8;
+    const int wo = (int)(q % (unsigned)Wo);
+    const unsigned t = q / (unsigned)Wo;
+    const int ho = (int)(t % (unsigned)Ho), b = (int)(t / (unsigned)Ho);
+    f32x4 b0 = {-INFINITY, -INFINITY, -INFINITY, -INFINITY}, b1 = b0;
+    unsigned s0 = 0, s1 = 0;
+    bool first = true;
+#pragma unroll
+    for (int r = 0; r < 3; ++r) {
+      const int hi = ho * 2 - 1 + r;
+      if ((unsigned)hi >= (unsigned)Hi) continue;
+#pragma unroll
+      for (int s = 0; s < 3; ++s) {
+        const int wi = wo * 2 - 1 + s;
+        if ((unsigned)wi >= (unsigned)Wi) continue;
+        const float* p = y + (((size_t)b * Hi + hi) * Wi + wi) * C + col;
+        f32x4 v0 = bn_affine(LD4S(p), m0, a0, be0), v1 = bn_affine(LD4S(p + 4), m1, a1, be1);
+        const unsigned slot = (unsigned)(r * 3 + s);
+#pragma unroll
+        for (int j = 0; j < 4; ++j) {
+          v0[j] = fmaxf(v0[j], 0.f);
+          v1[j] = fmaxf(v1[j], 0.f);
+          if (first || v0[j] > b0[j] || v0[j] != v0[j]) {
+            b0[j] = v0[j];
+            s0 = (s0 & ~(0xffu << (8 * j))) | (slot << (8 * j));
+          }
+          if (first || v1[j] > b1[j] || v1[j] != v1[j]) {
+            b1[j] = v1[j];
+            s1 = (s1 & ~(0xffu << (8 * j))) | (slot << (8 * j));
+          }
+        }
+        first = false;
+      }
+    }
+    u32x4 l1, l2;
+    split8(b0 * so, b1 * so, l1, l2);
+    store_limb_lines(out + (size_t)q * 2 * (size_t)C + lcol, l1, l2, __ballot(1) == ~0ull);
+    if (idx != nullptr) *reinterpret_cast<u32x2*>(idx + e * 8) = u32x2{s0, s1};
   }
 }
 
@@ -536,6 +616,131 @@
   }
 }
 
+__device__ __forceinline__ f32x4 pool_gather4(const float* __restrict__ dy, const unsigned char* __restrict__ idx, int b, int hi, int wi,
+                                              int col, int Ho, int Wo, int C) {
+  f32x4 acc = {0.f, 0.f, 0.f, 0.f};
+  const int ho_lo = hi / 2, ho_hi = (hi + 1) / 2;
+  const int wo_lo = wi / 2, wo_hi = (wi + 1) / 2;
+  for (int ho = ho_lo; ho <= ho_hi; ++ho) {
+    if (ho >= Ho) continue;
+    for (int wo = wo_lo; wo <= wo_hi; ++wo) {
+      if (wo >= Wo) continue;
+      const int slot = (hi - (ho * 2 - 1)) * 3 + (wi - (wo * 2 - 1));
+      const size_t o = (((size_t)b * Ho + ho) * Wo + wo) * C + col;
+      const unsigned pk = *reinterpret_cast<const unsigned*>(idx + o);
+      const f32x4 g = LD4(dy + o);
+#pragma unroll
+      for (int j = 0; j < 4; ++j)
+        if ((int)((pk >> (8 * j)) & 0xff) == slot) acc[j] += g[j];
+    }
+  }
+  return acc;
+}
+__device__ __forceinline__ f32x4 relu_gate4(f32x4 g, const f32x4 v) {
+#pragma unroll
+  for (int j = 0; j < 4; ++j) g[j] = v[j] > 0.f ? g[j] : 0.f;
+  return g;
+}
+
+__global__ __launch_bounds__(256) void stem_bwd_reduce_l2_kernel(const float* __restrict__ dy, const unsigned char* __restrict__ idx,
+                                                                 const float* __restrict__ x, const float* __restrict__ mean,
+                                                                 const float* __restrict__ invstd, const float* __restrict__ gamma,
+                                                                 const float* __restrict__ beta, int Hi, int Wi, int Ho, int Wo,
+                                                                 int64_t M, int C, int cx, int64_t rows_per_chunk,
+                                                                 float* __restrict__ partials, int64_t split, int chunks0) {
+  __shared__ f32x4 red[3][256];
+  const int t = threadIdx.x;
+  const int ry_n = 256 / cx;
+  const int tx = t % cx, ty = t / cx;
+  const int col = (blockIdx.x * cx + tx) * 4;
+  const int chunk = blockIdx.y;
+  const bool second = split > 0 && chunk >= chunks0;
+  const int64_t r0 = second ? split + (int64_t)(chunk - chunks0) * rows_per_chunk : (int64_t)chunk * rows_per_chunk;
+  const int64_t r1 = min(split > 0 && !second ? split : M, r0 + rows_per_chunk);
+  f32x4 s1 = {0.f, 0.f, 0.f, 0.f}, s2 = {0.f, 0.f, 0.f, 0.f}, s3 = {0.f, 0.f, 0.f, 0.f};
+  if (col < C) {
+    const int gofs = second ? C : 0;
+    const f32x4 mu = LD4(mean + gofs + col), is = LD4(invstd + gofs + col);
+    const f32x4 sc = is * LD4(gamma + col), be = LD4(beta + col);
+    for (int64_t r = r0 + ty; r < r1; r += ry_n) {
+      const unsigned wi = (unsigned)r % (unsigned)Wi, q = (unsigned)r / (unsigned)Wi;
+      const int hi = (int)(q % (unsigned)Hi), b = (int)(q / (unsigned)Hi);
+      const f32x4 xv = LD4(x + (size_t)r * C + col);
+      const f32x4 g = relu_gate4(pool_gather4(dy, idx, b, hi, (int)wi, col, Ho, Wo, C), bn_affine(xv, mu, sc, be));
+      const f32x4 xh = (xv - mu) * is;
+      s1 += g;
+      s2 += g * xh;
+#pragma unroll
+      for (int j = 0; j < 4; ++j) s3[j] = fmaxf(s3[j], fabsf(g[j]));
+    }
+  }
+  red[0][t] = s1;
+  red[1][t] = s2;
+  red[2][t] = s3;
+  __syncthreads();
+  if (ty == 0 && col < C) {
+    for (int y = 1; y < ry_n; ++y) {
+      s1 += red[0][y * cx + tx];
+      s2 += red[1][y * cx + tx];
+      const f32x4 o3 = red[2][y * cx + tx];
+#pragma unroll
+      for (int j = 0; j < 4; ++j) s3[j] = fmaxf(s3[j], o3[j]);
+    }
+    float* dst = partials + ((size_t)chunk * 3) * C + col;
+    *reinterpret_cast<f32x4*>(dst) = s1;
+    *reinterpret_cast<f32x4*>(dst + C) = s2;
+    *reinterpret_cast<f32x4*>(dst + 2 * C) = s3;
+  }
+}
+
+__global__ __launch_bounds__(256) void stem_bwd_apply_l2_kernel(const float* __restrict__ dy, const unsigned char* __restrict__ idx,
+                                                                const float* __restrict__ x, const float* __restrict__ mean,
+                                                                const float* __restrict__ invstd, const float* __restrict__ gamma,
+                                                                const float* __restrict__ beta, const float* __restrict__ sums,
+                                                                _Float16* __restrict__ dx, const float* __restrict__ dx_amax, int Hi,
+                                                                int Wi, int Ho, int Wo, size_t total8, int C, float inv_m,
+                                                                size_t group1_at, float inv_m1) {
+  const int c8 = C / 8;
+  const float sd = scale_of(dx_amax).s;
+  const size_t e0 = (size_t)blockIdx.x * blockDim.x + threadIdx.x;
+  const int col = (int)(e0 % c8) * 8;
+  f32x4 is[2][2], mu[2][2], gi[2][2], m1[2][2], m2[2][2], be[2];
+#pragma unroll
+  for (int g = 0; g < 2; ++g) {
+    const int go = g && group1_at > 0 ? C : 0;
+    const float im = g && group1_at > 0 ? inv_m1 : inv_m;
+#pragma unroll
+    for (int h = 0; h < 2; ++h) {
+      const int cc = col + 4 * h;
+      is[g][h] = LD4(invstd + go + cc);
+      mu[g][h] = LD4(mean + go + cc);
+      gi[g][h] = LD4(gamma + cc) * is[g][h];
+      m1[g][h] = LD4(sums + 2 * go + cc) * im;
+      m2[g][h] = LD4(sums + 2 * go + C + cc) * im;
+    }
+  }
+  be[0] = LD4(beta + col);
+  be[1] = LD4(beta + col + 4);
+  for (size_t e = e0; e < total8; e += (size_t)gridDim.x * blockDim.x) {
+    const bool second = group1_at > 0 && e >= group1_at;
+    const unsigned r = (unsigned)e / (unsigned)c8;
+    const unsigned wi = r % (unsigned)Wi, q = r / (unsigned)Wi;
+    const int hi = (int)(q % (unsigned)Hi), b = (int)(q / (unsigned)Hi);
+    f32x4 v[2];
+#pragma unroll
+    for (int h = 0; h < 2; ++h) {
+      const f32x4 xv = LD4S(x + e * 8 + 4 * h);
+      const f32x4 mm = second ? mu[1][h] : mu[0][h], ii = second ? is[1][h] : is[0][h], gg = second ? gi[1][h] : gi[0][h];
+      const f32x4 g = relu_gate4(pool_gather4(dy, idx, b, hi, (int)wi, col + 4 * h, Ho, Wo, C), bn_affine(xv, mm, gg, be[h]));
+      const f32x4 xh = (xv - mm) * ii;
+      v[h] = gg * (g - (second ? m1[1][h] : m1[0][h]) - xh * (second ? m2[1][h] : m2[0][h]));
+    }
+    u32x4 l1, l2;
+    split8(v[0] * sd, v[1] * sd, l1, l2);
+    store_limb_lines(dx + (size_t)r * 2 * (size_t)C + limb_at(0, col, C), l1, l2, __ballot(1) == ~0ull);
+  }
+}
+
 __global__ __launch_bounds__(256) void chan_scale_limbs_kernel(const float* __restrict__ x, const float* __restrict__ gate,
                                                                _Float16* __restrict__ out, size_t plane,
                                                                const float* __restrict__ amax, int64_t HW, int C, size_t total8) {
@@ -580,8 +785,8 @@
                         const float* beta, const float* res_amax, int relu, float* xhat_amax, float* out_amax, int64_t split,
                         int tile_rows, int run_group, const float* y, int ldy, onda_stream_t s) {
   ONDA_REQUIRE(partials && mean && invstd && gamma && beta && xhat_amax && out_amax && tiles >= 1 && C >= 4 && C % 4 == 0 && count >= 1);
-  ONDA_REQUIRE(split >= 0 && split < count && (split == 0 || (tile_rows > 0 && y && ldy >= C && split / tile_rows < tiles)));
-  if (!ONDA_ALIGNED16(partials)) return ONDA_EALIGN;
+  ONDA_REQUIRE(split >= 0 && split < count && (split == 0 || (tile_rows > 0 && tile_rows <= 256 && y && ldy >= C && split / tile_rows < tiles)));
+  if (!ONDA_ALIGNED16(partials) || (split > 0 && (!ONDA_ALIGNED16(y) || ldy % 4 != 0))) return ONDA_EALIGN;
   hipLaunchKernelGGL(bn_finalize_l2_kernel, dim3((C + 15) / 16, split > 0 ? 2 : 1), dim3(256), 0, ONDA_STREAM(s),
                      finalize_args(partials, tiles, C, count, eps, mean, invstd, running_mean, running_var, nbt, momentum, gamma, beta,
                                    res_amax, relu, xhat_amax, out_amax, split, tile_rows, run_group, y, ldy));
@@ -619,7 +824,7 @@
                      uint8_t* relu_mask, int64_t split, int tile_rows, int run_group, onda_stream_t s) {
   ONDA_REQUIRE(x && partials && mean && invstd && gamma && beta && xhat_amax && out && out_amax && tiles >= 1 && M >= 1);
   ONDA_REQUIRE(C % 32 == 0 && (!res || res_amax) && (256 % (C / 8) == 0 || (C / 8) % 256 == 0));
-  ONDA_REQUIRE(split >= 0 && split < M && (split == 0 || (tile_rows > 0 && split / tile_rows < tiles)));
+  ONDA_REQUIRE(split >= 0 && split < M && (split == 0 || (tile_rows > 0 && tile_rows <= 256 && split / tile_rows < tiles)));
   if (!ONDA_ALIGNED16(x) || !ONDA_ALIGNED16(out) || (res && !ONDA_ALIGNED16(res)) || !ONDA_ALIGNED16(partials)) return ONDA_EALIGN;
   const size_t total8 = (size_t)M * C / 8;
   const int nfin = (C + 15) / 16 * (split > 0 ? 2 : 1);
@@ -680,4 +885,46 @@
   return ONDA_LAUNCH_RESULT();
 }
 
-}
+static inline bool stem_pool_geometry(int B, int Hi, int Wi, int C, int Ho, int Wo, int first_images) {
+  return B > 0 && Hi > 0 && Wi > 0 && Ho > 0 && Wo > 0 && C % 32 == 0 && 256 % (C / 8) == 0 && 2 * (Ho - 1) - 1 < Hi &&
+         2 * (Wo - 1) - 1 < Wi && 2 * Ho >= Hi && 2 * Wo >= Wi && (int64_t)B * Hi * Wi * (C / 8) < (int64_t)1 << 31 &&
+         first_images >= 0 && first_images < B;
+}
+
+int onda_bn_relu_maxpool_l2(const float* y, const float* mean, const float* invstd, const float* gamma, const float* beta, void* out,
+                            const float* out_amax, uint8_t* idx, int B, int Hi, int Wi, int C, int Ho, int Wo, int first_images,
+                            onda_stream_t s) {
+  ONDA_REQUIRE(y && mean && invstd && gamma && beta && out && out_amax && stem_pool_geometry(B, Hi, Wi, C, Ho, Wo, first_images));
+  if (!ONDA_ALIGNED16(y) || !ONDA_ALIGNED16(out) || (idx && !ONDA_ALIGNED16(idx))) return ONDA_EALIGN;
+  const size_t per_image = (size_t)Ho * Wo * (C / 8), total8 = (size_t)B * per_image;
+  hipLaunchKernelGGL(bn_relu_maxpool_l2_kernel, dim3(ew_grid(total8)), dim3(256), 0, ONDA_STREAM(s), y, mean, invstd, gamma, beta,
+                     static_cast<_Float16*>(out), out_amax, idx, Hi, Wi, Ho, Wo, C, total8, (size_t)first_images * per_image);
+  return ONDA_LAUNCH_RESULT();
+}
+
+int onda_bn_relu_maxpool_bwd_l2(const float* dy, const uint8_t* idx, const float* y, const float* mean, const float* invstd,
+                                const float* gamma, const float* beta, const float* xhat_amax, void* dx, float* dx_amax, float* ws,
+                                int B, int Hi, int Wi, int C, int Ho, int Wo, int first_images, onda_stream_t s) {
+  ONDA_REQUIRE(dy && idx && y && mean && invstd && gamma && beta && xhat_amax && dx && dx_amax && ws &&
+               stem_pool_geometry(B, Hi, Wi, C, Ho, Wo, first_images));
+  if (!ONDA_ALIGNED16(dy) || !ONDA_ALIGNED16(y) || !ONDA_ALIGNED16(dx) || !ONDA_ALIGNED16(idx)) return ONDA_EALIGN;
+  const int64_t M = (int64_t)B * Hi * Wi, split = (int64_t)first_images * Hi * Wi;
+  const ColPlan3 p = col_plan3(M, C);
+  int chunks0, chunks;
+  bwd_chunks(p, M, split, chunks0, chunks);
+  float* sums = ws + (size_t)(p.chunks + 1) * 3 * C;
+  hipStream_t st = ONDA_STREAM(s);
+  hipLaunchKernelGGL(stem_bwd_reduce_l2_kernel, dim3(p.gridx, chunks), dim3(256), 0, st, dy, idx, y, mean, invstd, gamma, beta, Hi, Wi,
+                     Ho, Wo, M, C, p.cx, p.rows_per_chunk, ws, split, chunks0);
+  const double inv_m0 = 1.0 / (double)(split > 0 ? split : M), inv_m1 = 1.0 / (double)(M - split);
+  const int groups = split > 0 ? 2 : 1;
+  const BnBwdSumsArgs fin{ws, chunks, C, inv_m0, inv_m1, gamma, invstd, xhat_amax, sums, dx_amax, chunks0, groups};
+  hipLaunchKernelGGL(bn_bwd_sums_l2_kernel, dim3((C + 15) / 16, groups), dim3(256), 0, st, fin);
+  const size_t total8 = (size_t)M * C / 8;
+  hipLaunchKernelGGL(stem_bwd_apply_l2_kernel, dim3(ew_grid(total8)), dim3(256), 0, st, dy, idx, y, mean, invstd, gamma, beta, sums,
+                     static_cast<_Float16*>(dx), dx_amax, Hi, Wi, Ho, Wo, total8, C, (float)inv_m0, (size_t)split * C / 8,
+                     (float)inv_m1);
+  return ONDA_LAUNCH_RESULT();
+}
+
+}
diff --git a/onda_amd/framework/model/deeplabv2.py b/onda_amd/framework/model/deeplabv2.py
--- a/onda_amd/framework/model/deeplabv2.py
+++ b/onda_amd/framework/model/deeplabv2.py
@@ -284,7 +284,9 @@
 
     def _stem_train(self, x, running):
         bn = self.bn1
-        y, stats = ops.StemConvFn.apply(x, self.conv1.weight, self.conv1._pack, True)
+        y, stats = ops.StemConvFn.apply(x, self.conv1.weight, self.conv1._pack, 4 if ops.limb_mode(self.conv1.out_channels) else True)
+        if stats.shape[1] == 4:
+            return ops.StemBNPoolFn.apply(y, stats, bn.weight, bn.bias, running, bn.momentum)
         y = ops.BNTrainFn.apply(y, stats, bn.weight, bn.bias, None, True, running, bn.momentum)
         return ops.MaxPoolFn.apply(y, True)
 
diff --git a/onda_amd/ops/conv.py b/onda_amd/ops/conv.py
--- a/onda_amd/ops/conv.py
+++ b/onda_amd/ops/conv.py
@@ -501,7 +501,9 @@
             return None, None, None, None
         (col,) = ctx.saved_tensors
         into = _accumulate_target(ctx.weight)
-        dw = conv_wgrad(col, as_nhwc(dy), 1, 1, 1, 0, ctx.cout, 3, flat_k=49, into=into, xlimbs=ctx.col_limbs)
+        if not is_limb_only(dy):
+            dy = as_nhwc(dy)
+        dw = conv_wgrad(col, dy, 1, 1, 1, 0, ctx.cout, 3, flat_k=49, into=into, xlimbs=ctx.col_limbs)
         if into is not None and _state.GRAD_READY is not None:
             _state.GRAD_READY(ctx.weight)
         return None, dw, None, None
diff --git a/onda_amd/ops/norm.py b/onda_amd/ops/norm.py
--- a/onda_amd/ops/norm.py
+++ b/onda_amd/ops/norm.py
@@ -162,6 +162,56 @@
         return dx, None, None, None, dres, None, None, None
 
 
+def pool_out_size(n):
+    o = -(-(n - 1) // 2) + 1
+    return o - 1 if (o - 1) * 2 - 1 >= n else o
+
+
+class StemBNPoolFn(torch.autograd.Function):
+
+    @staticmethod
+    def forward(ctx, y, stats, gamma, beta, running, momentum):
+        B, Hi, Wi, C = y.shape
+        M, dev = B * Hi * Wi, y.device
+        if nhwc_ld(y) != C or not y.is_contiguous():
+            raise RuntimeError("onda_amd: the stem's fused BatchNorm + pool needs a dense conv output")
+        Ho, Wo = pool_out_size(Hi), pool_out_size(Wi)
+        split = _group_split(B, Hi, Wi)
+        first = split // (Hi * Wi)
+        mean = torch.empty((2 if split else 1) * C, device=dev, dtype=torch.float32)
+        invstd, xhat_amax = torch.empty_like(mean), torch.empty_like(mean)
+        rm, rv, nbt = running if running is not None else (None, None, None)
+        out_amax = amax_slot(dev)
+        call("onda_bn_finalize_l2", _p(stats), stats.shape[0], C, M, BN_EPS, _p(mean), _p(invstd), _p(rm), _p(rv), _p(nbt),
+             float(momentum), _p(gamma), _p(beta), None, 1, _p(xhat_amax), _p(out_amax), split,
+             _stat_tile_rows(stats) if split else 0, 1, _p(y) if split else None, C if split else 0, _stream())
+        if running is not None:
+            for t in running:
+                torch.autograd.graph.increment_version(t)
+        planes = torch.empty(2, B * Ho * Wo, C, device=dev, dtype=torch.float16)
+        idx = torch.empty(B, Ho, Wo, C, device=dev, dtype=torch.uint8) if any(ctx.needs_input_grad) else None
+        call("onda_bn_relu_maxpool_l2", _p(y), _p(mean), _p(invstd), _p(gamma), _p(beta), _p(planes), _p(out_amax), _p(idx),
+             B, Hi, Wi, C, Ho, Wo, first, _stream())
+        ctx.save_for_backward(y, mean, invstd, gamma, beta, xhat_amax, idx)
+        ctx.first = first
+        return limb_only((B, Ho, Wo, C), dev, Limbs(planes, out_amax, C, B * Ho * Wo * C))
+
+    @staticmethod
+    def backward(ctx, dout):
+        y, mean, invstd, gamma, beta, xhat_amax, idx = ctx.saved_tensors
+        B, Hi, Wi, C = y.shape
+        M, dev = B * Hi * Wi, y.device
+        if is_limb_only(dout):
+            raise RuntimeError("onda_amd: the gradient of the pooled stem output must be an fp32 tensor")
+        dout = dout.contiguous()
+        ws = torch.empty(query("onda_bn_bwd_l2_ws", M, C), device=dev, dtype=torch.float32)
+        planes = torch.empty(2, M, C, device=dev, dtype=torch.float16)
+        dx_amax = amax_slot(dev)
+        call("onda_bn_relu_maxpool_bwd_l2", _p(dout), _p(idx), _p(y), _p(mean), _p(invstd), _p(gamma), _p(beta), _p(xhat_amax),
+             _p(planes), _p(dx_amax), _p(ws), B, Hi, Wi, C, dout.shape[1], dout.shape[2], ctx.first, _stream())
+        return limb_only((B, Hi, Wi, C), dev, Limbs(planes, dx_amax, C, M * C)), None, None, None, None, None
+
+
 def fold_bounds(weight, scale, shift):
     with torch.no_grad():
         l1 = weight.detach().abs().sum(dim=(1, 2, 3))
@@ -180,11 +230,7 @@
     @staticmethod
     def forward(ctx, x, limbs=False):
         B, Hi, Wi, C = x.shape
-        Ho, Wo = -(-(Hi - 1) // 2) + 1, -(-(Wi - 1) // 2) + 1
-        if (Ho - 1) * 2 - 1 >= Hi:
-            Ho -= 1
-        if (Wo - 1) * 2 - 1 >= Wi:
-            Wo -= 1
+        Ho, Wo = pool_out_size(Hi), pool_out_size(Wi)
         idx = torch.empty(B, Ho, Wo, C, device=x.device, dtype=torch.uint8)
         x = x.contiguous()
         slot = known_amax(x)
```

New measurement: 43.01 images/s (median of 6 runs). Within noise of the previous version (+0.5%).
